# RuyiLian/CheckerPose

Hardware: AMD Instinct MI355X
Metric: crops/sec forward (256x256, npt=512) (higher is better)
Workload: dtype bf16; 1 GPU; LMO 'ape' hr18GNN2_res6_gnn3Skip_mlpQuery npt=512, PoseNet_GNNskip forward, deterministic random-init weights; global_batch=256, parallelism=dp1 (no forward collective), launch=hipGraph replay of 104 kernel launches

## Files before the change

checkerpose_amd/_abi.py:

```python
import ctypes as C
import os

_HERE = os.path.dirname(os.path.abspath(__file__))
LIB_PATH = os.environ.get("CHECKERPOSE_AMD_LIB") or os.path.join(_HERE, "libcheckerpose_hip.so")

CP_F32, CP_BF16, CP_F16 = 0, 1, 2
ACT_NONE, ACT_RELU, ACT_LEAKY = 0, 1, 2
LOSS_BCE, LOSS_L1 = 0, 1
POSE_ERR_ADD, POSE_ERR_ADI = 1, 2


class CpConvDesc(C.Structure):
    _fields_ = [("dtype", C.c_int32), ("out_f32", C.c_int32), ("B", C.c_int32), ("H", C.c_int32), ("W", C.c_int32),
                ("Cin", C.c_int32), ("in_cstride", C.c_int32), ("in_coff", C.c_int32),
                ("R", C.c_int32), ("S", C.c_int32), ("stride", C.c_int32), ("pad", C.c_int32),
                ("Ho", C.c_int32), ("Wo", C.c_int32), ("Cout", C.c_int32), ("act", C.c_int32), ("slope", C.c_float), ("ksplit", C.c_int32),
                ("o_base", C.c_int64), ("o_sb", C.c_int64), ("o_sy", C.c_int64), ("o_sx", C.c_int64),
                ("o_sc", C.c_int64)]


_P, _I, _F, _L = C.c_void_p, C.c_int, C.c_float, C.c_longlong


class CpChainTail(C.Structure):
    _fields_ = [("packed_w", C.c_void_p), ("shift", C.c_void_p), ("out", C.c_void_p * 3), ("nconv", C.c_int32),
                ("Cout", C.c_int32 * 3), ("out_cphys", C.c_int32 * 3), ("relu", C.c_int32 * 3)]


class CpChainTailConv(C.Structure):
    _fields_ = [("packed_w", C.c_void_p), ("shift", C.c_void_p), ("out", C.c_void_p),
                ("kind", C.c_int32), ("Cout", C.c_int32), ("out_cphys", C.c_int32), ("relu", C.c_int32)]


class CpI2fGather(C.Structure):
    _fields_ = [("patches", C.c_void_p), ("x_id", C.c_void_p), ("y_id", C.c_void_p), ("mask", C.c_void_p), ("zeros", C.c_void_p),
                ("p_cstride", C.c_int32), ("p_coff", C.c_int32), ("Hp", C.c_int32), ("Wp", C.c_int32), ("k", C.c_int32)]


class CpFuseConv(C.Structure):
    _fields_ = [("packed_w", C.c_void_p), ("affine", C.c_void_p), ("out", C.c_void_p),
                ("kind", C.c_int32), ("Cout", C.c_int32), ("out_cphys", C.c_int32), ("relu", C.c_int32)]


class CpPackItem(C.Structure):
    _fields_ = [("kind", C.c_int32), ("a", C.c_int32 * 9), ("src", C.c_void_p), ("dst", C.c_void_p), ("row_map", C.c_void_p),
                ("total", C.c_uint64)]


class CpWgradReduceItem(C.Structure):
    _fields_ = [("ws", C.c_void_p), ("dw", C.c_void_p), ("S", C.c_int32), ("GY", C.c_int32), ("co_blocks", C.c_int32),
                ("ci_blocks", C.c_int32), ("R", C.c_int32), ("Ssz", C.c_int32), ("Cout", C.c_int32), ("Cin", C.c_int32),
                ("taps_in_block", C.c_int32), ("dw_base", C.c_int64), ("dw_sco", C.c_int64), ("dw_sci", C.c_int64),
                ("dw_sr", C.c_int64), ("dw_ss", C.c_int64)]


CP_BN_ITEM_STATS, CP_BN_ITEM_APPLY, CP_BN_ITEM_BWD_SUMS, CP_BN_ITEM_BWD_APPLY = 0, 1, 2, 3
BN_GROUP_MAX = 16


class CpBnItem(C.Structure):
    _fields_ = [("kind", C.c_int32), ("dtype", C.c_int32), ("blocks", C.c_uint32), ("lds_bytes", C.c_uint32),
                ("params", C.c_uint64 * 24)]


CP_WGRAD_ITEM_3X3, CP_WGRAD_ITEM_3X3_SMALL, CP_WGRAD_ITEM_GENERIC_BF16, CP_WGRAD_ITEM_GENERIC_F32 = 0, 1, 2, 3
CP_WGRAD_ITEM_3X3_S2_SMALL = 4


class CpWgradItem(C.Structure):
    _fields_ = [("kind", C.c_int32), ("blocks", C.c_uint32), ("gx", C.c_uint32), ("gy", C.c_uint32), ("params", C.c_uint64 * 20)]


class CpOptItem(C.Structure):
    _fields_ = [("p", C.c_void_p), ("g", C.c_void_p), ("m", C.c_void_p), ("v", C.c_void_p), ("n", C.c_uint64), ("step0", C.c_uint32),
                ("pad", C.c_uint32)]


class CpFuseBwdItem(C.Structure):
    _fields_ = [("dout", C.c_void_p), ("out", C.c_void_p), ("dsrc", C.c_void_p), ("Hs", C.c_int32), ("Ws", C.c_int32), ("CG", C.c_int32),
                ("shift", C.c_int32), ("relu", C.c_int32), ("accumulate", C.c_int32), ("total", C.c_uint64)]


class CpWgradDesc(C.Structure):
    _fields_ = [("dtype", C.c_int32), ("B", C.c_int32), ("H", C.c_int32), ("W", C.c_int32), ("Ho", C.c_int32),
                ("Wo", C.c_int32), ("Cout", C.c_int32), ("dy_cstride", C.c_int32), ("dy_coff", C.c_int32),
                ("Cin", C.c_int32), ("x_cstride", C.c_int32), ("x_coff", C.c_int32),
                ("R", C.c_int32), ("S", C.c_int32), ("stride", C.c_int32), ("pad", C.c_int32),
                ("dw_base", C.c_int64), ("dw_sco", C.c_int64), ("dw_sci", C.c_int64), ("dw_sr", C.c_int64),
                ("dw_ss", C.c_int64)]


SIGNATURES = {
    "cp_version": (_I, []),
    "cp_device_status": (_I, [_P, _I]),
    "cp_set_deterministic": (None, [_I]),
    "cp_get_deterministic": (_I, []),
    "cp_strerror": (C.c_char_p, [_I]),
    "cp_last_kernel": (C.c_char_p, []),
    "cp_kernel_log_begin": (None, []),
    "cp_kernel_log": (C.c_char_p, []),
    "cp_chan_align": (_I, [_I]),
    "cp_packed_weight_bytes": (C.c_size_t, [_I, _I, _I, _I, _I]),
    "cp_pack_conv_weight": (_I, [_P, _I, _P, _I, _I, _I, _I, _I, _I, _I, _P, _I, _P]),
    "cp_conv2d_igemm": (_I, [_P, C.POINTER(CpConvDesc), _P, _P, _P, _P, _P, _P]),
    "cp_conv2d_igemm_splitk": (_I, [_I, C.c_longlong, _I, _I]),
    "cp_packed_halo_weight_bytes": (C.c_size_t, [_I, _I, _I]),
    "cp_pack_conv3x3_halo_weight": (_I, [_P, _I, _P, _I, _I, _I, _P]),
    "cp_conv3x3_halo": (_I, [_P, C.POINTER(CpConvDesc), _P, _P, _P, _P, _P, _P]),
    "cp_conv2x2_halo_supported": (_I, [_I, _I, _I, _I]),
    "cp_packed_conv2x2_halo_weight_bytes": (C.c_size_t, [_I, _I, _I]),
    "cp_pack_conv2x2_halo_weight": (_I, [_P, _I, _P, _I, _I, _I, _P]),
    "cp_conv2x2_halo": (_I, [_P, C.POINTER(CpConvDesc), _P, _P, _P, _P, _P, _P]),
    "cp_conv3x3_s2_small_supported": (_I, [_I, _I, _I, _I]),
    "cp_conv3x3_s2_small_weight_bytes": (C.c_size_t, [_I, _I]),
    "cp_pack_conv3x3_s2_small_weight": (_I, [_P, _P, _I, _I, _I, _I, _P]),
    "cp_conv3x3_s2_small": (_I, [_P, C.POINTER(CpConvDesc), _P, _P, _P, _P, _P]),
    "cp_conv3x3_halo_up2x_supported": (_I, [_I, _I]),
    "cp_conv3x3_halo_up2x": (_I, [_P, C.POINTER(CpConvDesc), _P, _P, _P, _P, _P]),
    "cp_conv3x3_halo_seg_supported": (_I, [_I, _I, _I]),
    "cp_conv3x3_halo_seg": (_I, [_P, C.POINTER(CpConvDesc), _P, _P, _P, _P, _P, _P, _P, _I, _P]),
    "cp_pack_conv3x3_rows_weight": (_I, [_P, _I, _P, _I, _I, _I, _P]),
    "cp_basicblock_fused": (_I, [_P, C.POINTER(CpConvDesc), _P, _P, _P, _P, _P, _P, _P, _P]),
    "cp_bottleneck_fused": (_I, [_P, C.POINTER(CpConvDesc)] + [_P] * 14),
    "cp_packed_gemm_weight_bytes": (C.c_size_t, [_I, _I, _I]),
    "cp_pack_gemm_weight": (_I, [_P, _I, _P, _I, _I, _I, _P]),
    "cp_gemm_rows": (_I, [_P, C.POINTER(CpConvDesc), _P, _P, _P, _P, _P, _P]),
    "cp_mlp_query_fused_supported": (_I, [_I, _I, _I, _I]),
    "cp_mlp_query_fused": (_I, [_P, _P, _I, _I, _I, _I, _P, _P, _P, _F, _P, _P, _P, _F, _P, _P, _P, _L, _L, _L, _L]),
    "cp_mlp_query_fused_t": (_I, [_P, _I, _P, _I, _I, _I, _I, _P, _P, _P, _F, _P, _P, _P, _F, _P, _P, _P, _L, _L, _L, _L]),
    "cp_mlp_query_fused_n": (_I, [_P, _I, _P, _I, _I, _I, _I, _P, _P, _P, _F, _P, _P, _P, _F, _P, _P, _I, _P, _L, _L, _L, _L,
                                  _P, _P, _P, _P]),
    "cp_mlp_pair_fused_supported": (_I, [_I, _I, _I]),
    "cp_mlp_pair_fused": (_I, [_P, _P, _I, _I, _I, _I, _I, _P, _P, _F, _P, _P, _F, _P, _I, _I]),
    "cp_mlp_pair_fused_t": (_I, [_P, _I, _P, _I, _I, _I, _I, _I, _P, _P, _F, _P, _P, _F, _P, _I, _I]),
    "cp_mlp_pair_fused_gather_supported": (_I, [_I, _I, _I]),
    "cp_mlp_pair_fused_gather": (_I, [_P, C.POINTER(CpI2fGather), _P, _I, _I, _I, _I, _I, _P, _P, _F, _P, _P, _F, _P, _I, _I]),
    "cp_mlp_pair_fused_gather_t": (_I, [_P, _I, C.POINTER(CpI2fGather), _P, _I, _I, _I, _I, _I, _P, _P, _F, _P, _P, _F, _P, _I, _I]),
    "cp_hr_stem_weight_bytes": (C.c_size_t, [_I]),
    "cp_pack_hr_stem_weights": (_I, [_P, _P, _P, _P, _P]),
    "cp_hr_stem": (_I, [_P, _P, _I, _I, _I, _P, _P, _P, _P, _P, _P, _P]),
    "cp_hr_chain_supported": (_I, [_I, _I, _I]),
    "cp_hr_chain_weight_bytes": (C.c_size_t, [_I, _I, _I]),
    "cp_hr_chain_affine_floats": (_I, [_I, _I, _I]),
    "cp_pack_hr_chain_weight": (_I, [_P, _P, _P, _I, _I, _I, _I, _P]),
    "cp_hr_branch_chain": (_I, [_P, _I, _I, _I, _I, _I, C.POINTER(_P), C.POINTER(C.c_int32), _I, _P, _P, _P]),
    "cp_hr_chain_tail_supported": (_I, [_I, _I, _I]),
    "cp_hr_chain_tail_weight_bytes": (C.c_size_t, []),
    "cp_hr_chain_tail_channels": (_I, []),
    "cp_pack_hr_chain_tail_weight": (_I, [_P, _P, _P, _I, _I, _I, _P]),
    "cp_hr_branch_chain_tail": (_I, [_P, _I, _I, _I, _I, _I, C.POINTER(_P), C.POINTER(C.c_int32), _I, _P, _P, _P, C.POINTER(CpChainTail)]),
    "cp_hr_chain_tailconv_supported": (_I, [_I, _I, _I, _I, _I]),
    "cp_hr_chain_tailconv_weight_bytes": (C.c_size_t, [_I, _I, _I, _I, _I]),
    "cp_pack_hr_chain_tailconv_weight": (_I, [_P, _P, _P, _I, _I, _I, _I, _I, _P]),
    "cp_hr_branch_chain_tails": (_I, [_P, _I, _I, _I, _I, _I, C.POINTER(_P), C.POINTER(C.c_int32), _I, _P, _P, _P, _I, C.POINTER(CpChainTailConv)]),
    "cp_upsample2x_bilinear_ac": (_I, [_P, _I, _P, _P, _I, _I, _I, _I, _I, _I, _I, _I]),
    "cp_fuse_sum_act": (_I, [_P, _I, _I, C.POINTER(_P), C.POINTER(C.c_int32), _P, _I, _I, _I, _I, _I, _I, _I]),
    "cp_maxpool3x3s2": (_I, [_P, _I, _P, _P, _I, _I, _I, _I]),
    "cp_edgeconv_gather_max": (_I, [_P, _I, _P, _P, _P, _P, _I, _I, _I, _I, _I, _I, _I, _F]),
    "cp_hr_fuse_out_supported": (_I, [_I, _I, _I]),
    "cp_hr_fuse_out_weight_bytes": (C.c_size_t, [_I, _I, _I]),
    "cp_hr_fuse_out_affine_floats": (_I, [_I]),
    "cp_pack_hr_fuse_out_weight": (_I, [_P, _P, _I, _I, _I, _I, _I, _P]),
    "cp_hr_fuse_out": (_I, [_P, _P, _I, _I, _I, _I, _I, C.POINTER(CpFuseConv)]),
    "cp_edgeconv_fused_supported": (_I, [_I, _I, _I, _I]),
    "cp_edgeconv_fused_weight_bytes": (C.c_size_t, [_I, _I]),
    "cp_pack_edgeconv_fused_weight": (_I, [_P, _P, _I, _I, _P]),
    "cp_edgeconv_fused": (_I, [_P, _P, _I, _I, _P, _P, _P, _P, _P, _P, _I, _I, _I, _I, _I, _I, _I, _I, _F]),
    "cp_pack_edgeconv_fused_weight_t": (_I, [_P, _I, _P, _I, _I, _P]),
    "cp_edgeconv_fused_t": (_I, [_P, _I, _P, _I, _I, _P, _P, _P, _P, _P, _P, _I, _I, _I, _I, _I, _I, _I, _I, _F]),
    "cp_edgeconv_tiled_supported": (_I, [_I, _I, _I, _I, _I]),
    "cp_edgeconv_tiled_weight_bytes": (C.c_size_t, [_I, _I]),
    "cp_edgeconv_tiled_table_bytes": (C.c_size_t, [_I, _I, _I]),
    "cp_pack_edgeconv_tiled_weight": (_I, [_P, _P, _I, _I, _P]),
    "cp_edgeconv_tiled": (_I, [_P, _P, _I, _I, _P, _P, _P, _P, _P, _P, _P, _P, _P, _I, _I, _I, _I, _I, _I, _I, _I, _I, _F]),
    "cp_pack_edgeconv_tiled_weight_t": (_I, [_P, _I, _P, _I, _I, _P]),
    "cp_edgeconv_tiled_t": (_I, [_P, _I, _P, _I, _I, _P, _P, _P, _P, _P, _P, _P, _P, _P, _I, _I, _I, _I, _I, _I, _I, _I, _I, _F]),
    "cp_permute_rows": (_I, [_P, _P, _P, _P, _P, _I, _I, _I]),
    "cp_permute_cols": (_I, [_P, _P, _P, _P, _P, _I, _I, _I, _I, _I]),
    "cp_index2feat_conv_supported": (_I, [_I, _I, _I]),
    "cp_index2feat_conv_weight_bytes": (C.c_size_t, []),
    "cp_pack_index2feat_conv_weight": (_I, [_P, _P, _P]),
    "cp_index2feat_conv": (_I, [_P, _P, _I, _I, _P, _P, _P, _P, _P, _P, _I, _I, _I, _I, _I, _I, _I]),
    "cp_index2feat_conv_t": (_I, [_P, _I, _P, _I, _I, _P, _P, _P, _P, _P, _P, _I, _I, _I, _I, _I, _I, _I]),
    "cp_index2feat_gather": (_I, [_P, _I, _P, _P, _P, _P, _P, _I, _I, _I, _I, _I, _I, _I, _I]),
    "cp_bits_decode": (_I, [_P, _P, _I, _P, _P, _P, _P, _P, _I, _I]),
    "cp_code_decode": (_I, [_P, _P, _I, _I, _P, _P, _P, _P, _I, _I]),
    "cp_correspondences": (_I, [_P, _P, _P, _P, _P, _P, _P, _P, _P, _I, _I, _I, _I, _I]),
    "cp_correspondences_bbox": (_I, [_P, _P, _P, _P, _P, _P, _P, _P, _P, _I, _I, _I, _I, _I]),
    "cp_pnp_ransac_scratch_bytes": (C.c_size_t, [_I, _I]),
    "cp_pnp_ransac": (_I, [_P, _P, _L, _P, _P, _I, _P, _L, _I, _I, _F, _I, C.c_uint32, _P, _P, _P, _P]),
    "cp_pose_errors_scratch_bytes": (C.c_size_t, [_I, _I]),
    "cp_pose_errors": (_I, [_P, _P, _P, _P, _P, _I, _P, _I, _I, _I, _P, _P, _P]),
    "cp_encode_targets": (_I, [_P, _P, _L, _P, _I, _P, _L, _P, _P, _P, _P, _P, _I, _I, _I, _P, _P, _P, _P, _P, _P, _P]),
    "cp_code_report": (_I, [_P, _P, _L, _P, _L, _P, _L, _I, _P, _I, _I, _P, _P, _P, _I, _P, _P, _I, _I, _I, _I, _P, _P]),
    "cp_edgeconv_bwd_workspace_bytes": (C.c_size_t, [_I, _I, _I]),
    "cp_edgeconv_gather_max_bwd": (_I, [_P, _I, _P, _P, _P, _P, _P, _P, _P, _P, _I, _I, _I, _I, _I, _I, _I, _F]),
    "cp_index2feat_gather_bwd": (_I, [_P, _P, _P, _P, _P, _P, _I, _I, _I, _I, _I, _I, _I, _I]),
    "cp_loss_workspace_bytes": (C.c_size_t, []),
    "cp_code_loss": (_I, [_P, _I, _P, _L, _P, _L, _P, _I, _I, _I, _P, _P, _L, _P]),
    "cp_mask_loss": (_I, [_P, _P, _L, _P, _I, _I, _I, _I, _I, _P, _P, _L, _P]),
    "cp_masked_ce_loss": (_I, [_P, _P, _L, _P, _P, _I, _I, _I, _P, _P, _L, _P]),
    "cp_conv2d_wgrad": (_I, [_P, C.POINTER(CpWgradDesc), _P, _P, _P]),
    "cp_conv2d_wgrad_ws": (_I, [_P, C.POINTER(CpWgradDesc), _P, _P, _P, _P, C.c_size_t]),
    "cp_conv2d_wgrad_scratch_bytes": (C.c_size_t, [C.POINTER(CpWgradDesc)]),
    "cp_conv2d_wgrad_deferred": (_I, [_P, C.POINTER(CpWgradDesc), _P, _P, _P, _P, C.c_size_t, C.POINTER(CpWgradReduceItem)]),
    "cp_conv2d_wgrad_plan": (_I, [C.POINTER(CpWgradDesc), _P, _P, _P, _P, C.c_size_t, C.POINTER(CpWgradReduceItem)]),
    "cp_conv2d_wgrad_item": (_I, [C.POINTER(CpWgradDesc), _P, _P, _P, _P, C.c_size_t, _I, C.POINTER(CpWgradItem), C.POINTER(CpWgradReduceItem)]),
    "cp_wgrad_group": (_I, [_P, _I, _P, _P, _I, C.c_uint32]),
    "cp_opt_item_blocks": (C.c_uint32, [C.c_uint64]),
    "cp_adam_multi": (_I, [_P, _P, _P, _I, C.c_uint32, _F, _F, _F, _F, _F, _I]),
    "cp_sgd_multi": (_I, [_P, _P, _P, _I, C.c_uint32, _F, _F, _F, _I]),
    "cp_wgrad_reduce_item_blocks": (C.c_uint32, [C.POINTER(CpWgradReduceItem)]),
    "cp_wgrad_reduce_batch": (_I, [_P, _P, _P, _I, C.c_uint32]),
    "cp_weight_dgrad": (_I, [_P, _P, _I, _I, _I, _I, _P]),
    "cp_bn_workspace_bytes": (C.c_size_t, [_I]),
    "cp_bn_train_stats": (_I, [_P, _I, _P, _I, _I, _I, _I, _P, _P, _P, _P, _F, _F, _P, _P, _P, _P, _P]),
    "cp_affine_act": (_I, [_P, _I, _P, _I, _I, _P, _P, _P, _I, _I, _P, _I, _I, _I, _I, _I, _F]),
    "cp_bn_bwd_workspace_bytes": (C.c_size_t, [_I]),
    "cp_bn_train_bwd": (_I, [_P, _I, _P, _I, _I, _P, _I, _I, _P, _I, _I, _P, _P, _P, _I, _I, _I, _F, _P, _I, _I, _P, _I, _I,
                             _I, _P, _P, _P]),
    "cp_pack_item_conv": (_I, [_I, _P, _I, _I, _I, _I, _I, _I, _I, _P, _I, _P, C.POINTER(CpPackItem)]),
    "cp_pack_item_halo": (_I, [_I, _P, _I, _I, _I, _P, C.POINTER(CpPackItem)]),
    "cp_pack_item_gemm": (_I, [_I, _P, _I, _I, _I, _P, C.POINTER(CpPackItem)]),
    "cp_pack_item_dgrad_view": (_I, [_P, _I, _I, _I, _I, _P, C.POINTER(CpPackItem)]),
    "cp_pack_item_edge_view": (_I, [_P, _I, _I, _I, _P, C.POINTER(CpPackItem)]),
    "cp_pack_item_copy_f32": (_I, [_P, _P, _I, C.POINTER(CpPackItem)]),
    "cp_pack_batch": (_I, [_P, _I, _P, _P, _I, C.c_uint32]),
    "cp_bn_acc_doubles": (C.c_size_t, [_I]),
    "cp_bn_stats_accumulate": (_I, [_P, _I, _P, _I, _I, _I, _I, _P]),
    "cp_bn_apply": (_I, [_P, _I, _P, _I, _I, _P, _P, _P, _P, _P, _F, _F, _P, _I, _I, _P, _I, _I, _I, _I, _I, _F, _P, _P]),
    "cp_bn_bwd_accumulate": (_I, [_P, _I, _P, _I, _I, _P, _I, _I, _P, _I, _I, _P, _P, _I, _I, _I, _F, _P]),
    "cp_bn_bwd_apply": (_I, [_P, _I, _P, _I, _I, _P, _I, _I, _P, _I, _I, _P, _P, _P, _P, _I, _I, _I, _F, _P, _I, _I, _P, _I, _I,
                             _I, _P, _P]),
    "cp_bn_item_stats": (_I, [_I, _P, _I, _I, _I, _I, _P, C.POINTER(CpBnItem)]),
    "cp_bn_item_apply": (_I, [_I, _P, _I, _I, _P, _P, _P, _P, _P, _F, _F, _P, _I, _I, _P, _I, _I, _I, _I, _I, _F, _P, _P,
                              C.POINTER(CpBnItem)]),
    "cp_bn_item_bwd_sums": (_I, [_I, _P, _I, _I, _P, _I, _I, _P, _I, _I, _P, _P, _I, _I, _I, _F, _P, C.POINTER(CpBnItem)]),
    "cp_bn_item_bwd_apply": (_I, [_I, _P, _I, _I, _P, _I, _I, _P, _I, _I, _P, _P, _P, _P, _I, _I, _I, _F, _P, _I, _I, _P, _I, _I,
                                  _I, _P, _P, C.POINTER(CpBnItem)]),
    "cp_bn_group": (_I, [_P, _I, _I, _P, _P, _I, C.c_uint32, C.c_uint32]),
    "cp_edge_train_workspace_bytes": (C.c_size_t, [_I, _I]),
# ... 78 lines not shown
```

checkerpose_amd/csrc/hr_chain.hip:

```cpp
#include <stdlib.h>

#include "common.h"

size_t cp_chain0_conv_bytes();
int cp_chain0_aff();
int cp_chain0_pack(hipStream_t st, const float* w, const float* scale, int conv_index, void* blob);
int cp_chain0_launch(hipStream_t st, int B, int nsrc, const void* const* srcs, const int32_t* shifts, int relu_in,
                     const void* packed_w, const float* affine, void* out, const CpChainTail* tail);
size_t cp_chain0_tail_bytes();
int cp_chain0_tail_channels();
int cp_chain0_tail_pack(hipStream_t st, const float* w, const float* scale, int Cout, int first_piece, int out_cphys, void* blob);

namespace {

template <int C_, int H_, int W_, int CPW_, int NWC_, int S_, int RL_>
struct ChainCfg {
  static constexpr int C = C_, H = H_, W = W_, CPW = CPW_, NWC = NWC_, S = S_, RL = RL_;
  static constexpr int NW = 8, NTHR = 512;
  static constexpr int CPHYS = (C + 7) / 8 * 8;
  static constexpr int CG = CPHYS / 8;
  static constexpr int NT_ALL = (C + 15) / 16;
  static constexpr int KC = (9 * CG + 3) / 4;
  static constexpr int KCP = (KC + S - 1) / S * S;
  static constexpr int NS = KCP / S;
  static constexpr int HP = H + 2, WP = W + 2;
  static constexpr bool PLANES = W >= 16;
  static constexpr int PLANE = (HP * WP + 15) / 16 * 16 * 16;
  static constexpr int SLOTS = (CG % 2) ? CG : CG + 1;
  static constexpr int PIX = PLANES ? 16 : SLOTS * 16;
  static constexpr int GRP = PLANES ? PLANE : 16;
  static constexpr int MAP = PLANES ? CG * PLANE : HP * WP * SLOTS * 16;
  static constexpr int FPC = H * W / 16;
  static constexpr int NFRAG = CPW * FPC;
  static constexpr int NWP = NW / NWC;
  static constexpr int MT = NFRAG / NWP;
  static constexpr int PM = MT < 4 ? MT : 4;
  static constexpr int NST = MT / PM;
  static constexpr int NTW = (NT_ALL + NWC - 1) / NWC;
  static constexpr int SLAB = S * NT_ALL * 1024;
  static constexpr int WITER = (SLAB / 16 + NTHR - 1) / NTHR;
  static constexpr int AFF = NT_ALL * 16;
  static constexpr int AFF_BYTES = 2 * 2 * AFF * 4;
  static constexpr int RES_LDS = NW * RL * NTW * 64 * 8;
  static constexpr int LDS = CPW * MAP + 2 * SLAB + AFF_BYTES + RES_LDS;
  static constexpr size_t CONV_W = (size_t)KCP * NT_ALL * 1024;
  static_assert(NFRAG % NWP == 0 && MT % PM == 0 && RL <= MT, "fragments must split evenly over the pixel waves");
  static_assert(W >= 16 ? (W % 16 == 0) : (W == 8), "fragment = 16 pixels of a row, or two 8-pixel rows");
  static_assert((SLAB / 16) % 64 == 0, "slab pieces are copied by whole waves");
  static_assert(LDS <= 160 * 1024, "LDS budget");
};

using CfgB1 = ChainCfg<36, 32, 32, 1, 1, 3, 4>;
using CfgB2 = ChainCfg<72, 16, 16, 2, 1, 3, 0>;
using CfgB3 = ChainCfg<144, 8, 8, 4, 2, 2, 0>;
using CfgB2m = ChainCfg<72, 16, 16, 1, 1, 3, 0>;
using CfgB3h = ChainCfg<144, 8, 8, 2, 2, 2, 0>;
using CfgB3m = ChainCfg<144, 8, 8, 1, 2, 2, 0>;

struct ChainTailConv {
  const void* w;
  const float* shift;
  void* out;
  int kind, nt, out_cp, relu;
};
struct ChainParams {
  const void* src[4];
  int shift[4];
  int nsrc, relu_in;
  const void* w;
  const float* aff;
  void* out;
  int B;
  int dbg;
  int ntail;
  ChainTailConv tc[3];
};

#ifdef CP_DEBUG_KNOBS
#define CHAIN_DBG(bit) (p.dbg & (bit))
#else
#define CHAIN_DBG(bit) 0
#endif

__device__ __forceinline__ void mma16(const u32x4& w, const u32x4& a, f32x4& acc) {
  acc = __builtin_amdgcn_mfma_f32_16x16x32_bf16(__builtin_bit_cast(bf16x8, w), __builtin_bit_cast(bf16x8, a), acc, 0, 0, 0);
}

template <typename Cfg, int NSRC>
__device__ __forceinline__ void stage_sources(const ChainParams& p, unsigned char* sMap, int tid, int crop0) {
  constexpr int CG = Cfg::CG, H = Cfg::H, W = Cfg::W, U = 4;
  constexpr int TOTAL = Cfg::CPW * H * W * CG;
  for (int i0 = tid; i0 < TOTAL; i0 += U * Cfg::NTHR) {
    u32x4 v[U][NSRC];
    uint32_t dst[U];
    bool ok[U];
#pragma unroll
    for (int u = 0; u < U; ++u) {
      const int i = i0 + u * Cfg::NTHR;
      const int g = i % CG;
      int t = i / CG;
      const int c = t / (H * W);
      t -= c * (H * W);
      const int y = t / W, xx = t - y * W;
      const int b = crop0 + c;
      ok[u] = i < TOTAL;
      dst[u] = (uint32_t)(c * Cfg::MAP + ((y + 1) * Cfg::WP + xx + 1) * Cfg::PIX + g * Cfg::GRP);
      const bool ld = ok[u] && b < p.B && !(CHAIN_DBG(1));
#pragma unroll
      for (int k = 0; k < NSRC; ++k) {
        const int sh = p.shift[k];
        const size_t o = (((size_t)b * (H >> sh) + (y >> sh)) * (W >> sh) + (xx >> sh)) * CG + g;
        v[u][k] = ld ? ((const u32x4*)p.src[k])[o] : u32x4{0u, 0u, 0u, 0u};
      }
    }
#pragma unroll
    for (int u = 0; u < U; ++u) {
      float acc[8], f[8];
#pragma unroll
      for (int k = 0; k < NSRC; ++k) {
        Vec16<BF16Tag>::unpack(v[u][k], f);
#pragma unroll
        for (int j = 0; j < 8; ++j) acc[j] = (k == 0) ? f[j] : acc[j] + f[j];
      }
      if (p.relu_in) {
#pragma unroll
        for (int j = 0; j < 8; ++j) acc[j] = fmaxf(acc[j], 0.f);
      }
      if (ok[u]) *(u32x4*)(sMap + dst[u]) = Vec16<BF16Tag>::pack(acc);
    }
  }
}

template <typename Cfg, int KIND, int NT, int TG>
__device__ __forceinline__ void chain_tail_conv(const ChainTailConv& t, const unsigned char* sMap, int lane, int wave, int crop0, int B) {
  constexpr int CG = Cfg::CG, H = Cfg::H, W = Cfg::W, WP = Cfg::WP, PIX = Cfg::PIX, GRP = Cfg::GRP, MAP = Cfg::MAP, CPW = Cfg::CPW;
  constexpr int HT = KIND ? H / 2 : H, WT = KIND ? W / 2 : W;
  static_assert(WT >= 16 ? WT % 16 == 0 : WT == 8, "a tail fragment is 16 pixels of an output row, or two 8-pixel rows");
  constexpr int FG = 8 / TG, NTW = (NT + TG - 1) / TG;
  constexpr int FPC = HT * WT / 16, NF = CPW * FPC, FW = (NF + FG - 1) / FG;
  constexpr int KC = KIND ? (9 * CG + 3) / 4 : (CG + 3) / 4;
  constexpr uint32_t CENTER = (uint32_t)((WP + 1) * PIX);
  const int x = lane & 15, q = lane >> 4;
  const int tg = wave % TG, fg = wave / TG;
  const int nt0 = tg * NTW;
  if (nt0 >= NT) return;
  const int ntn = nt0 + NTW <= NT ? NTW : NT - nt0;
  uint32_t base[FW];
  int opix[FW];
  int crop[FW];
#pragma unroll
  for (int f = 0; f < FW; ++f) {
    const int F = fg + FG * f;
    const int c = F / FPC, Fc = F - c * FPC;
    int orow, ocol;
    if (WT >= 16) { orow = Fc / (WT / 16); ocol = (Fc - orow * (WT / 16)) * 16 + x; }
    else { orow = Fc * 2 + (x >> 3); ocol = x & 7; }
    const bool live = F < NF;
    crop[f] = c;
// ... 202 lines not shown
    }

#pragma unroll 1
    for (int s = 0; s < NS; ++s, ++gs) {
      if (gs + 1 < TOTAL_SLABS && !CHAIN_DBG(8)) slab_issue(gs + 1, (gs + 1) & 1);
      if (active) {
        const unsigned char* const sWb = sW + (gs & 1) * SLAB + nt0 * 1024 + lane * 16;
        const int kc0 = s * S;
        u32x4 af[2][PM], wf[2][NTW];
        {
          const uint32_t o = a_off(kc0);
#pragma unroll
          for (int i = 0; i < PM; ++i) af[0][i] = *(const u32x4*)(sMap + base[i] + o);
#pragma unroll
          for (int nt = 0; nt < NTW; ++nt)
            if (has(nt)) wf[0][nt] = *(const u32x4*)(sWb + nt * 1024);
        }
#pragma unroll
        for (int cc = 0; cc < S; ++cc) {
#pragma unroll
          for (int st = 0; st < NST; ++st) {
            const int cur = (cc * NST + st) & 1;
            const bool last = (cc == S - 1) && (st == NST - 1);
            if (!last) {
              const int ncc = (st == NST - 1) ? cc + 1 : cc, nst = (st == NST - 1) ? 0 : st + 1;
              const uint32_t o = a_off(kc0 + ncc);
#pragma unroll
              for (int i = 0; i < PM; ++i) af[cur ^ 1][i] = *(const u32x4*)(sMap + base[nst * PM + i] + o);
            }
            if (st == 0 && cc + 1 < S) {
#pragma unroll
              for (int nt = 0; nt < NTW; ++nt)
                if (has(nt)) wf[(cc + 1) & 1][nt] = *(const u32x4*)(sWb + ((cc + 1) * NT_ALL + nt) * 1024);
            }
            __builtin_amdgcn_sched_barrier(0);
#pragma unroll
            for (int i = 0; i < PM; ++i)
#pragma unroll
              for (int nt = 0; nt < NTW; ++nt)
                if (has(nt)) mma16(wf[cc & 1][nt], af[cur][i], acc[st * PM + i][nt]);
            __builtin_amdgcn_sched_barrier(0);
          }
        }
      }
      __syncthreads();
    }

    if (tid < 2 * AFF) sAff[((cv + 1) & 1) * 2 * AFF + tid] = affv;
    {
#pragma unroll
      for (int nt = 0; nt < NTW; ++nt) {
        const int c0 = q * 4 * NT_ALL + (nt0 + nt) * 4;
        if (has(nt) && c0 < CPHYS) {
          uint32_t co = c_off(c0);
          asm volatile("" : "+v"(co));
#pragma unroll
          for (int f = 0; f < MT; ++f) {
            u32x2 pk;
            pk.x = relu_bf16x2(pack_bf16x2(acc[f][nt][0], acc[f][nt][1]));
            pk.y = relu_bf16x2(pack_bf16x2(acc[f][nt][2], acc[f][nt][3]));
            *(u32x2*)(sMap + base[f] + co) = pk;
          }
        }
      }
    }
    __syncthreads();
  }

  if (!CHAIN_DBG(4)) {
    constexpr int TOTAL = CPW * H * W * CG;
#pragma unroll 4
    for (int i = tid; i < TOTAL; i += NTHR) {
      const int g = i % CG;
      int t = i / CG;
      const int c = t / (H * W);
      t -= c * (H * W);
      const int y = t / W, xx = t - y * W;
      const int b = crop0 + c;
      if (b < p.B)
        ((u32x4*)p.out)[(((size_t)b * H + y) * W + xx) * CG + g] = *(const u32x4*)(sMap + c * MAP + ((y + 1) * WP + xx + 1) * PIX + g * GRP);
    }
  }
  if constexpr (TAIL) chain_tails<Cfg>(p, sMap, lane, wave, crop0);
}

__global__ void pack_chain_tail_kernel(const float* __restrict__ w, const float* __restrict__ scale, uint16_t* __restrict__ out, int Cin,
                                       int CG, int Cout, int NT, int kind, size_t total) {
  const size_t i = (size_t)blockIdx.x * blockDim.x + threadIdx.x;
  if (i >= total) return;
  const int e = (int)(i % 8);
  const int lane = (int)((i / 8) % 64);
  size_t blk = i / 512;
  const int nt = (int)(blk % NT);
  const int kc = (int)(blk / NT);
  const int row = lane & 15, q = lane >> 4;
  const int G = kc * 4 + q;
  int tap = -1, cin = 0;
  if (kind) { tap = G / CG; cin = (G % CG) * 8 + e; if (tap >= 9) tap = -1; }
  else if (G < CG) { tap = 0; cin = G * 8 + e; }
  const int n = (row >> 2) * 4 * NT + nt * 4 + (row & 3);
  const int KK = kind ? 9 : 1;
  float v = 0.f;
  if (tap >= 0 && cin < Cin && n < Cout) v = w[((size_t)n * Cin + cin) * KK + tap] * (scale ? scale[n] : 1.f);
  out[i] = (uint16_t)f32_to_bf16_bits(v);
}

__global__ void pack_chain_weight_kernel(const float* __restrict__ w, const float* __restrict__ scale, uint16_t* __restrict__ out, int C,
                                         int CG, int NT_ALL, size_t total) {
  const size_t i = (size_t)blockIdx.x * blockDim.x + threadIdx.x;
  if (i >= total) return;
  const int e = (int)(i % 8);
  const int lane = (int)((i / 8) % 64);
  size_t blk = i / 512;
  const int nt = (int)(blk % NT_ALL);
  const int kc = (int)(blk / NT_ALL);
  const int row = lane & 15, q = lane >> 4;
  const int G = kc * 4 + q;
  const int tap = G / CG, cin = (G % CG) * 8 + e;
  const int n = (row >> 2) * 4 * NT_ALL + nt * 4 + (row & 3);
  float v = 0.f;
  if (tap < 9 && cin < C && n < C) v = w[((size_t)n * C + cin) * 9 + tap] * (scale ? scale[n] : 1.f);
  out[i] = (uint16_t)f32_to_bf16_bits(v);
}

constexpr int CHAIN_CPW_FULL_B = 192;

template <typename Cfg>
int launch_chain(hipStream_t st, const ChainParams& p) {
  static CpDeviceOnce once;
  const int dev = cp_current_device();
  CP_LDS_ATTR_ONCE(once, dev, cp_set_max_lds((const void*)hr_chain_kernel<Cfg, false>, Cfg::LDS) &&
                                  cp_set_max_lds((const void*)hr_chain_kernel<Cfg, true>, Cfg::LDS));
  const unsigned grid = (unsigned)((p.B + Cfg::CPW - 1) / Cfg::CPW);
  if (p.ntail > 0) CP_LAUNCH((hr_chain_kernel<Cfg, true>), dim3(grid), dim3(Cfg::NTHR), Cfg::LDS, st, p);
  else CP_LAUNCH((hr_chain_kernel<Cfg, false>), dim3(grid), dim3(Cfg::NTHR), Cfg::LDS, st, p);
  return cp_check_launch();
}

int tail_conv_chunks(int C, int kind, int nt) {
  const int CG = (C + 7) / 8;
  bool ok = false;
  if (C == 36) ok = (kind == 0 && nt == 2) || (kind == 1 && (nt == 5 || nt == 3));
  else if (C == 72) ok = (kind == 0 && (nt == 2 || nt == 3)) || (kind == 1 && nt == 9);
  else if (C == 144) ok = kind == 0 && (nt == 2 || nt == 3 || nt == 5);
  if (!ok) return 0;
  return kind ? (9 * CG + 3) / 4 : (CG + 3) / 4;
}

struct ChainInfo { int C, H, W, KCP, NT_ALL, CG, AFF; size_t conv_w; };
bool chain_info(int C, int H, int W, ChainInfo* o) {
#define CP_CI(CFG) if (C == CFG::C && H == CFG::H && W == CFG::W) { *o = ChainInfo{C, H, W, CFG::KCP, CFG::NT_ALL, CFG::CG, CFG::AFF, CFG::CONV_W}; return true; }
  CP_CI(CfgB1) CP_CI(CfgB2) CP_CI(CfgB3)
#undef CP_CI
  if (C == 18 && H == 64 && W == 64) { *o = ChainInfo{C, H, W, 7, 2, 3, cp_chain0_aff(), cp_chain0_conv_bytes()}; return true; }
  return false;
}

}

extern "C" int cp_hr_chain_supported(int C, int H, int W) {
  ChainInfo ci;
  return chain_info(C, H, W, &ci) ? 1 : 0;
}

extern "C" size_t cp_hr_chain_weight_bytes(int C, int H, int W) {
  ChainInfo ci;
  return chain_info(C, H, W, &ci) ? 8 * ci.conv_w : 0;
}

extern "C" int cp_hr_chain_affine_floats(int C, int H, int W) {
  ChainInfo ci;
  return chain_info(C, H, W, &ci) ? ci.AFF : 0;
}

extern "C" int cp_pack_hr_chain_weight(cp_stream_t stream, const float* w, const float* scale, int C, int H, int W, int conv_index,
                                       void* blob) {
  ChainInfo ci;
  if (!w || !blob || conv_index < 0 || conv_index > 7 || !chain_info(C, H, W, &ci)) return CP_ERR_INVALID;
  if (!cp_aligned16(blob)) return CP_ERR_ALIGN;
  if (C == 18) return cp_chain0_pack((hipStream_t)stream, w, scale, conv_index, blob);
  const size_t total = ci.conv_w / 2;
  uint16_t* dst = (uint16_t*)((unsigned char*)blob + (size_t)conv_index * ci.conv_w);
  CP_LAUNCH(pack_chain_weight_kernel, dim3((unsigned)((total + 255) / 256)), dim3(256), 0, (hipStream_t)stream, w, scale, dst, C, ci.CG, ci.NT_ALL, total);
  return cp_check_launch();
}

extern "C" int cp_hr_chain_tail_supported(int C, int H, int W) { return (C == 18 && H == 64 && W == 64) ? 1 : 0; }
extern "C" size_t cp_hr_chain_tail_weight_bytes(void) { return cp_chain0_tail_bytes(); }
extern "C" int cp_hr_chain_tail_channels(void) { return cp_chain0_tail_channels(); }
extern "C" int cp_pack_hr_chain_tail_weight(cp_stream_t stream, const float* w, const float* scale, int Cout, int first_piece, int out_cphys,
                                            void* blob) {
  return cp_chain0_tail_pack((hipStream_t)stream, w, scale, Cout, first_piece, out_cphys, blob);
}

static int branch_chain(cp_stream_t stream, int B, int C, int H, int W, int nsrc, const void* const* srcs, const int32_t* shifts, int relu_in,
                        const void* packed_w, const float* affine, void* out, const CpChainTail* tail, int ntail = 0,
                        const CpChainTailConv* tconvs = nullptr);

extern "C" int cp_hr_chain_tailconv_supported(int C, int H, int W, int kind, int Cout) {
  ChainInfo ci;
  if (C == 18 || !chain_info(C, H, W, &ci) || Cout <= 0 || (kind != 0 && kind != 1)) return 0;
  return tail_conv_chunks(C, kind, (Cout + 15) / 16) > 0 ? 1 : 0;
}
extern "C" size_t cp_hr_chain_tailconv_weight_bytes(int C, int H, int W, int kind, int Cout) {
  if (!cp_hr_chain_tailconv_supported(C, H, W, kind, Cout)) return 0;
  const int nt = (Cout + 15) / 16;
  return (size_t)tail_conv_chunks(C, kind, nt) * nt * 1024;
}
extern "C" int cp_pack_hr_chain_tailconv_weight(cp_stream_t stream, const float* w, const float* scale, int C, int H, int W, int kind, int Cout,
                                                void* packed) {
  if (!w || !packed || !cp_hr_chain_tailconv_supported(C, H, W, kind, Cout)) return CP_ERR_INVALID;
  if (!cp_aligned16(packed)) return CP_ERR_ALIGN;
  const int nt = (Cout + 15) / 16;
  const size_t total = cp_hr_chain_tailconv_weight_bytes(C, H, W, kind, Cout) / 2;
  CP_LAUNCH(pack_chain_tail_kernel, dim3((unsigned)((total + 255) / 256)), dim3(256), 0, (hipStream_t)stream, w, scale, (uint16_t*)packed, C,
            (C + 7) / 8, Cout, nt, kind, total);
  return cp_check_launch();
}
extern "C" int cp_hr_branch_chain_tails(cp_stream_t stream, int B, int C, int H, int W, int nsrc, const void* const* srcs, const int32_t* shifts,
                                        int relu_in, const void* packed_w, const float* affine, void* out, int ntail, const CpChainTailConv* convs) {
  if (ntail < 1 || ntail > 3 || !convs || C == 18) return CP_ERR_INVALID;
  return branch_chain(stream, B, C, H, W, nsrc, srcs, shifts, relu_in, packed_w, affine, out, nullptr, ntail, convs);
}

extern "C" int cp_hr_branch_chain(cp_stream_t stream, int B, int C, int H, int W, int nsrc, const void* const* srcs,
                                  const int32_t* shifts, int relu_in, const void* packed_w, const float* affine, void* out) {
  return branch_chain(stream, B, C, H, W, nsrc, srcs, shifts, relu_in, packed_w, affine, out, nullptr);
}

extern "C" int cp_hr_branch_chain_tail(cp_stream_t stream, int B, int C, int H, int W, int nsrc, const void* const* srcs,
                                       const int32_t* shifts, int relu_in, const void* packed_w, const float* affine, void* out,
                                       const CpChainTail* tail) {
  if (!tail || !cp_hr_chain_tail_supported(C, H, W)) return CP_ERR_INVALID;
  return branch_chain(stream, B, C, H, W, nsrc, srcs, shifts, relu_in, packed_w, affine, out, tail);
}

static int branch_chain(cp_stream_t stream, int B, int C, int H, int W, int nsrc, const void* const* srcs, const int32_t* shifts, int relu_in,
                        const void* packed_w, const float* affine, void* out, const CpChainTail* tail, int ntail, const CpChainTailConv* tconvs) {
  ChainInfo ci;
  if (B <= 0 || !srcs || !shifts || nsrc < 1 || nsrc > 4 || !packed_w || !affine || !out) return CP_ERR_INVALID;
  if (!chain_info(C, H, W, &ci)) return CP_ERR_INVALID;
  if (!cp_aligned16(packed_w) || !cp_aligned16(affine) || !cp_aligned16(out)) return CP_ERR_ALIGN;
  ChainParams p;
  for (int k = 0; k < 4; ++k) { p.src[k] = nullptr; p.shift[k] = 0; }
  for (int k = 0; k < nsrc; ++k) {
    if (!srcs[k] || !cp_aligned16(srcs[k]) || shifts[k] < 0 || shifts[k] > 3) return CP_ERR_INVALID;
    if (((H >> shifts[k]) << shifts[k]) != H || ((W >> shifts[k]) << shifts[k]) != W) return CP_ERR_INVALID;
    if (srcs[k] == out) return CP_ERR_INVALID;
    p.src[k] = srcs[k]; p.shift[k] = shifts[k];
  }
  if (C == 18) return cp_chain0_launch((hipStream_t)stream, B, nsrc, srcs, shifts, relu_in, packed_w, affine, out, tail);
  p.nsrc = nsrc; p.relu_in = relu_in ? 1 : 0;
  p.w = packed_w; p.aff = affine; p.out = out; p.B = B;
  p.dbg = cp_knob("CP_CHAIN_DBG") ? atoi(cp_knob("CP_CHAIN_DBG")) : 0;
  p.ntail = 0;
  for (int i = 0; i < ntail; ++i) {
    const CpChainTailConv& c = tconvs[i];
    const int nt = (c.Cout + 15) / 16;
    if (!c.packed_w || !c.shift || !c.out || c.out == out || !cp_hr_chain_tailconv_supported(C, H, W, c.kind, c.Cout)) return CP_ERR_INVALID;
    if (c.out_cphys % 8 || c.Cout > c.out_cphys || c.out_cphys > nt * 16) return CP_ERR_INVALID;
    if (!cp_aligned16(c.packed_w) || !cp_aligned16(c.shift) || !cp_aligned16(c.out)) return CP_ERR_ALIGN;
    p.tc[i].w = c.packed_w; p.tc[i].shift = c.shift; p.tc[i].out = c.out;
    p.tc[i].kind = c.kind; p.tc[i].nt = nt; p.tc[i].out_cp = c.out_cphys; p.tc[i].relu = c.relu ? 1 : 0;
  }
  p.ntail = ntail;
  hipStream_t st = (hipStream_t)stream;
  if (C == CfgB1::C) return launch_chain<CfgB1>(st, p);
  if (C == CfgB2::C) return B >= CHAIN_CPW_FULL_B ? launch_chain<CfgB2>(st, p) : launch_chain<CfgB2m>(st, p);
  if (B >= CHAIN_CPW_FULL_B) return launch_chain<CfgB3>(st, p);
  return B >= CHAIN_CPW_FULL_B / 2 ? launch_chain<CfgB3h>(st, p) : launch_chain<CfgB3m>(st, p);
}
```

checkerpose_amd/csrc/hr_chain0.hip:

```cpp
#include "common.h"

namespace {

constexpr int ZH = 64, ZW = 64, ZC = 18, ZWP = 66, ZHP = 66;
constexpr int ZPLPX = (ZHP * ZWP + 15) / 16 * 16;
constexpr int ZPL16 = ZPLPX * 16, ZPL4 = ZPLPX * 4;
constexpr int ZAFF = 32;
constexpr int ZLDS = 2 * ZPL16 + ZPL4 + 2 * 2 * ZAFF * 4;
constexpr int ZKC = 6;
constexpr size_t ZCONV_W = (size_t)ZKC * 2 * 1024;
static_assert(ZLDS <= 160 * 1024, "LDS budget");

struct Chain0Params {
  const void* src[4];
  int shift[4];
  int nsrc, relu_in;
  const void* w;
  const float* aff;
  void* out;
  int B;
  int tnp;
  int tps[3], tcph[3], trelu[3];
  const void* tw;
  const float* tshift;
  void* tout[3];
  uint32_t* status;
  int dbg_spin_limit;
};
constexpr int ZTAIL_CH = 96;

__device__ __forceinline__ void mma16z(const u32x4& w, const u32x4& a, f32x4& acc) {
  acc = __builtin_amdgcn_mfma_f32_16x16x32_bf16(__builtin_bit_cast(bf16x8, w), __builtin_bit_cast(bf16x8, a), acc, 0, 0, 0);
}

template <int NSRC>
__device__ __forceinline__ void stage0(const Chain0Params& p, unsigned char* smem, int tid, int b) {
  constexpr int U = 4, TOTAL = ZH * ZW * 3;
  for (int i0 = tid; i0 < TOTAL; i0 += U * 512) {
    u32x4 v[U][NSRC];
#pragma unroll
    for (int u = 0; u < U; ++u) {
      const int i = i0 + u * 512;
      const int g = i % 3, px = i / 3;
      const int y = px >> 6, xx = px & 63;
#pragma unroll
      for (int k = 0; k < NSRC; ++k) {
        const int sh = p.shift[k];
        const size_t o = (((size_t)b * (ZH >> sh) + (y >> sh)) * (ZW >> sh) + (xx >> sh)) * 3 + g;
        v[u][k] = ((const u32x4*)p.src[k])[o];
      }
    }
#pragma unroll
    for (int u = 0; u < U; ++u) {
      const int i = i0 + u * 512;
      const int g = i % 3, px = i / 3;
      const int y = px >> 6, xx = px & 63;
      float acc[8], f[8];
#pragma unroll
      for (int k = 0; k < NSRC; ++k) {
        Vec16<BF16Tag>::unpack(v[u][k], f);
#pragma unroll
        for (int j = 0; j < 8; ++j) acc[j] = (k == 0) ? f[j] : acc[j] + f[j];
      }
      if (p.relu_in) {
#pragma unroll
        for (int j = 0; j < 8; ++j) acc[j] = fmaxf(acc[j], 0.f);
      }
      const u32x4 pk = Vec16<BF16Tag>::pack(acc);
      const int pc = (y + 1) * ZWP + xx + 1;
      if (g < 2) *(u32x4*)(smem + g * ZPL16 + pc * 16) = pk;
      else *(uint32_t*)(smem + 2 * ZPL16 + pc * 4) = pk.x;
      ((u32x4*)p.out)[((size_t)b * ZH * ZW + px) * 3 + g] = pk;
    }
  }
}

#ifdef CP_DEBUG_KNOBS
__device__ unsigned long long z_stamps[8][8];
#define Z_T0() unsigned long long z_t = __builtin_amdgcn_s_memtime(), z_acc[8] = {0, 0, 0, 0, 0, 0, 0, 0}
#define Z_MARK(k) do { const unsigned long long n_ = __builtin_amdgcn_s_memtime(); z_acc[k] += n_ - z_t; z_t = n_; } while (0)
#define Z_DUMP() do { if (blockIdx.x == 0 && lane == 0) for (int k_ = 0; k_ < 8; ++k_) z_stamps[wave][k_] = z_acc[k_]; } while (0)
#else
#define Z_T0() do {} while (0)
#define Z_MARK(k) do {} while (0)
#define Z_DUMP() do {} while (0)
#endif

__global__ __launch_bounds__(512) void hr_chain0_kernel(const Chain0Params p) {
  extern __shared__ __attribute__((aligned(16))) unsigned char smem[];
  float* const sAff = (float*)(smem + 2 * ZPL16 + ZPL4);
  const int tid = threadIdx.x;
  const int lane = tid & 63;
  const int wave = __builtin_amdgcn_readfirstlane(tid >> 6);
  const int x = lane & 15, q = lane >> 4;
  const int b = blockIdx.x;

  const u32x4* const wg = (const u32x4*)p.w;
  u32x4 Wf[ZKC][2];
#pragma unroll
  for (int kc = 0; kc < ZKC; ++kc)
#pragma unroll
    for (int nt = 0; nt < 2; ++nt) Wf[kc][nt] = wg[(kc * 2 + nt) * 64 + lane];

  for (int i = tid; i < ZPLPX; i += 512) {
    const int ry = i / ZWP, rx = i - ry * ZWP;
    if (ry == 0 || ry >= ZH + 1 || rx == 0 || rx == ZW + 1) {
      *(u32x4*)(smem + i * 16) = u32x4{0u, 0u, 0u, 0u};
      *(u32x4*)(smem + ZPL16 + i * 16) = u32x4{0u, 0u, 0u, 0u};
      *(uint32_t*)(smem + 2 * ZPL16 + i * 4) = 0u;
    }
// ... 353 lines not shown
      const uint32_t a16 = live && g < 2 ? ro + (uint32_t)(g * PP1 + (px + 1) * 16) : POOR;
      const uint32_t a4 = live && g == 2 ? ro + (uint32_t)(PP2 + (px + 1) * 4) : POOR;
      *(u32x4*)(smem + a16) = pk;
      *(uint32_t*)(smem + a4) = pk.x;
      p_post(cnt + PC_PART + part, (p_cnt_t*)nullptr, (uint32_t)(ys + 1), lane);
      ++ys;
      did = true;
    }
    if (oy < ZH / 2 && p_peek(cnt + 8) >= (2 * oy + 2 < ZH ? 2 * oy + 2 : ZH)) {
      asm volatile("" ::: "memory");
      uint32_t rb[3];
#pragma unroll
      for (int r = 0; r < 3; ++r) {
        const int yy = 2 * oy - 1 + r;
        rb[r] = yy < 0 ? (uint32_t)PZERO : p_ring(8) + p_slot(8, yy);
      }
      f32x4 acc[2][2];
      u32x4 af[2][2];
      p_load<2>(af[0], 0, smem, tg, rb, qlo, q3);
#pragma unroll
      for (int kc = 0; kc < ZKC; ++kc) {
        if (kc + 1 < ZKC) p_load<2>(af[(kc + 1) & 1], kc + 1, smem, tg, rb, qlo, q3);
        __builtin_amdgcn_sched_barrier(0);
#pragma unroll
        for (int f = 0; f < 2; ++f) {
          if (kc == 0) {
            acc[f][0] = __builtin_amdgcn_mfma_f32_16x16x32_bf16(__builtin_bit_cast(bf16x8, Wt[0][0]), __builtin_bit_cast(bf16x8, af[0][f]), tt0, 0, 0, 0);
            acc[f][1] = __builtin_amdgcn_mfma_f32_16x16x32_bf16(__builtin_bit_cast(bf16x8, Wt[0][1]), __builtin_bit_cast(bf16x8, af[0][f]), tt1, 0, 0, 0);
          } else {
            mma16z(Wt[kc][0], af[kc & 1][f], acc[f][0]);
            mma16z(Wt[kc][1], af[kc & 1][f], acc[f][1]);
          }
        }
        __builtin_amdgcn_sched_barrier(0);
      }
      if (tlive) {
#pragma unroll
        for (int f = 0; f < 2; ++f) {
          float e[8];
#pragma unroll
          for (int j = 0; j < 4; ++j) { e[j] = acc[f][0][j]; e[4 + j] = acc[f][1][j]; }
          u32x4 pk = Vec16<BF16Tag>::pack(e);
          if (trelu) { pk.x = relu_bf16x2(pk.x); pk.y = relu_bf16x2(pk.y); pk.z = relu_bf16x2(pk.z); pk.w = relu_bf16x2(pk.w); }
          *(u32x4*)(ob + (size_t)(oy * 32 + 16 * f + x) * cph * 2) = pk;
        }
      }
      p_post(cnt + PC_TAIL + part, (p_cnt_t*)nullptr, (uint32_t)(oy + 1), lane);
      ++oy;
      did = true;
    }
    if (!did) __builtin_amdgcn_s_sleep(1);
  }
  if ((ys < ZH || oy < ZH / 2) && p.status && lane == 0) atomicOr(p.status, (uint32_t)CP_STATUS_CHAIN0_STAGING);
}

__global__ __launch_bounds__(PNT) void hr_chain0p_kernel(const Chain0Params p) {
  extern __shared__ __attribute__((aligned(16))) unsigned char smem[];
  const int tid = threadIdx.x;
  const int lane = tid & 63;
  const int wave = __builtin_amdgcn_readfirstlane(tid >> 6);
  const int x = lane & 15, q = lane >> 4;
  const int b = blockIdx.x;
  p_cnt_t* const cnt = (p_cnt_t*)(smem + PCNT);

  for (int i = tid; i < PROWS * 2; i += PNT) {
    const int rr = i >> 1, px = (i & 1) ? ZWP - 1 : 0;
    unsigned char* const row = smem + rr * PROW;
    *(u32x4*)(row + px * 16) = u32x4{0u, 0u, 0u, 0u};
    *(u32x4*)(row + PP1 + px * 16) = u32x4{0u, 0u, 0u, 0u};
    *(uint32_t*)(row + PP2 + px * 4) = 0u;
  }
  for (int i = tid; i < PROW / 16; i += PNT) *(u32x4*)(smem + PZERO + i * 16) = u32x4{0u, 0u, 0u, 0u};
  if (tid < 32) cnt[tid] = 0u;
  if (tid < 8 * ZAFF) ((float*)(smem + PSHF))[tid] = p.aff[(tid / ZAFF) * 2 * ZAFF + ZAFF + (tid % ZAFF)];
  __syncthreads();

  if (wave >= 8) {
    switch (p.nsrc) {
      case 1: p_stage_and_tail<1>(p, smem, lane, b, wave - 8); break;
      case 2: p_stage_and_tail<2>(p, smem, lane, b, wave - 8); break;
      case 3: p_stage_and_tail<3>(p, smem, lane, b, wave - 8); break;
      default: p_stage_and_tail<4>(p, smem, lane, b, wave - 8); break;
    }
    return;
  }

#ifdef CP_C0_PLAIN_MAP
  const int s = wave;
#else
  const int s = 2 * (wave & 3) + (wave >> 2);
#endif
  const bool second = s & 1;
  const int nslab = (p.tnp + 3) >> 2;
  const u32x4* const wg = (const u32x4*)p.w + (size_t)s * ZKC * 2 * 64;
  u32x4 Wf[ZKC][2];
#pragma unroll
  for (int kc = 0; kc < ZKC; ++kc)
#pragma unroll
    for (int nt = 0; nt < 2; ++nt) Wf[kc][nt] = wg[(kc * 2 + nt) * 64 + lane];
  const float* const sh = (const float*)(smem + PSHF) + s * ZAFF + q * 8;
#ifndef CP_C0_PRIO_ODD
#define CP_C0_PRIO_ODD 2
#endif
#ifndef CP_C0_PRIO_EVEN
#define CP_C0_PRIO_EVEN 1
#endif
  if (second) __builtin_amdgcn_s_setprio(CP_C0_PRIO_ODD);
  else if (CP_C0_PRIO_EVEN) __builtin_amdgcn_s_setprio(CP_C0_PRIO_EVEN);
  const PGeo cg = p_geo(x, q, 1);
  const bool q3 = q == 3, qlo = q < 2;
  uint32_t wb16 = q < 2 ? (uint32_t)(q * PP1 + (1 + x) * 16) : POOR, wb4 = q == 2 ? (uint32_t)(PP2 + (1 + x) * 4) : POOR;
  asm volatile("" : "+v"(wb16), "+v"(wb4));
  const uint32_t rin = p_ring(s), rout = p_ring(s + 1), rrs = p_ring(second ? s - 1 : 0);
  const int dout = p_depth(s + 1);
  const size_t gpix0 = (size_t)b * ZH * ZW;

  Z_T0();
#pragma unroll 1
  for (int y = 0; y < ZH; ++y) {
    const int need = y + 2 < ZH ? y + 2 : ZH;
    Z_MARK(0);
    if (s == 0) {
#pragma unroll
      for (int k = 0; k < PSW; ++k) p_wait(cnt + PC_PART + k, need, p);
    } else p_wait(cnt + s, need, p);
    Z_MARK(1);
    uint32_t rb[3];
#pragma unroll
    for (int r = 0; r < 3; ++r) {
      const int yy = y - 1 + r;
      rb[r] = (yy < 0 || yy >= ZH) ? (uint32_t)PZERO : rin + p_slot(s, yy);
    }
    u32x4 rbig[4];
    uint32_t rsm[4];
    if (second) {
      const uint32_t rr = rrs + p_slot(s - 1, y);
      const uint32_t rbg = (qlo ? rr : (uint32_t)PZERO) + (uint32_t)((q & 1) * PP1 + (1 + x) * 16);
#pragma unroll
      for (int f = 0; f < 4; ++f) {
        rbig[f] = *(const u32x4*)(smem + rbg + f * 256);
        rsm[f] = *(const uint32_t*)(smem + rr + PP2 + (1 + x) * 4 + f * 64);
      }
    }
    f32x4 acc[4][2];
    u32x4 af[PFD + 1][4];
    const f32x4 t0 = *(const f32x4*)(sh), t1 = *(const f32x4*)(sh + 4);
#pragma unroll
    for (int k = 0; k < PFD; ++k) p_load<4>(af[k], k, smem, cg, rb, qlo, q3);
#pragma unroll
    for (int kc = 0; kc < ZKC; ++kc) {
      if (kc + PFD < ZKC) p_load<4>(af[(kc + PFD) % (PFD + 1)], kc + PFD, smem, cg, rb, qlo, q3);
      __builtin_amdgcn_sched_barrier(0);
#pragma unroll
      for (int f = 0; f < 4; ++f) {
        if (kc == 0) {
          acc[f][0] = __builtin_amdgcn_mfma_f32_16x16x32_bf16(__builtin_bit_cast(bf16x8, Wf[0][0]), __builtin_bit_cast(bf16x8, af[0][f]), t0, 0, 0, 0);
          acc[f][1] = __builtin_amdgcn_mfma_f32_16x16x32_bf16(__builtin_bit_cast(bf16x8, Wf[0][1]), __builtin_bit_cast(bf16x8, af[0][f]), t1, 0, 0, 0);
        } else {
          mma16z(Wf[kc][0], af[kc % (PFD + 1)][f], acc[f][0]);
          mma16z(Wf[kc][1], af[kc % (PFD + 1)][f], acc[f][1]);
        }
      }
      __builtin_amdgcn_sched_barrier(0);
    }
    Z_MARK(2);
#ifndef CP_C0_LATE_CONS
    p_post(cnt + PC_CONS + s, (p_cnt_t*)nullptr, (uint32_t)(y + 1), lane);
#endif
    u32x4 v[4];
#pragma unroll
    for (int f = 0; f < 4; ++f) {
      float e[8];
#pragma unroll
      for (int j = 0; j < 4; ++j) { e[j] = acc[f][0][j]; e[4 + j] = acc[f][1][j]; }
      if (second) {
        const u32x4 raw = u32x4{qlo ? rbig[f].x : rsm[f], rbig[f].y, rbig[f].z, rbig[f].w};
        float r8[8];
        Vec16<BF16Tag>::unpack(raw, r8);
#pragma unroll
        for (int j = 0; j < 8; ++j) e[j] += r8[j];
      }
      u32x4 pk = Vec16<BF16Tag>::pack(e);
      pk.x = relu_bf16x2(pk.x); pk.y = relu_bf16x2(pk.y); pk.z = relu_bf16x2(pk.z); pk.w = relu_bf16x2(pk.w);
      v[f] = pk;
    }
    Z_MARK(3);
    if (s == 7 && q < 3) {
#pragma unroll
      for (int f = 0; f < 4; ++f) ((u32x4*)p.out)[(gpix0 + y * ZW + f * 16 + x) * 3 + q] = v[f];
    }
    if (s < 7 || nslab > 0) {
      if (y >= dout) {
        if (s == 7) {
          for (int k = 0; k < nslab; ++k) p_wait(cnt + PC_TAIL + k, (y - dout + 1) / 2 + 1, p);
        } else if (second) p_wait(cnt + PC_CONS + s + 2, y - (dout - 1), p);
        else p_wait(cnt + PC_CONS + s + 1, y - (dout - 2), p);
      }
      Z_MARK(4);
      const uint32_t ro = rout + p_slot(s + 1, y);
#pragma unroll
      for (int f = 0; f < 4; ++f) {
        *(u32x4*)(smem + ro + wb16 + f * 256) = v[f];
        *(uint32_t*)(smem + ro + wb4 + f * 64) = v[f].x;
      }
#ifdef CP_C0_LATE_CONS
      p_post(cnt + s + 1, cnt + PC_CONS + s, (uint32_t)(y + 1), lane);
    } else p_post(cnt + PC_CONS + s, (p_cnt_t*)nullptr, (uint32_t)(y + 1), lane);
#else
      p_post(cnt + s + 1, (p_cnt_t*)nullptr, (uint32_t)(y + 1), lane);
    }
#endif
    Z_MARK(5);
  }
  Z_DUMP();
}
__global__ void pack_chain0_weight_kernel(const float* __restrict__ w, const float* __restrict__ scale, uint16_t* __restrict__ out, size_t total) {
  const size_t i = (size_t)blockIdx.x * blockDim.x + threadIdx.x;
  if (i >= total) return;
  const int e = (int)(i % 8);
  const int lane = (int)((i / 8) % 64);
  const int nt = (int)((i / 512) % 2);
  const int kc = (int)(i / 1024);
  const int row = lane & 15, q = lane >> 4;
  const int G = kc * 4 + q;
  int tap = -1, cin = 0;
  if (G < 18) { tap = G >> 1; cin = (G & 1) * 8 + e; }
  else if (G < 21 && (G - 18) * 4 + (e >> 1) < 9) { tap = (G - 18) * 4 + (e >> 1); cin = 16 + (e & 1); }
  const int n = (row >> 2) * 8 + nt * 4 + (row & 3);
  float v = 0.f;
  if (tap >= 0 && n < ZC && cin < ZC) v = w[((size_t)n * ZC + cin) * 9 + tap] * (scale ? scale[n] : 1.f);
  out[i] = (uint16_t)f32_to_bf16_bits(v);
}

__global__ void pack_chain0_tail_kernel(const float* __restrict__ w, const float* __restrict__ scale, uint16_t* __restrict__ out, int Cout,
                                        int ps, int cphys, size_t total) {
  const size_t i = (size_t)blockIdx.x * blockDim.x + threadIdx.x;
  if (i >= total) return;
  const int e = (int)(i % 8);
  const int lane = (int)((i / 8) % 64);
  const int nt = (int)((i / 512) % 2);
  const int kc = (int)((i / 1024) % ZKC);
  const int slab = (int)(i / (1024 * ZKC));
  const int row = lane & 15, q = lane >> 4;
  const int G = kc * 4 + q;
  int tap = -1, cin = 0;
  if (G < 18) { tap = G >> 1; cin = (G & 1) * 8 + e; }
  else if (G < 21 && (G - 18) * 4 + (e >> 1) < 9) { tap = (G - 18) * 4 + (e >> 1); cin = 16 + (e & 1); }
  const int c = slab * 32 + (row >> 2) * 8 + nt * 4 + (row & 3) - ps * 8;
  if (c < 0 || c >= cphys) return;
  float v = 0.f;
  if (tap >= 0 && c < Cout && cin < ZC) v = w[((size_t)c * ZC + cin) * 9 + tap] * (scale ? scale[c] : 1.f);
  out[i] = (uint16_t)f32_to_bf16_bits(v);
}

}

#ifdef CP_DEBUG_KNOBS
extern "C" int cp_debug_chain0_stamps(unsigned long long* out64) {
  return hipMemcpyFromSymbol(out64, HIP_SYMBOL(z_stamps), sizeof(unsigned long long) * 64) == hipSuccess ? CP_OK : CP_ERR_HIP;
}
#endif


size_t cp_chain0_conv_bytes() { return ZCONV_W; }
int cp_chain0_aff() { return ZAFF; }

int cp_chain0_pack(hipStream_t st, const float* w, const float* scale, int conv_index, void* blob) {
  const size_t total = ZCONV_W / 2;
  uint16_t* dst = (uint16_t*)((unsigned char*)blob + (size_t)conv_index * ZCONV_W);
  CP_LAUNCH(pack_chain0_weight_kernel, dim3((unsigned)((total + 255) / 256)), dim3(256), 0, st, w, scale, dst, total);
  return cp_check_launch();
}

int cp_chain0_launch(hipStream_t st, int B, int nsrc, const void* const* srcs, const int32_t* shifts, int relu_in,
                     const void* packed_w, const float* affine, void* out, const CpChainTail* tail) {
  static CpDeviceOnce once;
  const int dev = cp_current_device();
  CP_LDS_ATTR_ONCE(once, dev, cp_set_max_lds((const void*)hr_chain0_kernel, ZLDS));
  Chain0Params p = {};
  for (int k = 0; k < 4; ++k) { p.src[k] = k < nsrc ? srcs[k] : nullptr; p.shift[k] = k < nsrc ? shifts[k] : 0; }
  p.nsrc = nsrc; p.relu_in = relu_in ? 1 : 0; p.w = packed_w; p.aff = affine; p.out = out; p.B = B;
  p.status = cp_status_word(true);
  p.dbg_spin_limit = cp_knob("CP_C0_FORCE_TIMEOUT") ? atoi(cp_knob("CP_C0_FORCE_TIMEOUT")) : 0;
  if (tail) {
    if (tail->nconv < 1 || tail->nconv > 3 || !tail->packed_w || !tail->shift) return CP_ERR_INVALID;
    if (!cp_aligned16(tail->packed_w) || !cp_aligned16(tail->shift)) return CP_ERR_ALIGN;
    int ps = 0;
    for (int i = 0; i < 3; ++i) { p.tps[i] = 1 << 20; p.tcph[i] = 8; p.trelu[i] = 0; p.tout[i] = nullptr; }
    for (int i = 0; i < tail->nconv; ++i) {
      const int cph = tail->out_cphys[i];
      if (cph <= 0 || cph % 8 || tail->Cout[i] <= 0 || tail->Cout[i] > cph || !tail->out[i] || tail->out[i] == out) return CP_ERR_INVALID;
      if (!cp_aligned16(tail->out[i])) return CP_ERR_ALIGN;
      p.tps[i] = ps; p.tcph[i] = cph; p.trelu[i] = tail->relu[i] ? 1 : 0; p.tout[i] = tail->out[i];
      ps += cph / 8;
    }
    if (ps * 8 > ZTAIL_CH) return CP_ERR_INVALID;
    p.tnp = ps; p.tw = tail->packed_w; p.tshift = tail->shift;
  }
#ifndef CP_C0_BAND
  {
    static CpDeviceOnce once_p;
    CP_LDS_ATTR_ONCE(once_p, dev, cp_set_max_lds((const void*)hr_chain0p_kernel, PLDS));
    CP_LAUNCH(hr_chain0p_kernel, dim3((unsigned)B), dim3(PNT), PLDS, st, p);
    return cp_check_launch();
  }
#endif
  CP_LAUNCH(hr_chain0_kernel, dim3((unsigned)B), dim3(512), ZLDS, st, p);
  return cp_check_launch();
}

size_t cp_chain0_tail_bytes() { return (size_t)(ZTAIL_CH / 32) * ZCONV_W; }
int cp_chain0_tail_channels() { return ZTAIL_CH; }

int cp_chain0_tail_pack(hipStream_t st, const float* w, const float* scale, int Cout, int first_piece, int out_cphys, void* blob) {
  if (!w || !blob || Cout <= 0 || out_cphys % 8 || Cout > out_cphys || first_piece < 0 || first_piece * 8 + out_cphys > ZTAIL_CH) return CP_ERR_INVALID;
  if (!cp_aligned16(blob)) return CP_ERR_ALIGN;
  const size_t total = cp_chain0_tail_bytes() / 2;
  CP_LAUNCH(pack_chain0_tail_kernel, dim3((unsigned)((total + 255) / 256)), dim3(256), 0, st, w, scale, (uint16_t*)blob, Cout, first_piece, out_cphys, total);
  return cp_check_launch();
}
```

checkerpose_amd/csrc/hr_fuse_out.hip:

```cpp
#include "common.h"

namespace {

constexpr int FO_MAXCONV = 4, FO_NTB = 8, FO_MTB = 3, FO_THREADS = 256, FO_SLOTS = 192, FO_WB = 8, FO_SU = 17, FO_AFF = 160;

struct FuseConvDev {
  const void* w; const float* aff; void* out;
  int kind, relu, mt, nchunk, out_cp, aff_n;
};
struct FuseOutParams {
  const void* src;
  int B, H, W, Cg, band, nconv, plane_bytes;
  FuseConvDev c[FO_MAXCONV];
};

__device__ __forceinline__ void mma16f(const u32x4& w, const u32x4& a, f32x4& acc) {
  acc = __builtin_amdgcn_mfma_f32_16x16x32_bf16(__builtin_bit_cast(bf16x8, w), __builtin_bit_cast(bf16x8, a), acc, 0, 0, 0);
}

__global__ __launch_bounds__(FO_THREADS) void hr_fuse_out_kernel(const FuseOutParams p) {
  extern __shared__ __attribute__((aligned(16))) unsigned char smem[];
  const int tid = threadIdx.x;
  const int lane = tid & 63;
  const int wave = __builtin_amdgcn_readfirstlane(tid >> 6);
  const int x = lane & 15, q = lane >> 4;
  const int nband = p.H / p.band;
  const int b = blockIdx.x / nband, r0 = (blockIdx.x - b * nband) * p.band;
  const int RW = p.W + 1, RH = p.band + 1, Cg = p.Cg;
  const int HE = (p.W >> 1) + 1;
  auto colslot = [&](int rc) { return (rc & 1) ? HE + (rc >> 1) : (rc >> 1); };
  const int planes_end = Cg * p.plane_bytes;
  uint32_t* const tab = (uint32_t*)(smem + planes_end);

  float* const saff = (float*)(tab + 2 * FO_SLOTS);
  uint32_t* const sdesc = (uint32_t*)(saff + FO_MAXCONV * 2 * FO_AFF);
  if (wave == FO_THREADS / 64 - 1) {
    for (int s = lane; s < 2 * FO_SLOTS; s += 64) {
      const int kind = s >= FO_SLOTS, sl = s - kind * FO_SLOTS;
      uint32_t off = 0u;
      if (kind == 0) { if (sl < Cg) off = (uint32_t)(sl * p.plane_bytes); }
      else if (sl < 9 * Cg) {
        const int tap = sl / Cg, cg = sl - tap * Cg;
        const int ts = tap % 3;
        off = (uint32_t)(cg * p.plane_bytes + ((tap / 3) * RW + (ts == 1 ? HE : ts >> 1)) * 16);
      }
      tab[s] = off;
    }
#pragma unroll
    for (int ci = 0; ci < FO_MAXCONV; ++ci) {
      if (ci < p.nconv) {
        const float* const ga = p.c[ci].aff;
        const int an = p.c[ci].aff_n;
        for (int r = lane; r < 2 * FO_AFF; r += 64) {
          const int h = r >= FO_AFF, c = r - h * FO_AFF;
          saff[ci * 2 * FO_AFF + r] = c < an ? ga[h * an + c] : 0.f;
        }
        if (lane == 0) {
          const uint64_t wq = (uint64_t)p.c[ci].w, oq = (uint64_t)p.c[ci].out;
          uint32_t* d = sdesc + ci * 8;
          d[0] = (uint32_t)wq; d[1] = (uint32_t)(wq >> 32); d[2] = (uint32_t)oq; d[3] = (uint32_t)(oq >> 32);
          d[4] = (uint32_t)(p.c[ci].kind | (p.c[ci].relu << 1)); d[5] = (uint32_t)p.c[ci].mt; d[6] = (uint32_t)p.c[ci].nchunk;
          d[7] = (uint32_t)p.c[ci].out_cp;
        }
      }
    }
  }
  const int nconv = p.nconv;
  auto D = [&](int ci, int k) -> int { return __builtin_amdgcn_readfirstlane((int)sdesc[ci * 8 + k]); };
  {
    const int per_row = p.W * Cg;
    const u32x4* src = (const u32x4*)p.src + ((size_t)b * p.H * p.W) * Cg;
    for (int pc = tid; pc < per_row; pc += FO_THREADS) {
      const int c = pc / Cg, cg = pc - c * Cg;
      unsigned char* dst = smem + cg * p.plane_bytes + colslot(c + 1) * 16;
#pragma unroll 1
      for (int ry0 = 0; ry0 < RH; ry0 += FO_SU) {
        u32x4 v[FO_SU];
#pragma unroll
        for (int u = 0; u < FO_SU; ++u) {
          const int gy = r0 - 1 + ry0 + u;
          v[u] = u32x4{0u, 0u, 0u, 0u};
          if (ry0 + u < RH && gy >= 0) v[u] = src[(size_t)gy * per_row + pc];
        }
#pragma unroll
        for (int u = 0; u < FO_SU; ++u)
          if (ry0 + u < RH) *(u32x4*)(dst + (ry0 + u) * RW * 16) = v[u];
      }
    }
    for (int i = tid; i < RH * Cg; i += FO_THREADS) {
      const int ry = i / Cg, cg = i - ry * Cg;
      *(u32x4*)(smem + cg * p.plane_bytes + (ry * RW) * 16) = u32x4{0u, 0u, 0u, 0u};
    }
  }
  __syncthreads();

  auto split = [&](int n, int Wo, int& oy, int& ox) {
    if ((Wo & (Wo - 1)) == 0) { const int lw = 31 - __builtin_clz((unsigned)Wo); oy = n >> lw; ox = n & (Wo - 1); }
    else { oy = n / Wo; ox = n - oy * Wo; }
  };
  auto geom = [&](int ci, int& Wo, int& npx, int& ntile, int& npg, int& nrg) {
    const int kind = D(ci, 4) & 1;
    Wo = kind ? p.W >> 1 : p.W;
    npx = Wo * (kind ? p.band >> 1 : p.band);
    ntile = (npx + 15) >> 4;
    npg = (ntile + FO_NTB - 1) / FO_NTB;
    nrg = (D(ci, 5) + FO_MTB - 1) / FO_MTB;
  };
#pragma unroll 1
  for (int t0 = wave, ci = 0, tbase = 0; ci < nconv; ++ci) {
    int Wo, npx, ntile, npg, nrg;
    geom(ci, Wo, npx, ntile, npg, nrg);
    const int kind = D(ci, 4) & 1, relu = D(ci, 4) >> 1, mtc = D(ci, 5), nch = D(ci, 6), out_cp = D(ci, 7);
    const u32x4* const wbase = (const u32x4*)(((uint64_t)(uint32_t)D(ci, 1) << 32) | (uint32_t)D(ci, 0)) + lane;
    uint16_t* const outp = (uint16_t*)(((uint64_t)(uint32_t)D(ci, 3) << 32) | (uint32_t)D(ci, 2));
    const uint32_t* const tb = tab + (kind ? FO_SLOTS : 0);
    const int Ho = kind ? p.H >> 1 : p.H, oy0 = kind ? r0 >> 1 : r0;
    const int nitem = nrg * npg;
#pragma unroll 1
    for (; t0 < tbase + nitem; t0 += 4) {
      const int it = t0 - tbase;
      const int rg = it / npg, pg = it - rg * npg;
      const int mt0 = rg * FO_MTB, nm = mtc - mt0 < FO_MTB ? mtc - mt0 : FO_MTB;
      const int tlim = ntile - pg * FO_NTB;
      uint32_t base[FO_NTB];
      f32x4 acc[FO_MTB][FO_NTB];
#pragma unroll
      for (int i = 0; i < FO_NTB; ++i) {
        int n = (pg * FO_NTB + i) * 16 + x;
        if (n >= npx) n = 0;
        int oy, ox;
        split(n, Wo, oy, ox);
        base[i] = kind ? (uint32_t)(((2 * oy) * RW + ox) * 16) : (uint32_t)(((oy + 1) * RW + colslot(ox + 1)) * 16);
#pragma unroll
        for (int m = 0; m < FO_MTB; ++m) acc[m][i] = f32x4{0.f, 0.f, 0.f, 0.f};
      }
#pragma unroll 1
      for (int kb = 0; kb < nch; kb += FO_WB) {
        u32x4 wf[FO_MTB][FO_WB];
#pragma unroll
        for (int m = 0; m < FO_MTB; ++m)
#pragma unroll
          for (int k = 0; k < FO_WB; ++k) {
            wf[m][k] = u32x4{0u, 0u, 0u, 0u};
            if (m < nm && kb + k < nch) wf[m][k] = wbase[(size_t)((mt0 + m) * nch + kb + k) * 64];
          }
#pragma unroll
        for (int k = 0; k < FO_WB; ++k) {
          if (kb + k < nch) {
            const uint32_t so = tb[(kb + k) * 4 + q];
#pragma unroll
            for (int i4 = 0; i4 < FO_NTB; i4 += 4) {
              if (i4 < tlim) {
                u32x4 a[4];
#pragma unroll
                for (int i = 0; i < 4; ++i) a[i] = *(const u32x4*)(smem + base[i4 + i] + so);
#pragma unroll
                for (int m = 0; m < FO_MTB; ++m)
                  if (m < nm) {
#pragma unroll
                    for (int i = 0; i < 4; ++i) mma16f(wf[m][k], a[i], acc[m][i4 + i]);
                  }
              }
            }
          }
        }
      }
#pragma unroll
      for (int m = 0; m < FO_MTB; ++m) {
        const int co = (mt0 + m) * 16 + 4 * q;
        if (m < nm && co < out_cp) {
          const f32x4 sc = *(const f32x4*)(saff + ci * 2 * FO_AFF + co), sh = *(const f32x4*)(saff + ci * 2 * FO_AFF + FO_AFF + co);
#pragma unroll
          for (int i = 0; i < FO_NTB; ++i) {
            const int n = (pg * FO_NTB + i) * 16 + x;
            if (i < tlim && n < npx) {
              int oy, ox;
              split(n, Wo, oy, ox);
              float v[4];
#pragma unroll
              for (int j = 0; j < 4; ++j) {
                v[j] = acc[m][i][j] * sc[j] + sh[j];
                if (relu) v[j] = fmaxf(v[j], 0.f);
              }
              u32x2 pk; pk.x = pack_bf16x2(v[0], v[1]); pk.y = pack_bf16x2(v[2], v[3]);
              *(u32x2*)(outp + ((size_t)(b * Ho + oy0 + oy) * Wo + ox) * out_cp + co) = pk;
            }
          }
        }
      }
    }
    tbase += nitem;
  }
}

__global__ void pack_fuse_out_weight_kernel(const float* __restrict__ w, uint16_t* __restrict__ out, int Cout, int Cin, int kind,
                                            int Cg, int nchunk, size_t total) {
  const size_t i = (size_t)blockIdx.x * blockDim.x + threadIdx.x;
  if (i >= total) return;
  const int e = (int)(i & 7);
  const int lane = (int)((i >> 3) & 63);
  const size_t f = i >> 9;
  const int kc = (int)(f % nchunk), mt = (int)(f / nchunk);
  const int row = lane & 15, q = lane >> 4;
  const int co = mt * 16 + row, slot = kc * 4 + q;
  const int taps = kind ? 9 : 1;
  float v = 0.f;
  if (slot < taps * Cg) {
    const int tap = slot / Cg, cg = slot - tap * Cg;
    const int ci = cg * 8 + e;
    if (co < Cout && ci < Cin) v = w[((size_t)co * Cin + ci) * taps + tap];
  }
  out[i] = (uint16_t)f32_to_bf16_bits(v);
}

inline int fo_nchunk(int cin_phys, int kind) { return ((kind ? 9 : 1) * (cin_phys / 8) + 3) / 4; }
inline int fo_mt(int out_cphys) { return (out_cphys + 15) / 16; }

}

extern "C" int cp_hr_fuse_out_supported(int H, int W, int cin_phys) {
  if (H < 2 || W < 2 || (H & 1) || (W & 1) || cin_phys <= 0 || cin_phys % 8) return 0;
  const int Cg = cin_phys / 8;
  if (9 * Cg + 3 > FO_SLOTS) return 0;
  return (3 * (W + 1) * Cg * 16 + 16 * Cg <= 60 * 1024) ? 1 : 0;
}

extern "C" size_t cp_hr_fuse_out_weight_bytes(int cin_phys, int out_cphys, int kind) {
  return (size_t)fo_mt(out_cphys) * fo_nchunk(cin_phys, kind) * 1024;
}

extern "C" int cp_hr_fuse_out_affine_floats(int out_cphys) {
  return (out_cphys <= 0 || out_cphys % 8 || out_cphys > FO_AFF) ? 0 : fo_mt(out_cphys) * 16;
}

extern "C" int cp_pack_hr_fuse_out_weight(cp_stream_t stream, const float* w, int Cout, int Cin, int cin_phys, int out_cphys,
                                          int kind, void* packed) {
  if (!w || !packed || Cout <= 0 || Cin <= 0 || cin_phys % 8 || Cin > cin_phys || Cout > out_cphys || (kind != 0 && kind != 1))
    return CP_ERR_INVALID;
  if (!cp_aligned16(packed)) return CP_ERR_ALIGN;
  const int nchunk = fo_nchunk(cin_phys, kind);
  const size_t total = cp_hr_fuse_out_weight_bytes(cin_phys, out_cphys, kind) / 2;
  CP_LAUNCH(pack_fuse_out_weight_kernel, dim3((unsigned)((total + 255) / 256)), dim3(256), 0, (hipStream_t)stream, w,
            (uint16_t*)packed, Cout, Cin, kind, cin_phys / 8, nchunk, total);
  return cp_check_launch();
}

extern "C" int cp_hr_fuse_out(cp_stream_t stream, const void* src, int B, int H, int W, int cin_phys, int nconv,
                              const CpFuseConv* convs) {
  if (!src || !convs || B <= 0 || nconv <= 0 || nconv > FO_MAXCONV) return CP_ERR_INVALID;
  if (!cp_hr_fuse_out_supported(H, W, cin_phys)) return CP_ERR_INVALID;
  if (!cp_aligned16(src)) return CP_ERR_ALIGN;
  FuseOutParams p;
  p.src = src; p.B = B; p.H = H; p.W = W; p.Cg = cin_phys / 8; p.nconv = nconv;
  int band = 2;
  for (int cand = 2; cand <= H; cand += 2)
    if (H % cand == 0 && (size_t)(cand + 1) * (W + 1) * p.Cg * 16 + 16 * p.Cg <= 60 * 1024) band = cand;
  p.band = band;
  p.plane_bytes = (band + 1) * (W + 1) * 16 + 16;
  for (int i = 0; i < nconv; ++i) {
    const CpFuseConv& c = convs[i];
    if (!c.packed_w || !c.affine || !c.out || (c.kind != 0 && c.kind != 1) || c.out_cphys <= 0 || c.out_cphys % 8 || c.out_cphys > FO_AFF) return CP_ERR_INVALID;
    if (!cp_aligned16(c.packed_w) || !cp_aligned16(c.affine) || !cp_aligned16(c.out)) return CP_ERR_ALIGN;
    if (c.out == src) return CP_ERR_INVALID;
    FuseConvDev& d = p.c[i];
    d.w = c.packed_w; d.aff = c.affine; d.out = c.out; d.kind = c.kind; d.relu = c.relu ? 1 : 0;
    d.mt = fo_mt(c.out_cphys); d.nchunk = fo_nchunk(cin_phys, c.kind); d.out_cp = c.out_cphys; d.aff_n = d.mt * 16;
  }
  const size_t lds = (size_t)p.Cg * p.plane_bytes + 2 * FO_SLOTS * 4 + (size_t)FO_MAXCONV * 2 * FO_AFF * 4 + FO_MAXCONV * 8 * 4;
  const long long grid = (long long)B * (H / band);
  if (grid >= (1LL << 31)) return CP_ERR_RANGE;
  CP_LAUNCH(hr_fuse_out_kernel, dim3((unsigned)grid), dim3(FO_THREADS), lds, (hipStream_t)stream, p);
  return cp_check_launch();
}
```

checkerpose_amd/engine.py:

```python
import ctypes as C
import os

import torch

from . import _abi
from ._abi import ACT_LEAKY, ACT_NONE, ACT_RELU, CP_BF16, CP_F16, CP_F32, CpChainTail, CpChainTailConv, CpConvDesc, CpFuseConv

_TORCH_DT = {CP_F32: torch.float32, CP_BF16: torch.bfloat16}
USE_HALO = os.environ.get("CHECKERPOSE_AMD_HALO", "1") != "0"
USE_FUSED_BN = os.environ.get("CHECKERPOSE_AMD_FUSED_BN", "1") != "0"
USE_FUSED_BB = os.environ.get("CHECKERPOSE_AMD_FUSED_BB", "1") != "0"
USE_GEMM = os.environ.get("CHECKERPOSE_AMD_GEMM", "1") != "0"
USE_CHAIN = os.environ.get("CHECKERPOSE_AMD_CHAIN", "1") != "0"
USE_UP_FUSED = os.environ.get("CHECKERPOSE_AMD_UP_FUSED", "1") != "0"
USE_FUSE_OUT = os.environ.get("CHECKERPOSE_AMD_FUSE_OUT", "1") != "0"
USE_S2_SMALL = os.environ.get("CHECKERPOSE_AMD_S2_SMALL", "1") != "0"
USE_SEG_FUSED = os.environ.get("CHECKERPOSE_AMD_SEG_FUSED", "1") != "0"
USE_HALO2 = os.environ.get("CHECKERPOSE_AMD_HALO2", "1") != "0"
USE_CHAIN_TAILS = os.environ.get("CHECKERPOSE_AMD_CHAIN_TAILS", "1") != "0"
USE_CHAIN_TAIL = os.environ.get("CHECKERPOSE_AMD_CHAIN_TAIL", "1") != "0"
FUSE_OUT_MIN_BATCH = int(os.environ.get("CHECKERPOSE_AMD_FUSE_OUT_MIN_BATCH", "1"))
USE_MLP_FUSED = os.environ.get("CHECKERPOSE_AMD_MLP_FUSED", "1") != "0"
MLP_FUSED_MIN_ROWS = int(os.environ.get("CHECKERPOSE_AMD_MLP_FUSED_MIN_ROWS", "1"))
EDGE_SCHED = os.environ.get("CHECKERPOSE_AMD_EDGE_SCHED", "1") != "0"
USE_SPLITK = os.environ.get("CHECKERPOSE_AMD_SPLITK", "1") != "0"
GEMM_WS_SMALL_K = os.environ.get("CHECKERPOSE_AMD_GEMM_WS_SMALL_K", "1") != "0"
USE_MLP_GATHER = os.environ.get("CHECKERPOSE_AMD_MLP_GATHER", "1") != "0"
USE_PATCH_GATHER = os.environ.get("CHECKERPOSE_AMD_PATCH_GATHER", "1") != "0"
USE_STEM = os.environ.get("CHECKERPOSE_AMD_STEM", "1") != "0"
STEM_MIN_BATCH = int(os.environ.get("CHECKERPOSE_AMD_STEM_MIN_BATCH", "96"))
USE_EDGE_FUSED = os.environ.get("CHECKERPOSE_AMD_EDGE_FUSED", "1") != "0"
USE_GNN_F16 = os.environ.get("CHECKERPOSE_AMD_GNN_F16", "1") != "0"
USE_EDGE_TILED = os.environ.get("CHECKERPOSE_AMD_EDGE_TILED", "1") != "0"
EDGE_FUSED_MIN_BATCH = int(os.environ.get("CHECKERPOSE_AMD_EDGE_FUSED_MIN_BATCH", "96"))
CHAIN_MIN_BATCH = int(os.environ.get("CHECKERPOSE_AMD_CHAIN_MIN_BATCH", "40"))
NO_RECYCLE = os.environ.get("CHECKERPOSE_AMD_NO_RECYCLE", "0") == "1"
DTYPES = {"fp32": CP_F32, "f32": CP_F32, "float32": CP_F32, "bf16": CP_BF16, "bfloat16": CP_BF16}


class _ConvLog(list):

    def __init__(self, prog):
        super().__init__()
        self.prog, self.op_index = prog, []

    def append(self, e):
        super().append(e)
        self.op_index.append(len(self.prog.ops) - 1)


def _rup(x, m):
    return (x + m - 1) // m * m


class TBuf:
    __slots__ = ("nbytes", "offset", "first", "last", "fixed")

    def __init__(self, nbytes):
        self.nbytes, self.offset, self.first, self.last, self.fixed = _rup(nbytes, 256), None, None, None, None


class Act:
    __slots__ = ("tbuf", "B", "H", "W", "C", "Cphys", "cstride", "coff")

    def __init__(self, tbuf, B, H, W, C, Cphys, cstride, coff):
        self.tbuf, self.B, self.H, self.W, self.C, self.Cphys, self.cstride, self.coff = tbuf, B, H, W, C, Cphys, cstride, coff

    def slice(self, coff, C, Cphys=None):
        return Act(self.tbuf, self.B, self.H, self.W, C, Cphys if Cphys is not None else C, self.cstride, self.coff + coff)


class WeightStore:

    def __init__(self, lib, sd, dtype, device):
        self.lib, self.sd, self.dtype, self.device = lib, sd, dtype, device
        self.E = lib.cp_chan_align(dtype)
        self.cache = {}
        self.keep = []
        self.repacks_every_step = False

    def _w(self, key):
        t = self.sd[key]
        if t.device != self.device or t.dtype != torch.float32:
            raise RuntimeError("parameter %s must be an fp32 tensor on %s" % (key, self.device))
        return t.detach().contiguous()

    def pack(self, name, w, Cout, Cin, R, S, cin_phys, cout_rows, transposed=0, phase=0, row_map=None, dtype=None):
        dtype = self.dtype if dtype is None else dtype
        ck = (name, cin_phys, cout_rows, transposed, phase) + (() if dtype == self.dtype else (dtype,))
# ... 351 lines not shown
        sw, sb = self.ws.cache[ck]
        out = self.act(x.H, x.W, wCout)
        d = CpConvDesc()
        d.dtype, d.out_f32 = self.dtype, 0
        d.B, d.H, d.W = x.B, x.H, x.W
        d.Cin, d.in_cstride, d.in_coff = x.Cphys, x.cstride, x.coff
        d.R, d.S, d.stride, d.pad, d.Ho, d.Wo = 3, 3, 1, 1, x.H, x.W
        d.act, d.slope, d.Cout = act, slope, out.Cphys
        d.o_base, d.o_sb, d.o_sy, d.o_sx, d.o_sc = out.coff, out.H * out.W * out.cstride, out.W * out.cstride, out.cstride, 1
        self.keep += [d, packed, sc, sh, sw, sb]
        fn = self.lib.cp_conv3x3_halo_seg
        dref = C.byref(d)
        pw, ps, pt, psw, psb = packed.data_ptr(), sc.data_ptr(), sh.data_ptr(), sw.data_ptr(), sb.data_ptr()
        xtb, otb = x.tbuf, out.tbuf
        self._add(fn, lambda P: (dref, P(xtb), pw, ps, pt, P(otb), psw, psb, S, P(seg_tbuf)), "conv3x3_halo4:" + wkey, [xtb], [otb, seg_tbuf])
        fl = 2 * x.B * x.H * x.W * 9 * wCin * wCout
        self.flops += fl
        nbytes = x.B * x.H * x.W * (wCin + wCout) * self.es + 9 * wCin * wCout * self.es
        self.conv_log.append((wkey, x.B * x.H * x.W, wCout, 9 * wCin, fl, "conv3x3_halo4", nbytes))
        return out

    def can_fuse_basicblock(self, x: Act, C_):
        return (USE_FUSED_BB and C_ <= 32 and x.Cphys <= 4 * self.E and x.W >= 16 and x.H >= 8 and x.C == C_)

    def basicblock_fused(self, x: Act, k1, w1, s1, t1, k2, w2, s2, t2):
        C_ = w1.shape[0]
        pw1 = self.ws.pack_rows3x3(k1, w1, C_, C_, x.Cphys)
        pw2 = self.ws.pack_halo(k2, w2, C_, C_, x.Cphys)
        a1 = self.ws.affine(k1 + "#0", s1, t1, C_)
        a2 = self.ws.affine(k2 + "#0", s2, t2, C_)
        out = self.act(x.H, x.W, C_)
        d = CpConvDesc()
        d.dtype, d.out_f32, d.B, d.H, d.W = self.dtype, 0, x.B, x.H, x.W
        d.Cin, d.in_cstride, d.in_coff = x.Cphys, x.cstride, x.coff
        d.R, d.S, d.stride, d.pad, d.Ho, d.Wo = 3, 3, 1, 1, x.H, x.W
        d.Cout, d.act, d.slope = out.Cphys, ACT_RELU, 0.0
        d.o_base, d.o_sb, d.o_sy, d.o_sx, d.o_sc = out.coff, out.H * out.W * out.cstride, out.W * out.cstride, out.cstride, 1
        self.keep += [d, pw1, pw2, a1, a2]
        fn = self.lib.cp_basicblock_fused
        dref = C.byref(d)
        ptrs = (pw1.data_ptr(), a1[0].data_ptr(), a1[1].data_ptr(), pw2.data_ptr(), a2[0].data_ptr(), a2[1].data_ptr())
        xtb, otb = x.tbuf, out.tbuf
        self._add(fn, lambda P: (dref, P(xtb)) + ptrs + (P(otb),), "basicblock_fused:" + k1, [xtb], [otb])
        fl = 2 * x.B * x.H * x.W * 9 * C_ * C_
        nb = x.B * x.H * x.W * C_ * self.es
        self.flops += 2 * fl
        self.conv_log.append((k1, x.B * x.H * x.W, C_, 9 * C_, 2 * fl, "basicblock_fused", 2 * nb + 2 * 9 * C_ * C_ * self.es))
        return out

    def can_fuse_stem(self, size):
        return USE_STEM and self.dtype == CP_BF16 and self.B >= self.stem_min and size % 64 == 0

    def hr_stem(self, img_t, size, k1, w1, s1, t1, k2, w2, s2, t2):
        ck = ("stem", k1)
        if ck not in self.ws.cache:
            p1 = torch.empty(self.lib.cp_hr_stem_weight_bytes(0), dtype=torch.uint8, device=self.device)
            p2 = torch.empty(self.lib.cp_hr_stem_weight_bytes(1), dtype=torch.uint8, device=self.device)
            w1c, w2c = w1.contiguous(), w2.contiguous()
            self.ws.keep += [w1c, w2c]
            st = torch.cuda.current_stream(self.device).cuda_stream
            _abi.check(self.lib.cp_pack_hr_stem_weights(st, w1c.data_ptr(), w2c.data_ptr(), p1.data_ptr(), p2.data_ptr()), "cp_pack_hr_stem_weights")
            self.ws.cache[ck] = (p1, p2)
        p1, p2 = self.ws.cache[ck]
        a1, a2 = self.ws.affine(k1 + "#0", s1, t1, 64), self.ws.affine(k2 + "#0", s2, t2, 64)
        out = self.act(size // 4, size // 4, 64)
        self.keep += [p1, p2, a1, a2]
        fn = self.lib.cp_hr_stem
        ip = img_t.data_ptr()
        ot = out.tbuf
        args = (p1.data_ptr(), a1[0].data_ptr(), a1[1].data_ptr(), p2.data_ptr(), a2[0].data_ptr(), a2[1].data_ptr())
        self._add(fn, lambda P: (ip, self.B, size, size) + args + (P(ot),), "hr_stem:" + k1, [], [ot])
        fl = 2 * self.B * ((size // 2) ** 2 * 64 * 27 + (size // 4) ** 2 * 64 * 576)
        self.flops += fl
        self.conv_log.append((k1, self.B * (size // 4) ** 2, 64, 576, fl, "hr_stem", self.B * (3 * size * size * 4 + (size // 4) ** 2 * 64 * 2)))
        return out

    def can_chain(self, C_, H, W):
        return (USE_CHAIN and self.dtype == CP_BF16 and self.B >= self.chain_min and bool(self.lib.cp_hr_chain_supported(C_, H, W)))

    def can_chain_tail(self, C_, H, W, convs):
        return (USE_CHAIN_TAIL and self.can_chain(C_, H, W) and 1 <= len(convs) <= 3 and bool(self.lib.cp_hr_chain_tail_supported(C_, H, W))
                and sum(_rup(c[1].shape[0], self.E) for c in convs) <= self.lib.cp_hr_chain_tail_channels())

    def hr_chain(self, name, srcs, shifts, relu_in, ws, affs, C_, H, W, tail=None):
        blob, aff = self.ws.pack_chain(name, ws, affs, C_, H, W)
        out = self.act(H, W, C_)
        if tail is not None:
            return self._hr_chain_tail(name, srcs, shifts, relu_in, blob, aff, out, C_, H, W, tail)
        n = len(srcs)
        arr_p = (C.c_void_p * 4)()
        arr_s = (C.c_int32 * 4)(*([int(v) for v in shifts] + [0] * (4 - n)))
        self.keep += [arr_p, arr_s, blob, aff]
        for s_, sh in zip(srcs, shifts):
            assert s_.coff == 0 and s_.cstride == s_.Cphys == out.Cphys and (s_.H << sh, s_.W << sh) == (H, W)
        tbs = [s_.tbuf for s_ in srcs]
        ot = out.tbuf
        fn = self.lib.cp_hr_branch_chain
        bp, ap = blob.data_ptr(), aff.data_ptr()

        def argb(P):
            for i, t in enumerate(tbs):
                arr_p[i] = P(t)
            return (self.B, C_, H, W, n, arr_p, arr_s, 1 if relu_in else 0, bp, ap, P(ot))

        self._add(fn, argb, "hr_chain:" + name, tbs, [ot])
        fl = 8 * 2 * self.B * H * W * 9 * C_ * C_
        self.flops += fl
        nb = self.B * H * W * C_ * self.es
        self.conv_log.append((name, self.B * H * W, C_, 9 * C_, fl, "hr_chain", (n + 1) * nb + 8 * 9 * C_ * C_ * self.es))
        return out

    def can_chain_tails(self, C_, H, W, convs):
        return (USE_CHAIN_TAILS and self.can_chain(C_, H, W) and 1 <= len(convs) <= 3 and
                all(bool(self.lib.cp_hr_chain_tailconv_supported(C_, H, W, 1 if c[4] == 3 else 0, int(c[1].shape[0]))) for c in convs))

    def hr_chain_tails(self, name, srcs, shifts, relu_in, ws, affs, C_, H, W, convs):
        lib = self.lib
        blob, aff = self.ws.pack_chain(name, ws, affs, C_, H, W)
        out = self.act(H, W, C_)
        arr = (CpChainTailConv * len(convs))()
        touts, keep, fl_t, nb_t = [], [], 0, 0
        for i, (wkey, w, scale, shift, k, relu) in enumerate(convs):
            kind = 1 if k == 3 else 0
            Cout = int(w.shape[0])
            ck = ("chain_tailconv", wkey)
            if ck not in self.ws.cache:
                buf = torch.empty(lib.cp_hr_chain_tailconv_weight_bytes(C_, H, W, kind, Cout), dtype=torch.uint8, device=self.device)
                wc = w.contiguous()
                sc = scale.to(device=self.device, dtype=torch.float32).contiguous()
                self.ws.keep += [wc, sc]
                st = torch.cuda.current_stream(self.device).cuda_stream
                _abi.check(lib.cp_pack_hr_chain_tailconv_weight(st, wc.data_ptr(), sc.data_ptr(), C_, H, W, kind, Cout, buf.data_ptr()),
                           "cp_pack_hr_chain_tailconv_weight(%s)" % wkey)
                sh = torch.zeros(_rup(Cout, 16), dtype=torch.float32, device=self.device)
                sh[:Cout] = shift
                self.ws.cache[ck] = (buf, sh)
            buf, sh = self.ws.cache[ck]
            o = self.act(H >> kind, W >> kind, Cout)
            assert o.coff == 0 and o.cstride == o.Cphys
            arr[i].packed_w, arr[i].shift = buf.data_ptr(), sh.data_ptr()
            arr[i].kind, arr[i].Cout, arr[i].out_cphys, arr[i].relu = kind, Cout, o.Cphys, 1 if relu else 0
            touts.append(o)
            keep += [buf, sh]
            fl_t += 2 * self.B * o.H * o.W * k * k * C_ * Cout
            nb_t += self.B * o.H * o.W * Cout * self.es + k * k * C_ * Cout * self.es
        n = len(srcs)
        arr_p = (C.c_void_p * 4)()
        arr_s = (C.c_int32 * 4)(*([int(v) for v in shifts] + [0] * (4 - n)))
        self.keep += [arr_p, arr_s, blob, aff, arr] + keep
        for s_, sh_ in zip(srcs, shifts):
            assert s_.coff == 0 and s_.cstride == s_.Cphys == out.Cphys and (s_.H << sh_, s_.W << sh_) == (H, W)
        tbs, ot, tts = [s_.tbuf for s_ in srcs], out.tbuf, [o.tbuf for o in touts]
        bp, ap = blob.data_ptr(), aff.data_ptr()

        def argb(P):
            for i, t in enumerate(tbs):
                arr_p[i] = P(t)
            for i, t in enumerate(tts):
                arr[i].out = P(t)
            return (self.B, C_, H, W, n, arr_p, arr_s, 1 if relu_in else 0, bp, ap, P(ot), len(convs), arr)

        self._add(lib.cp_hr_branch_chain_tails, argb, "hr_chain:" + name, tbs, [ot] + tts)
        fl = 8 * 2 * self.B * H * W * 9 * C_ * C_ + fl_t
        self.flops += fl
        nb = self.B * H * W * C_ * self.es
        self.conv_log.append((name, self.B * H * W, C_, 9 * C_, fl, "hr_chain", (n + 1) * nb + 8 * 9 * C_ * C_ * self.es + nb_t))
        return out, touts

    def _hr_chain_tail(self, name, srcs, shifts, relu_in, blob, aff, out, C_, H, W, tail):
        lib = self.lib
        ck = ("chain_tail", name)
        if ck not in self.ws.cache:
            tb = torch.zeros(lib.cp_hr_chain_tail_weight_bytes(), dtype=torch.uint8, device=self.device)
            tsh = torch.zeros(lib.cp_hr_chain_tail_channels(), dtype=torch.float32, device=self.device)
            st = torch.cuda.current_stream(self.device).cuda_stream
            piece = 0
            for wkey, w, scale, shift, relu in tail:
                Cout = w.shape[0]
                cph = _rup(Cout, self.E)
                wc = w.contiguous()
                sc = scale.to(device=self.device, dtype=torch.float32).contiguous()
                self.ws.keep += [wc, sc]
                _abi.check(lib.cp_pack_hr_chain_tail_weight(st, wc.data_ptr(), sc.data_ptr(), Cout, piece, cph, tb.data_ptr()),
                           "cp_pack_hr_chain_tail_weight(%s)" % wkey)
                tsh[piece * 8: piece * 8 + Cout] = shift
                piece += cph // 8
            self.ws.cache[ck] = (tb, tsh)
        tb, tsh = self.ws.cache[ck]
        touts = [self.act(H >> 1, W >> 1, w.shape[0]) for _, w, *_ in tail]
        tl = CpChainTail()
        tl.packed_w, tl.shift, tl.nconv = tb.data_ptr(), tsh.data_ptr(), len(tail)
        for i, ((wkey, w, scale, shift, relu), o) in enumerate(zip(tail, touts)):
            assert o.coff == 0 and o.cstride == o.Cphys
            tl.Cout[i], tl.out_cphys[i], tl.relu[i] = w.shape[0], o.Cphys, 1 if relu else 0
        n = len(srcs)
        arr_p = (C.c_void_p * 4)()
        arr_s = (C.c_int32 * 4)(*([int(v) for v in shifts] + [0] * (4 - n)))
        self.keep += [arr_p, arr_s, blob, aff, tb, tsh, tl]
        for s_, sh in zip(srcs, shifts):
            assert s_.coff == 0 and s_.cstride == s_.Cphys == out.Cphys and (s_.H << sh, s_.W << sh) == (H, W)
        tbs, ot, tts = [s_.tbuf for s_ in srcs], out.tbuf, [o.tbuf for o in touts]
        bp, ap = blob.data_ptr(), aff.data_ptr()

        def argb(P):
            for i, t in enumerate(tbs):
                arr_p[i] = P(t)
            for i, t in enumerate(tts):
                tl.out[i] = P(t)
            return (self.B, C_, H, W, n, arr_p, arr_s, 1 if relu_in else 0, bp, ap, P(ot), C.byref(tl))

        self._add(lib.cp_hr_branch_chain_tail, argb, "hr_chain:" + name, tbs, [ot] + tts)
        fl = 8 * 2 * self.B * H * W * 9 * C_ * C_ + sum(2 * self.B * (H >> 1) * (W >> 1) * 9 * C_ * w.shape[0] for _, w, *_ in tail)
        self.flops += fl
        nb = self.B * H * W * C_ * self.es
        nbt = sum(self.B * (H >> 1) * (W >> 1) * w.shape[0] * self.es + 9 * C_ * w.shape[0] * self.es for _, w, *_ in tail)
        self.conv_log.append((name, self.B * H * W, C_, 9 * C_, fl, "hr_chain", (n + 1) * nb + 8 * 9 * C_ * C_ * self.es + nbt))
        return out, touts

    def can_fuse_out(self, x: Act, couts=()):
        return (USE_FUSE_OUT and self.dtype == CP_BF16 and self.B >= self.fuse_out_min and x.coff == 0 and x.cstride == x.Cphys
                and bool(self.lib.cp_hr_fuse_out_supported(x.H, x.W, x.Cphys))
                and all(self.lib.cp_hr_fuse_out_affine_floats(_rup(int(c), self.E)) > 0 for c in couts))

    def hr_fuse_out(self, x: Act, convs):
        assert 1 <= len(convs) <= 4
        arr = (CpFuseConv * len(convs))()
        outs, keep, fl, nbytes = [], [], 0, x.B * x.H * x.W * x.C * self.es
        for i, (wkey, w, scale, shift, k, relu) in enumerate(convs):
            kind = 1 if k == 3 else 0
            Cout, Cin = w.shape[0], w.shape[1]
            assert Cin == x.C and w.shape[2] == k
            out = self.act(x.H >> kind, x.W >> kind, Cout)
            ck = ("fuse_out", wkey)
            if ck not in self.ws.cache:
                buf = torch.empty(self.lib.cp_hr_fuse_out_weight_bytes(x.Cphys, out.Cphys, kind), dtype=torch.uint8, device=self.device)
                wc = w.contiguous()
                self.ws.keep.append(wc)
                st = torch.cuda.current_stream(self.device).cuda_stream
                _abi.check(self.lib.cp_pack_hr_fuse_out_weight(st, wc.data_ptr(), Cout, Cin, x.Cphys, out.Cphys, kind, buf.data_ptr()),
                           "cp_pack_hr_fuse_out_weight")
                n = self.lib.cp_hr_fuse_out_affine_floats(out.Cphys)
                aff = torch.zeros(2, n, dtype=torch.float32, device=self.device)
                aff[0, :Cout] = scale
                aff[1, :Cout] = shift
                self.ws.cache[ck] = (buf, aff)
            buf, aff = self.ws.cache[ck]
            keep += [buf, aff]
            arr[i].packed_w, arr[i].affine = buf.data_ptr(), aff.data_ptr()
            arr[i].kind, arr[i].Cout, arr[i].out_cphys, arr[i].relu = kind, Cout, out.Cphys, 1 if relu else 0
            outs.append(out)
            fl += 2 * x.B * out.H * out.W * k * k * Cin * Cout
            nbytes += x.B * out.H * out.W * Cout * self.es + k * k * Cin * Cout * self.es
        self.keep += keep + [arr]
        fn = self.lib.cp_hr_fuse_out
        xt, ots = x.tbuf, [o.tbuf for o in outs]

        def argb(P):
            for i, t in enumerate(ots):
                arr[i].out = P(t)
            return (P(xt), x.B, x.H, x.W, x.Cphys, len(convs), arr)

        name = convs[0][0]
        self._add(fn, argb, "hr_fuse_out:" + name, [xt], ots)
        self.flops += fl
        self.conv_log.append((name, x.B * x.H * x.W, sum(c[1].shape[0] for c in convs), x.C, fl, "hr_fuse_out", nbytes))
        return outs

    def can_fuse_bottleneck(self, x: Act, planes, cout, has_ds):
        cin = 64 if has_ds else 256
        return (USE_FUSED_BN and self.dtype == CP_BF16 and x.C == cin and x.Cphys == cin and planes == 64 and cout == 256
                and x.B * x.H * x.W * x.cstride * 2 < (1 << 31))

    def bottleneck_fused(self, x: Act, keys, ws, affs, out: Act = None):
        has_ds = len(keys) == 4
        cin = x.C
        pw = [self.ws.pack(keys[0], ws[0], 64, cin, 1, 1, cin, 64), self.ws.pack(keys[1], ws[1], 64, 64, 3, 3, 64, 64),
              self.ws.pack(keys[2], ws[2], 256, 64, 1, 1, 64, 256)]
        if has_ds:
            pw.append(self.ws.pack(keys[3], ws[3], 256, 64, 1, 1, 64, 256))
        af = [self.ws.affine(keys[i] + "#0", affs[i][0], affs[i][1], (64, 64, 256, 256)[i]) for i in range(len(keys))]
        if out is None:
            out = self.act(x.H, x.W, 256)
        d = CpConvDesc()
        d.dtype, d.out_f32, d.B, d.H, d.W = self.dtype, 0, x.B, x.H, x.W
        d.Cin, d.in_cstride, d.in_coff = cin, x.cstride, x.coff
        d.R, d.S, d.stride, d.pad, d.Ho, d.Wo = 3, 3, 1, 1, x.H, x.W
        d.Cout, d.act, d.slope = 256, ACT_RELU, 0.0
        d.o_base, d.o_sb, d.o_sy, d.o_sx, d.o_sc = out.coff, out.H * out.W * out.cstride, out.W * out.cstride, out.cstride, 1
        self.keep += [d] + pw + af
        fn = self.lib.cp_bottleneck_fused
        dref = C.byref(d)
        ptrs = ()
        for i in range(len(keys)):
            ptrs += (pw[i].data_ptr(), af[i][0].data_ptr(), af[i][1].data_ptr())
        if not has_ds:
            ptrs += (None, None, None)
        xtb, otb = x.tbuf, out.tbuf
        self._add(fn, lambda P: (dref, P(xtb)) + ptrs + (P(otb),), "bottleneck_fused:" + keys[0], [xtb], [otb])
        npx = x.B * x.H * x.W
# ... 510 lines not shown
```

checkerpose_amd/netbuilder.py:

```python
import os

import torch

from ._abi import ACT_LEAKY, ACT_NONE, ACT_RELU
from .engine import Act, Program, _rup

from .model.backbone import HRNET_CFGS
IMG_FEATS_DIMS = {"resnet34": [64, 128, 256, 512], "hrnet_w18": [128, 256, 512, 1024], "hrnet_w18_small": [128, 256, 512, 1024],
                  "hrnet_w30": [128, 256, 512, 1024]}


FUSE_OUT_DEEP = os.environ.get("CHECKERPOSE_AMD_FUSE_OUT_DEEP", "1") != "0"


DECODER_SPLITK = os.environ.get("CHECKERPOSE_AMD_DECODER_SPLITK", "1") != "0"
HEAD_ON_REFINE_LANE = os.environ.get("CHECKERPOSE_AMD_HEAD_LANE", "1") != "0"
FUSE_SAME_LANE = os.environ.get("CHECKERPOSE_AMD_FUSE_SAME_LANE", "1") != "0"


class NetEmitter:
    def __init__(self, prog: Program, sd):
        self.p, self.ws, self.sd = prog, prog.ws, sd
        self.ones = {}
        self.tp = prog if getattr(prog, "training", False) else None
# ... 159 lines not shown
        if self.tp is not None and not kw:
            return self._linear_train(x, key, act, slope, out)
        w = self.W(key + ".weight")
        w4 = w.reshape(w.shape[0], w.shape[1], 1, 1)
        b = self.W(key + ".bias")
        return self.p.conv(x, key, w4, self._unit(w.shape[0]), b, 1, 1, 1, 0, w.shape[0], act, slope, out=out, **kw)

    def basic_block(self, pfx, x, stride=1):
        w1 = self.W(pfx + ".conv1.weight")
        if (self.tp is None and stride == 1 and (pfx + ".downsample.0.weight") not in self.sd and w1.shape[0] == w1.shape[1]
                and self.p.can_fuse_basicblock(x, w1.shape[0])):
            s1, t1 = self.ws.bn_fold(pfx + ".bn1")
            s2, t2 = self.ws.bn_fold(pfx + ".bn2")
            return self.p.basicblock_fused(x, pfx + ".conv1", w1, s1, t1, pfx + ".conv2", self.W(pfx + ".conv2.weight"), s2, t2)
        y = self.conv_bn(x, pfx + ".conv1", pfx + ".bn1", 3, stride, 1)
        sc = x
        if (pfx + ".downsample.0.weight") in self.sd:
            sc = self.conv_bn(x, pfx + ".downsample.0", pfx + ".downsample.1", 1, stride, 0, relu=False)
        return self.conv_bn(y, pfx + ".conv2", pfx + ".bn2", 3, 1, 1, relu=True, residual=sc)

    def bottleneck(self, pfx, x, out=None):
        w1, w3 = self.W(pfx + ".conv1.weight"), self.W(pfx + ".conv3.weight")
        has_ds = (pfx + ".downsample.0.weight") in self.sd
        if (self.tp is None and self.p.can_fuse_bottleneck(x, w1.shape[0], w3.shape[0], has_ds) and w1.shape[1] == x.C
                and (has_ds or w1.shape[1] == w3.shape[0])):
            keys = [pfx + ".conv%d" % i for i in (1, 2, 3)]
            affs = [self.ws.bn_fold(pfx + ".bn%d" % i) for i in (1, 2, 3)]
            ws = [w1, self.W(pfx + ".conv2.weight"), w3]
            if has_ds:
                wd = self.W(pfx + ".downsample.0.weight")
                if tuple(wd.shape[2:]) != (1, 1) or wd.shape[0] != 256:
                    has_ds = None
                else:
                    keys.append(pfx + ".downsample.0")
                    affs.append(self.ws.bn_fold(pfx + ".downsample.1"))
                    ws.append(wd)
            if has_ds is not None:
                return self.p.bottleneck_fused(x, keys, ws, affs, out=out)
        y = self.conv_bn(x, pfx + ".conv1", pfx + ".bn1", 1, 1, 0)
        y = self.conv_bn(y, pfx + ".conv2", pfx + ".bn2", 3, 1, 1)
        sc = x
        if (pfx + ".downsample.0.weight") in self.sd:
            sc = self.conv_bn(x, pfx + ".downsample.0", pfx + ".downsample.1", 1, 1, 0, relu=False, out=None)
        return self.conv_bn(y, pfx + ".conv3", pfx + ".bn3", 1, 1, 0, relu=True, residual=sc, out=out)

    def _fuse_chain_rest(self, a, convs):
        for ck, bk, relu in convs:
            if FUSE_OUT_DEEP and self.p.can_fuse_out(a, [self.W(ck + ".weight").shape[0]]):
                a = self.p.hr_fuse_out(a, [(ck, self.W(ck + ".weight")) + tuple(self.ws.bn_fold(bk)) + (3, relu)])[0]
            else:
                a = self.conv_bn(a, ck, bk, 3, 2, 1, relu=relu)
        return a

    def _materialize(self, x, out=None):
        if isinstance(x, Act):
            assert out is None
            return x
        terms, shifts = x
        if out is None:
            out = self.p.act(terms[0].H << shifts[0], terms[0].W << shifts[0], terms[0].C)
        return self.p.fuse_sum(terms, shifts, out, relu=True)

    def bottleneck_incre(self, pfx, cat: Act, planes, out=None):
        x = cat.slice(planes, cat.C - planes, _rup(cat.C - planes, self.p.E))
        y = self.conv_bn(x, pfx + ".conv1", pfx + ".bn1", 1, 1, 0)
        self.conv_bn(y, pfx + ".conv2", pfx + ".bn2", 3, 1, 1, out=cat.slice(0, planes))
        ck = pfx + ".conv3#merged"
        if ck not in self.ws.cache:
            s3, t3 = self.ws.bn_fold(pfx + ".bn3")
            sd, td = self.ws.bn_fold(pfx + ".downsample.1")
            w3, wd = self.W(pfx + ".conv3.weight"), self.W(pfx + ".downsample.0.weight")
            self.ws.cache[ck] = (torch.cat([w3 * s3.view(-1, 1, 1, 1), wd * sd.view(-1, 1, 1, 1)], dim=1).contiguous(), t3 + td)
        wm, shift = self.ws.cache[ck]
        return self.p.conv(cat, ck, wm, self._unit(wm.shape[0]), shift, 1, 1, 1, 0, wm.shape[0], ACT_RELU, out=out)

    def hr_module(self, pfx, xs, lazy=False, nblocks=4):
        if self.tp is not None:
            return self._hr_module_train(pfx, xs, nblocks)
        nb = len(xs)
        xs = list(xs)
        p = self.p
        terms = [[None] * nb for _ in range(nb)]
        first = {}
        p.par_begin(nb)
        for j in range(nb):
            p.set_lane(j)
            if isinstance(xs[j], Act):
                C_, H, W = xs[j].C, xs[j].H, xs[j].W
            else:
                t0, sh0 = xs[j][0][0], xs[j][1][0]
                C_, H, W = t0.C, t0.H << sh0, t0.W << sh0
            if nblocks == 4 and p.can_chain(C_, H, W):
                srcs, shifts = ([xs[j]], [0]) if isinstance(xs[j], Act) else xs[j]
                bp = "%s.branches.%d" % (pfx, j)
                ws = [self.W("%s.%d.conv%d.weight" % (bp, k, c)) for k in range(4) for c in (1, 2)]
                affs = [self.ws.bn_fold("%s.%d.bn%d" % (bp, k, c)) for k in range(4) for c in (1, 2)]
                tl = [("%s.fuse_layers.%d.%d.0.0" % (pfx, i, j), "%s.fuse_layers.%d.%d.0.1" % (pfx, i, j), i - j > 1) for i in range(j + 1, nb)]
                tconvs = [(ck, self.W(ck + ".weight")) + tuple(self.ws.bn_fold(bk)) + (relu,) for ck, bk, relu in tl]
                if tl and all(i > j for i in range(nb) if i != j) and p.can_chain_tail(C_, H, W, tconvs):
                    xs[j], touts = p.hr_chain(bp, srcs, shifts, not isinstance(xs[j], Act), ws, affs, C_, H, W, tail=tconvs)
                    for i, o in zip(range(j + 1, nb), touts):
                        first[(i, j)] = o
                    continue
                lst_t = []
                for i in range(nb):
                    q = "%s.fuse_layers.%d.%d" % (pfx, i, j)
                    if j > i:
                        lst_t.append((i, q + ".0", q + ".1", 1, False))
                    elif j < i:
                        lst_t.append((i, q + ".0.0", q + ".0.1", 3, i - j > 1))
                tcv = [(ck, self.W(ck + ".weight")) + tuple(self.ws.bn_fold(bk)) + (k, relu) for (_, ck, bk, k, relu) in lst_t]
                if nb > 1 and p.can_chain_tails(C_, H, W, tcv):
                    xs[j], touts = p.hr_chain_tails(bp, srcs, shifts, not isinstance(xs[j], Act), ws, affs, C_, H, W, tcv)
                    for (i, _, _, _, _), o in zip(lst_t, touts):
                        first[(i, j)] = o
                    continue
                xs[j] = p.hr_chain(bp, srcs, shifts, not isinstance(xs[j], Act), ws, affs, C_, H, W)
            else:
                xs[j] = self._materialize(xs[j])
                for k in range(nblocks):
                    xs[j] = self.basic_block("%s.branches.%d.%d" % (pfx, j, k), xs[j])
            lst = []
            for i in range(nb):
                q = "%s.fuse_layers.%d.%d" % (pfx, i, j)
                if j > i:
                    lst.append((i, q + ".0", q + ".1", 1, False))
                elif j < i:
                    lst.append((i, q + ".0.0", q + ".0.1", 3, i - j > 1))
            if nb > 1 and p.can_fuse_out(xs[j], [self.W(ck + ".weight").shape[0] for (_, ck, _, _, _) in lst]):
                outs = p.hr_fuse_out(xs[j], [(ck, self.W(ck + ".weight")) + tuple(self.ws.bn_fold(bk)) + (k, relu)
                                             for (_, ck, bk, k, relu) in lst])
                for (i, _, _, _, _), o in zip(lst, outs):
                    first[(i, j)] = o
        def cost_of(i, j):
            if (i, j) in first:
                return max(i - j - 1, 0)
            return (i - j) if j < i else 0.3
        load = [0.0] * nb
        sched = []
        same_lane = FUSE_SAME_LANE and len(first) == nb * (nb - 1)
        for cost, i, j in sorted([(cost_of(i, j), i, j) for i in range(nb) for j in range(nb) if i != j], reverse=True):
            if same_lane:
                ln = j
            else:
                ln = min(range(nb), key=lambda k: load[k]) if cost > 0 else 0
            load[ln] += cost
            sched.append((ln, i, j))
        second = any(c > 0 for c in load) and not same_lane
        if second:
            p.par_end()
            p.par_begin(nb)
        for i in range(nb):
            terms[i][i] = xs[i]
        for ln, i, j in sched:
            p.set_lane(ln)
            q = "%s.fuse_layers.%d.%d" % (pfx, i, j)
            if (i, j) in first:
                t = self._fuse_chain_rest(first[(i, j)], [("%s.%d.0" % (q, k), "%s.%d.1" % (q, k), k != i - j - 1) for k in range(1, i - j)])
            elif j > i:
                t = self.conv_bn(xs[j], q + ".0", q + ".1", 1, 1, 0, relu=False)
            else:
                t = xs[j]
                for k in range(i - j):
                    t = self.conv_bn(t, "%s.%d.0" % (q, k), "%s.%d.1" % (q, k), 3, 2, 1, relu=(k != i - j - 1))
            terms[i][j] = t
        p.par_end()
        if lazy:
            return [(terms[i], [max(j - i, 0) for j in range(nb)]) for i in range(nb)]
        outs = []
        p.par_begin(nb)
        for i in range(nb):
            p.set_lane(i)
            out = p.act(xs[i].H, xs[i].W, xs[i].C)
            shifts = [max(j - i, 0) for j in range(nb)]
            outs.append(p.fuse_sum(terms[i], shifts, out, relu=True))
        p.par_end()
        return outs

    def hrnet(self, pfx, x, feat_outs=None, stem_done=False, name="hrnet_w18"):
        hcfg = HRNET_CFGS[name]
        stages = [("stage%d" % (si + 2),) + tuple(st) for si, st in enumerate(hcfg["stages"])]
        if not stem_done:
            x = self.conv_bn(x, pfx + "conv1", pfx + "bn1", 3, 2, 1)
            x = self.conv_bn(x, pfx + "conv2", pfx + "bn2", 3, 2, 1)
        for k in range(hcfg["layer1"][0]):
            x = self.bottleneck("%slayer1.%d" % (pfx, k), x)
        if self.tp is None:
            self.p.par_begin(2)
            xs = [self.conv_bn(x, pfx + "transition1.0.0", pfx + "transition1.0.1", 3, 1, 1)]
            self.p.set_lane(1)
            xs.append(self.conv_bn(x, pfx + "transition1.1.0.0", pfx + "transition1.1.0.1", 3, 2, 1))
            self.p.par_end()
        else:
            xs = [self.conv_bn(x, pfx + "transition1.0.0", pfx + "transition1.0.1", 3, 1, 1),
                  self.conv_bn(x, pfx + "transition1.1.0.0", pfx + "transition1.1.0.1", 3, 2, 1)]
        for si, (stage, nmod, nblk, chans) in enumerate(stages):
            if si > 0:
                t = "%stransition%d.%d.0" % (pfx, si + 1, len(chans) - 1)
                xs = xs + [self.conv_bn(xs[-1], t + ".0", t + ".1", 3, 2, 1)]
            last_stage = si == len(stages) - 1
            for m in range(nmod):
                xs = self.hr_module("%s%s.%d" % (pfx, stage, m), xs, lazy=(m + 1 < nmod) or (last_stage and self.tp is None), nblocks=nblk)
        feats = []
        self.p.par_begin(len(xs))
        for i, f in enumerate(xs):
            self.p.set_lane(i)
            q = "%sincre_modules.%d.0" % (pfx, i)
            if isinstance(f, Act):
                feats.append(self.bottleneck(q, f, out=(feat_outs[i] if feat_outs else None)))
            else:
                terms, shifts = f
                planes = self.W(q + ".conv1.weight").shape[0]
                cat = self.p.act(terms[0].H << shifts[0], terms[0].W << shifts[0], planes + terms[0].C)
                self._materialize(f, out=cat.slice(planes, terms[0].C, _rup(terms[0].C, self.p.E)))
                feats.append(self.bottleneck_incre(q, cat, planes, out=(feat_outs[i] if feat_outs else None)))
        self.p.par_end()
        return feats

    def resnet34(self, pfx, x, feat_outs=None):
        x = self.conv_bn(x, pfx + "conv1", pfx + "bn1", 7, 2, 3)
        x0 = x
        x = self.p.maxpool(x0)
        if self.tp is not None:
            tp, xo = self.tp, x

            def bwd_pool():
                if xo.tbuf in tp.grads:
                    tp.maxpool_bwd(x0, tp.grad_of(xo), tp.grad_of(x0))
            tp.tape.append(bwd_pool)
        feats = []
        for li, nblk in enumerate((3, 4, 6, 3)):
            for k in range(nblk):
                x = self.basic_block("%slayer%d.%d" % (pfx, li + 1, k), x, stride=2 if (k == 0 and li > 0) else 1)
            feats.append(x)
        return feats

    def _edgeconv_train(self, pfx, x, graph, slope, out):
        tp = self.tp
        w = self.W(pfx + ".conv.0.weight")
        Co, Cc = w.shape[0], w.shape[1] // 2
# ... 521 lines not shown
```

include/checkerpose_hip.h:

```cpp
#ifndef CHECKERPOSE_HIP_H
#define CHECKERPOSE_HIP_H

#include <stddef.h>
#include <stdint.h>

#ifdef __cplusplus
extern "C" {
#endif

typedef void* cp_stream_t;

enum { CP_F32 = 0, CP_BF16 = 1, CP_F16 = 2 };
enum { CP_ACT_NONE = 0, CP_ACT_RELU = 1, CP_ACT_LEAKY = 2 };
enum { CP_LOSS_BCE = 0, CP_LOSS_L1 = 1 };
enum {
  CP_OK = 0,
  CP_ERR_INVALID = -1,
  CP_ERR_HIP = -2,
  CP_ERR_ALIGN = -3,
  CP_ERR_RANGE = -4
};

int cp_version(void);
const char* cp_strerror(int code);
// ... 102 lines not shown
  const void* patches;
  const int32_t* x_id;
  const int32_t* y_id;
  const float* mask;
  const void* zeros;
  int32_t p_cstride, p_coff, Hp, Wp, k;
} CpI2fGather;
int cp_mlp_pair_fused_gather_supported(int Cg, int E_ch, int k);
int cp_mlp_pair_fused_gather(cp_stream_t stream, const CpI2fGather* g, const void* gin, int gin_cstride, int gin_coff, int Cg, int B, int N,
                             const void* packed_w1, const float* bias1, float slope1, const void* packed_w2, const float* bias2,
                             float slope2, void* out, int out_cstride, int out_coff);
int cp_mlp_pair_fused_gather_t(cp_stream_t stream, int dtype, const CpI2fGather* g, const void* gin, int gin_cstride, int gin_coff, int Cg,
                               int B, int N, const void* packed_w1, const float* bias1, float slope1, const void* packed_w2,
                               const float* bias2, float slope2, void* out, int out_cstride, int out_coff);

int cp_upsample2x_bilinear_ac(cp_stream_t stream, int dtype, const void* in, void* out, int B, int H, int W,
                              int C, int in_cstride, int in_coff, int out_cstride, int out_coff);

int cp_fuse_sum_act(cp_stream_t stream, int dtype, int nsrc, const void* const* srcs, const int32_t* shifts,
                    void* out, int B, int H, int W, int C, int relu, int out_cstride, int out_coff);

int cp_maxpool3x3s2(cp_stream_t stream, int dtype, const void* in, void* out, int B, int H, int W, int C);

int cp_edgeconv_gather_max(cp_stream_t stream, int dtype, const void* pq, const int32_t* idx,
                           const int32_t* graph_ids, void* out, int B, int N, int K, int C, int G,
                           int out_cstride, int out_coff, float slope);

int cp_index2feat_gather(cp_stream_t stream, int dtype, const void* patches, const int32_t* x_id,
                         const int32_t* y_id, const float* mask, void* out, int B, int N, int Hp, int Wp,
                         int E, int k, int out_cstride, int out_coff);

size_t cp_hr_stem_weight_bytes(int which);
int cp_pack_hr_stem_weights(cp_stream_t stream, const float* w1, const float* w2, void* packed1, void* packed2);
int cp_hr_stem(cp_stream_t stream, const float* img_nchw, int B, int Hin, int Win, const void* packed1, const float* scale1,
               const float* shift1, const void* packed2, const float* scale2, const float* shift2, void* out);

int cp_hr_chain_supported(int C, int H, int W);
size_t cp_hr_chain_weight_bytes(int C, int H, int W);
int cp_hr_chain_affine_floats(int C, int H, int W);
int cp_pack_hr_chain_weight(cp_stream_t stream, const float* w, const float* scale, int C, int H, int W, int conv_index, void* blob);
int cp_hr_branch_chain(cp_stream_t stream, int B, int C, int H, int W, int nsrc, const void* const* srcs,
                       const int32_t* shifts, int relu_in, const void* packed_w, const float* affine, void* out);

typedef struct CpChainTail {
  const void* packed_w;
  const float* shift;
  void* out[3];
  int32_t nconv;
  int32_t Cout[3], out_cphys[3], relu[3];
} CpChainTail;
int cp_hr_chain_tail_supported(int C, int H, int W);
size_t cp_hr_chain_tail_weight_bytes(void);
int cp_hr_chain_tail_channels(void);
int cp_pack_hr_chain_tail_weight(cp_stream_t stream, const float* w, const float* scale, int Cout, int first_piece, int out_cphys, void* blob);
int cp_hr_branch_chain_tail(cp_stream_t stream, int B, int C, int H, int W, int nsrc, const void* const* srcs,
                            const int32_t* shifts, int relu_in, const void* packed_w, const float* affine, void* out,
                            const CpChainTail* tail);

typedef struct {
  const void* packed_w;
  const float* shift;
  void* out;
  int32_t kind, Cout, out_cphys, relu;
} CpChainTailConv;
int cp_hr_chain_tailconv_supported(int C, int H, int W, int kind, int Cout);
size_t cp_hr_chain_tailconv_weight_bytes(int C, int H, int W, int kind, int Cout);
int cp_pack_hr_chain_tailconv_weight(cp_stream_t stream, const float* w, const float* scale, int C, int H, int W, int kind, int Cout,
                                     void* packed);
int cp_hr_branch_chain_tails(cp_stream_t stream, int B, int C, int H, int W, int nsrc, const void* const* srcs, const int32_t* shifts,
                             int relu_in, const void* packed_w, const float* affine, void* out, int ntail, const CpChainTailConv* convs);

typedef struct CpFuseConv {
  const void* packed_w;
  const float* affine;
  void* out;
  int32_t kind, Cout, out_cphys, relu;
} CpFuseConv;
int cp_hr_fuse_out_supported(int H, int W, int cin_phys);
size_t cp_hr_fuse_out_weight_bytes(int cin_phys, int out_cphys, int kind);
int cp_hr_fuse_out_affine_floats(int out_cphys);
int cp_pack_hr_fuse_out_weight(cp_stream_t stream, const float* w, int Cout, int Cin, int cin_phys, int out_cphys, int kind,
                               void* packed);
int cp_hr_fuse_out(cp_stream_t stream, const void* src, int B, int H, int W, int cin_phys, int nconv, const CpFuseConv* convs);

int cp_edgeconv_fused_supported(int N, int K, int Cin, int Cout);
size_t cp_edgeconv_fused_weight_bytes(int Cin, int Cout);
int cp_pack_edgeconv_fused_weight(cp_stream_t stream, const float* wpq, int Cin, int Cout, void* packed);
int cp_edgeconv_fused(cp_stream_t stream, const void* x, int in_cstride, int in_coff, const void* packed_w,
                      const float* scale, const float* shift, const int32_t* idx, const int32_t* graph_ids, void* out,
                      int out_cstride, int out_coff, int B, int N, int K, int Cin, int Cout, int G, float slope);
int cp_pack_edgeconv_fused_weight_t(cp_stream_t stream, int dtype, const float* wpq, int Cin, int Cout, void* packed);
int cp_edgeconv_fused_t(cp_stream_t stream, int dtype, const void* x, int in_cstride, int in_coff, const void* packed_w,
                        const float* scale, const float* shift, const int32_t* idx, const int32_t* graph_ids, void* out,
                        int out_cstride, int out_coff, int B, int N, int K, int Cin, int Cout, int G, float slope);

int cp_edgeconv_tiled_supported(int N, int K, int Cin, int Cout, int HPAD);
size_t cp_edgeconv_tiled_weight_bytes(int Cin, int Cout);
size_t cp_edgeconv_tiled_table_bytes(int B, int N, int Cout);
int cp_pack_edgeconv_tiled_weight(cp_stream_t stream, const float* wpq, int Cin, int Cout, void* packed);
int cp_edgeconv_tiled(cp_stream_t stream, const void* x, int in_cstride, int in_coff, const void* packed_w_fused,
                      const void* packed_w_q, const float* scale, const float* shift, const int32_t* halo,
                      const int16_t* nbr, const int32_t* graph_ids, void* key_table, void* out, int out_cstride, int out_coff,
                      int B, int N, int K, int Cin, int Cout, int G, int HPAD, float slope);
int cp_pack_edgeconv_tiled_weight_t(cp_stream_t stream, int dtype, const float* wpq, int Cin, int Cout, void* packed);
int cp_edgeconv_tiled_t(cp_stream_t stream, int dtype, const void* x, int in_cstride, int in_coff, const void* packed_w_fused,
                        const void* packed_w_q, const float* scale, const float* shift, const int32_t* halo, const int16_t* nbr,
                        const int32_t* graph_ids, void* key_table, void* out, int out_cstride, int out_coff, int B, int N, int K,
                        int Cin, int Cout, int G, int HPAD, float slope);
int cp_permute_rows(cp_stream_t stream, const void* in, void* out, const int32_t* perm, const int32_t* graph_ids, int B, int N,
                    int row_bytes);
int cp_permute_cols(cp_stream_t stream, const void* in, void* out, const int32_t* perm, const int32_t* graph_ids, int B, int R,
                    int N, int elem_bytes, int scatter);

int cp_index2feat_conv_supported(int Cin, int E_ch, int k);
size_t cp_index2feat_conv_weight_bytes(void);
int cp_pack_index2feat_conv_weight(cp_stream_t stream, const float* w, void* packed);
int cp_index2feat_conv(cp_stream_t stream, const void* f, int in_cstride, int in_coff, const void* packed_w, const float* bias,
                       const int32_t* x_id, const int32_t* y_id, const float* mask, void* out, int B, int N, int H, int W, int k,
                       int out_cstride, int out_coff);
int cp_index2feat_conv_t(cp_stream_t stream, int out_dtype, const void* f, int in_cstride, int in_coff, const void* packed_w,
                         const float* bias, const int32_t* x_id, const int32_t* y_id, const float* mask, void* out, int B, int N,
                         int H, int W, int k, int out_cstride, int out_coff);

#define CP_SIGMOID_HALF_Z0_BITS 0x33C00000u
int cp_bits_decode(cp_stream_t stream, const float* bits, int stage, float* mask, int32_t* x_id,
                   int32_t* y_id, int64_t* x_id64, int64_t* y_id64, int B, int N);
int cp_code_decode(cp_stream_t stream, const float* bits, int rows, int r, int64_t* x_id64, int64_t* y_id64, int32_t* x_id32,
                   int32_t* y_id32, int B, int N);

int cp_correspondences(cp_stream_t stream, const float* bits, const float* seg, const int64_t* x_id, const int64_t* y_id,
                       const float* roi_xy_ori, float* p2d, uint8_t* valid, int32_t* count, int B, int N, int H, int W,
                       int discard_bd_pixel);
int cp_correspondences_bbox(cp_stream_t stream, const float* bits, const float* seg, const int64_t* x_id, const int64_t* y_id,
                            const int32_t* final_bbox, float* p2d, uint8_t* valid, int32_t* count, int B, int N, int H, int W,
                            int discard_bd_pixel);

size_t cp_pnp_ransac_scratch_bytes(int B, int N);
int cp_pnp_ransac(cp_stream_t stream, const float* p3d, long long p3d_bstride, const float* p2d, const uint8_t* valid,
                  int valid_stride, const float* cam_K, long long K_bstride, int B, int N, float reproj_threshold,
                  int iterations, uint32_t seed, double* pose, uint8_t* inliers, int32_t* status, void* scratch);

enum { CP_POSE_ERR_ADD = 1, CP_POSE_ERR_ADI = 2 };
size_t cp_pose_errors_scratch_bytes(int B, int Vmax);
int cp_pose_errors(cp_stream_t stream, const double* pose_est, const double* pose_gt, const float* verts, const int32_t* offsets,
                   int M, const int32_t* mesh_id, int B, int Vmax, int kinds, double* add, double* adi, void* scratch);

int cp_encode_targets(cp_stream_t stream, const double* p3d, long long p3d_bstride, const int32_t* obj_ids, int n_obj,
                      const double* cam_K, long long K_bstride, const double* R, const double* t, const int32_t* boxes,
                      const int32_t* boxes_host, const uint8_t* no_detection_host, int B, int N, int S, float* roi_mask_bit,
                      float* pixel_x_code, float* pixel_y_code, int32_t* x_id, int32_t* y_id, double* proj_xy, double* depth);

int cp_code_report(cp_stream_t stream, const float* pred_roi, long long roi_bstride, const float* pred_x, long long x_bstride,
                   const float* pred_y, long long y_bstride, int nb, const float* seg, int H, int W, const float* gt_roi,
                   const float* gt_x, const float* gt_y, int bits, const void* mask_visib, const void* mask_full, int mask_f32, int S,
                   int B, int N, int32_t* counts, double* figures);


size_t cp_edgeconv_bwd_workspace_bytes(int B, int N, int C);
int cp_edgeconv_gather_max_bwd(cp_stream_t stream, int dtype, const void* pq, const int32_t* idx,
                               const int32_t* rev_ptr, const int32_t* rev_edge, const int32_t* graph_ids,
                               const float* gout, float* dpq, void* workspace, int B, int N, int K, int C,
                               int G, int gout_cstride, int gout_coff, float slope);

int cp_index2feat_gather_bwd(cp_stream_t stream, const float* gout, const int32_t* x_id, const int32_t* y_id,
                             const float* mask, float* dpatches, int B, int N, int Hp, int Wp, int E, int k,
                             int gout_cstride, int gout_coff);
// ... 194 lines not shown
```

Before: 26490 crops/s.

## Fuse deeper stride-2 fuse-layer convs into HR branch chain kernel tails

Adds a 'deep' stage to the HRNet branch-chain kernels. After the tail convs run, the same kernel runs up to three more stride-2 3x3 downsampling convs from the fuse layers (the multi-hop i-j>1 paths), reusing the block's LDS through a shared fo_run_deep helper. The net builder now marks these paths as fully computed, so the separate fuse-chain-rest launches and the scheduling cost for them go away. This removes kernel launches and intermediate round trips, but serializes the extra convs inside blocks sized for the chain work, which may underuse the GPU on small downsampled maps.

```diff
diff --git a/checkerpose_amd/_abi.py b/checkerpose_amd/_abi.py
--- a/checkerpose_amd/_abi.py
+++ b/checkerpose_amd/_abi.py
@@ -30,6 +30,11 @@
 class CpChainTailConv(C.Structure):
     _fields_ = [("packed_w", C.c_void_p), ("shift", C.c_void_p), ("out", C.c_void_p),
                 ("kind", C.c_int32), ("Cout", C.c_int32), ("out_cphys", C.c_int32), ("relu", C.c_int32)]
+
+
+class CpChainDeep(C.Structure):
+    _fields_ = [("src", C.c_void_p), ("packed_w", C.c_void_p), ("affine", C.c_void_p), ("out", C.c_void_p),
+                ("H", C.c_int32), ("W", C.c_int32), ("cin_phys", C.c_int32), ("Cout", C.c_int32), ("out_cphys", C.c_int32), ("relu", C.c_int32)]
 
 
 class CpI2fGather(C.Structure):
@@ -157,6 +162,11 @@
     "cp_fuse_sum_act": (_I, [_P, _I, _I, C.POINTER(_P), C.POINTER(C.c_int32), _P, _I, _I, _I, _I, _I, _I, _I]),
     "cp_maxpool3x3s2": (_I, [_P, _I, _P, _P, _I, _I, _I, _I]),
     "cp_edgeconv_gather_max": (_I, [_P, _I, _P, _P, _P, _P, _I, _I, _I, _I, _I, _I, _I, _F]),
+    "cp_hr_chain_deep_supported": (_I, [_I, _I, _I, _I, _I, _I, _I]),
+    "cp_hr_branch_chain_tail_deep": (_I, [_P, _I, _I, _I, _I, _I, C.POINTER(_P), C.POINTER(C.c_int32), _I, _P, _P, _P, C.POINTER(CpChainTail),
+                                          _I, C.POINTER(CpChainDeep)]),
+    "cp_hr_branch_chain_tails_deep": (_I, [_P, _I, _I, _I, _I, _I, C.POINTER(_P), C.POINTER(C.c_int32), _I, _P, _P, _P, _I, C.POINTER(CpChainTailConv),
+                                           _I, C.POINTER(CpChainDeep)]),
     "cp_hr_fuse_out_supported": (_I, [_I, _I, _I]),
     "cp_hr_fuse_out_weight_bytes": (C.c_size_t, [_I, _I, _I]),
     "cp_hr_fuse_out_affine_floats": (_I, [_I]),
diff --git a/checkerpose_amd/csrc/hr_chain.hip b/checkerpose_amd/csrc/hr_chain.hip
--- a/checkerpose_amd/csrc/hr_chain.hip
+++ b/checkerpose_amd/csrc/hr_chain.hip
@@ -1,12 +1,13 @@
 #include <stdlib.h>
 
-#include "common.h"
+#include "hr_fuse_dev.h"
 
 size_t cp_chain0_conv_bytes();
 int cp_chain0_aff();
 int cp_chain0_pack(hipStream_t st, const float* w, const float* scale, int conv_index, void* blob);
 int cp_chain0_launch(hipStream_t st, int B, int nsrc, const void* const* srcs, const int32_t* shifts, int relu_in,
-                     const void* packed_w, const float* affine, void* out, const CpChainTail* tail);
+                     const void* packed_w, const float* affine, void* out, const CpChainTail* tail, int ndeep, const CpChainDeep* deep);
+size_t cp_chain0_deep_lds();
 size_t cp_chain0_tail_bytes();
 int cp_chain0_tail_channels();
 int cp_chain0_tail_pack(hipStream_t st, const float* w, const float* scale, int Cout, int first_piece, int out_cphys, void* blob);
@@ -74,6 +75,8 @@
   int dbg;
   int ntail;
   ChainTailConv tc[3];
+  int ndeep;
+  ChainDeepDev deep[CHAIN_MAXDEEP];
 };
 
 #ifdef CP_DEBUG_KNOBS
@@ -442,6 +445,14 @@
     }
   }
   if constexpr (TAIL) chain_tails<Cfg>(p, sMap, lane, wave, crop0);
+  if constexpr (TAIL && CPW == 1 && Cfg::C == 36) {
+#pragma unroll 1
+    for (int i = 0; i < p.ndeep; ++i) {
+      const ChainDeepDev d = p.deep[i];
+      __syncthreads();
+      if (crop0 < p.B) fo_run_deep<NTHR>(d, smem, crop0, p.B);
+    }
+  }
 }
 
 __global__ void pack_chain_tail_kernel(const float* __restrict__ w, const float* __restrict__ scale, uint16_t* __restrict__ out, int Cin,
@@ -555,7 +566,7 @@
 
 static int branch_chain(cp_stream_t stream, int B, int C, int H, int W, int nsrc, const void* const* srcs, const int32_t* shifts, int relu_in,
                         const void* packed_w, const float* affine, void* out, const CpChainTail* tail, int ntail = 0,
-                        const CpChainTailConv* tconvs = nullptr);
+                        const CpChainTailConv* tconvs = nullptr, int ndeep = 0, const CpChainDeep* deep = nullptr);
 
 extern "C" int cp_hr_chain_tailconv_supported(int C, int H, int W, int kind, int Cout) {
   ChainInfo ci;
@@ -583,6 +594,22 @@
   return branch_chain(stream, B, C, H, W, nsrc, srcs, shifts, relu_in, packed_w, affine, out, nullptr, ntail, convs);
 }
 
+extern "C" int cp_hr_branch_chain_tails_deep(cp_stream_t stream, int B, int C, int H, int W, int nsrc, const void* const* srcs,
+                                             const int32_t* shifts, int relu_in, const void* packed_w, const float* affine, void* out, int ntail,
+                                             const CpChainTailConv* convs, int ndeep, const CpChainDeep* deep) {
+  if (ntail < 1 || ntail > 3 || !convs || C != CfgB1::C || ndeep < 1 || ndeep > CHAIN_MAXDEEP || !deep) return CP_ERR_INVALID;
+  return branch_chain(stream, B, C, H, W, nsrc, srcs, shifts, relu_in, packed_w, affine, out, nullptr, ntail, convs, ndeep, deep);
+}
+
+extern "C" int cp_hr_chain_deep_supported(int C, int H, int W, int src_H, int src_W, int cin_phys, int out_cphys) {
+  ChainInfo ci;
+  if (!chain_info(C, H, W, &ci) || (C != 18 && C != CfgB1::C)) return 0;
+  if (src_H < 2 || src_W < 2 || (src_H & 1) || (src_W & 1) || cin_phys <= 0 || cin_phys % 8 || out_cphys <= 0 || out_cphys % 8 || out_cphys > FO_AFF) return 0;
+  if (9 * (cin_phys / 8) + 3 > FO_SLOTS) return 0;
+  const size_t lds = C == 18 ? cp_chain0_deep_lds() : (size_t)CfgB1::LDS;
+  return fo_lds_bytes(cin_phys / 8, fo_plane_bytes(src_H, src_W)) <= lds ? 1 : 0;
+}
+
 extern "C" int cp_hr_branch_chain(cp_stream_t stream, int B, int C, int H, int W, int nsrc, const void* const* srcs,
                                   const int32_t* shifts, int relu_in, const void* packed_w, const float* affine, void* out) {
   return branch_chain(stream, B, C, H, W, nsrc, srcs, shifts, relu_in, packed_w, affine, out, nullptr);
@@ -595,8 +622,16 @@
   return branch_chain(stream, B, C, H, W, nsrc, srcs, shifts, relu_in, packed_w, affine, out, tail);
 }
 
+extern "C" int cp_hr_branch_chain_tail_deep(cp_stream_t stream, int B, int C, int H, int W, int nsrc, const void* const* srcs,
+                                            const int32_t* shifts, int relu_in, const void* packed_w, const float* affine, void* out,
+                                            const CpChainTail* tail, int ndeep, const CpChainDeep* deep) {
+  if (!tail || !cp_hr_chain_tail_supported(C, H, W) || ndeep < 1 || ndeep > CHAIN_MAXDEEP || !deep) return CP_ERR_INVALID;
+  return branch_chain(stream, B, C, H, W, nsrc, srcs, shifts, relu_in, packed_w, affine, out, tail, 0, nullptr, ndeep, deep);
+}
+
 static int branch_chain(cp_stream_t stream, int B, int C, int H, int W, int nsrc, const void* const* srcs, const int32_t* shifts, int relu_in,
-                        const void* packed_w, const float* affine, void* out, const CpChainTail* tail, int ntail, const CpChainTailConv* tconvs) {
+                        const void* packed_w, const float* affine, void* out, const CpChainTail* tail, int ntail, const CpChainTailConv* tconvs,
+                        int ndeep, const CpChainDeep* deep) {
   ChainInfo ci;
   if (B <= 0 || !srcs || !shifts || nsrc < 1 || nsrc > 4 || !packed_w || !affine || !out) return CP_ERR_INVALID;
   if (!chain_info(C, H, W, &ci)) return CP_ERR_INVALID;
@@ -609,7 +644,7 @@
     if (srcs[k] == out) return CP_ERR_INVALID;
     p.src[k] = srcs[k]; p.shift[k] = shifts[k];
   }
-  if (C == 18) return cp_chain0_launch((hipStream_t)stream, B, nsrc, srcs, shifts, relu_in, packed_w, affine, out, tail);
+  if (C == 18) return cp_chain0_launch((hipStream_t)stream, B, nsrc, srcs, shifts, relu_in, packed_w, affine, out, tail, ndeep, deep);
   p.nsrc = nsrc; p.relu_in = relu_in ? 1 : 0;
   p.w = packed_w; p.aff = affine; p.out = out; p.B = B;
   p.dbg = cp_knob("CP_CHAIN_DBG") ? atoi(cp_knob("CP_CHAIN_DBG")) : 0;
@@ -624,6 +659,13 @@
     p.tc[i].kind = c.kind; p.tc[i].nt = nt; p.tc[i].out_cp = c.out_cphys; p.tc[i].relu = c.relu ? 1 : 0;
   }
   p.ntail = ntail;
+  p.ndeep = 0;
+  if (ndeep > 0) {
+    if (C != CfgB1::C || ntail < 1) return CP_ERR_INVALID;
+    const int rc = fo_deep_fill(ndeep, deep, out, (size_t)CfgB1::LDS, p.deep);
+    if (rc != CP_OK) return rc;
+    p.ndeep = ndeep;
+  }
   hipStream_t st = (hipStream_t)stream;
   if (C == CfgB1::C) return launch_chain<CfgB1>(st, p);
   if (C == CfgB2::C) return B >= CHAIN_CPW_FULL_B ? launch_chain<CfgB2>(st, p) : launch_chain<CfgB2m>(st, p);
diff --git a/checkerpose_amd/csrc/hr_chain0.hip b/checkerpose_amd/csrc/hr_chain0.hip
--- a/checkerpose_amd/csrc/hr_chain0.hip
+++ b/checkerpose_amd/csrc/hr_chain0.hip
@@ -1,4 +1,4 @@
-#include "common.h"
+#include "hr_fuse_dev.h"
 
 namespace {
 
@@ -26,6 +26,8 @@
   void* tout[3];
   uint32_t* status;
   int dbg_spin_limit;
+  int ndeep;
+  ChainDeepDev deep[CHAIN_MAXDEEP];
 };
 constexpr int ZTAIL_CH = 96;
 
@@ -545,8 +547,7 @@
       case 3: p_stage_and_tail<3>(p, smem, lane, b, wave - 8); break;
       default: p_stage_and_tail<4>(p, smem, lane, b, wave - 8); break;
     }
-    return;
-  }
+  } else {
 
 #ifdef CP_C0_PLAIN_MAP
   const int s = wave;
@@ -676,6 +677,14 @@
     Z_MARK(5);
   }
   Z_DUMP();
+  __builtin_amdgcn_s_setprio(0);
+  }
+#pragma unroll 1
+  for (int i = 0; i < p.ndeep; ++i) {
+    const ChainDeepDev d = p.deep[i];
+    __syncthreads();
+    fo_run_deep<PNT>(d, smem, b, p.B);
+  }
 }
 __global__ void pack_chain0_weight_kernel(const float* __restrict__ w, const float* __restrict__ scale, uint16_t* __restrict__ out, size_t total) {
   const size_t i = (size_t)blockIdx.x * blockDim.x + threadIdx.x;
@@ -736,7 +745,7 @@
 }
 
 int cp_chain0_launch(hipStream_t st, int B, int nsrc, const void* const* srcs, const int32_t* shifts, int relu_in,
-                     const void* packed_w, const float* affine, void* out, const CpChainTail* tail) {
+                     const void* packed_w, const float* affine, void* out, const CpChainTail* tail, int ndeep, const CpChainDeep* deep) {
   static CpDeviceOnce once;
   const int dev = cp_current_device();
   CP_LDS_ATTR_ONCE(once, dev, cp_set_max_lds((const void*)hr_chain0_kernel, ZLDS));
@@ -760,6 +769,15 @@
     if (ps * 8 > ZTAIL_CH) return CP_ERR_INVALID;
     p.tnp = ps; p.tw = tail->packed_w; p.tshift = tail->shift;
   }
+  if (ndeep > 0) {
+#ifdef CP_C0_BAND
+    return CP_ERR_INVALID;
+#endif
+    if (!tail) return CP_ERR_INVALID;
+    const int rc = fo_deep_fill(ndeep, deep, out, (size_t)PLDS, p.deep);
+    if (rc != CP_OK) return rc;
+    p.ndeep = ndeep;
+  }
 #ifndef CP_C0_BAND
   {
     static CpDeviceOnce once_p;
@@ -772,6 +790,7 @@
   return cp_check_launch();
 }
 
+size_t cp_chain0_deep_lds() { return (size_t)PLDS; }
 size_t cp_chain0_tail_bytes() { return (size_t)(ZTAIL_CH / 32) * ZCONV_W; }
 int cp_chain0_tail_channels() { return ZTAIL_CH; }
 
diff --git a/checkerpose_amd/csrc/hr_fuse_dev.h b/checkerpose_amd/csrc/hr_fuse_dev.h
--- /dev/null
+++ b/checkerpose_amd/csrc/hr_fuse_dev.h
@@ -0,0 +1,255 @@
+#pragma once
+#include "common.h"
+
+namespace {
+
+constexpr int FO_MAXCONV = 4, FO_NTB = 8, FO_MTB = 3, FO_THREADS = 256, FO_SLOTS = 192, FO_WB = 8, FO_SU = 17, FO_AFF = 160;
+
+struct FuseConvDev {
+  const void* w; const float* aff; void* out;
+  int kind, relu, mt, nchunk, out_cp, aff_n;
+};
+struct FuseOutParams {
+  const void* src;
+  int B, H, W, Cg, band, nconv, plane_bytes;
+  FuseConvDev c[FO_MAXCONV];
+};
+
+__device__ __forceinline__ void mma16f(const u32x4& w, const u32x4& a, f32x4& acc) {
+  acc = __builtin_amdgcn_mfma_f32_16x16x32_bf16(__builtin_bit_cast(bf16x8, w), __builtin_bit_cast(bf16x8, a), acc, 0, 0, 0);
+}
+
+template <int NTHR, int MTB, int NTB, int WB, int SU>
+__device__ __forceinline__ void fo_run(const FuseOutParams& p, unsigned char* smem, int b, int r0) {
+  const int tid = threadIdx.x;
+  const int lane = tid & 63;
+  const int wave = __builtin_amdgcn_readfirstlane(tid >> 6);
+  const int x = lane & 15, q = lane >> 4;
+  const int RW = p.W + 1, RH = p.band + 1, Cg = p.Cg;
+  const int HE = (p.W >> 1) + 1;
+  auto colslot = [&](int rc) { return (rc & 1) ? HE + (rc >> 1) : (rc >> 1); };
+  const int planes_end = Cg * p.plane_bytes;
+  uint32_t* const tab = (uint32_t*)(smem + planes_end);
+
+  float* const saff = (float*)(tab + 2 * FO_SLOTS);
+  uint32_t* const sdesc = (uint32_t*)(saff + FO_MAXCONV * 2 * FO_AFF);
+  if (wave == NTHR / 64 - 1) {
+    for (int s = lane; s < 2 * FO_SLOTS; s += 64) {
+      const int kind = s >= FO_SLOTS, sl = s - kind * FO_SLOTS;
+      uint32_t off = 0u;
+      if (kind == 0) { if (sl < Cg) off = (uint32_t)(sl * p.plane_bytes); }
+      else if (sl < 9 * Cg) {
+        const int tap = sl / Cg, cg = sl - tap * Cg;
+        const int ts = tap % 3;
+        off = (uint32_t)(cg * p.plane_bytes + ((tap / 3) * RW + (ts == 1 ? HE : ts >> 1)) * 16);
+      }
+      tab[s] = off;
+    }
+#pragma unroll
+    for (int ci = 0; ci < FO_MAXCONV; ++ci) {
+      if (ci < p.nconv) {
+        const float* const ga = p.c[ci].aff;
+        const int an = p.c[ci].aff_n;
+        for (int r = lane; r < 2 * FO_AFF; r += 64) {
+          const int h = r >= FO_AFF, c = r - h * FO_AFF;
+          saff[ci * 2 * FO_AFF + r] = c < an ? ga[h * an + c] : 0.f;
+        }
+        if (lane == 0) {
+          const uint64_t wq = (uint64_t)p.c[ci].w, oq = (uint64_t)p.c[ci].out;
+          uint32_t* d = sdesc + ci * 8;
+          d[0] = (uint32_t)wq; d[1] = (uint32_t)(wq >> 32); d[2] = (uint32_t)oq; d[3] = (uint32_t)(oq >> 32);
+          d[4] = (uint32_t)(p.c[ci].kind | (p.c[ci].relu << 1)); d[5] = (uint32_t)p.c[ci].mt; d[6] = (uint32_t)p.c[ci].nchunk;
+          d[7] = (uint32_t)p.c[ci].out_cp;
+        }
+      }
+    }
+  }
+  const int nconv = p.nconv;
+  auto D = [&](int ci, int k) -> int { return __builtin_amdgcn_readfirstlane((int)sdesc[ci * 8 + k]); };
+  {
+    const int per_row = p.W * Cg;
+    const u32x4* src = (const u32x4*)p.src + ((size_t)b * p.H * p.W) * Cg;
+    if constexpr (SU == 0) {
+      const int total = RH * per_row;
+      for (int i0 = tid; i0 < total; i0 += 4 * NTHR) {
+        u32x4 v[4];
+#pragma unroll
+        for (int u = 0; u < 4; ++u) {
+          const int i = i0 + u * NTHR;
+          const int ry = i / per_row, pc = i - ry * per_row, gy = r0 - 1 + ry;
+          v[u] = u32x4{0u, 0u, 0u, 0u};
+          if (i < total && gy >= 0) v[u] = src[(size_t)gy * per_row + pc];
+        }
+#pragma unroll
+        for (int u = 0; u < 4; ++u) {
+          const int i = i0 + u * NTHR;
+          const int ry = i / per_row, pc = i - ry * per_row;
+          const int c = pc / Cg, cg = pc - c * Cg;
+          if (i < total) *(u32x4*)(smem + cg * p.plane_bytes + (ry * RW + colslot(c + 1)) * 16) = v[u];
+        }
+      }
+    } else
+    for (int pc = tid; pc < per_row; pc += NTHR) {
+      const int c = pc / Cg, cg = pc - c * Cg;
+      unsigned char* dst = smem + cg * p.plane_bytes + colslot(c + 1) * 16;
+#pragma unroll 1
+      for (int ry0 = 0; ry0 < RH; ry0 += SU) {
+        u32x4 v[SU > 0 ? SU : 1];
+#pragma unroll
+        for (int u = 0; u < SU; ++u) {
+          const int gy = r0 - 1 + ry0 + u;
+          v[u] = u32x4{0u, 0u, 0u, 0u};
+          if (ry0 + u < RH && gy >= 0) v[u] = src[(size_t)gy * per_row + pc];
+        }
+#pragma unroll
+        for (int u = 0; u < SU; ++u)
+          if (ry0 + u < RH) *(u32x4*)(dst + (ry0 + u) * RW * 16) = v[u];
+      }
+    }
+    for (int i = tid; i < RH * Cg; i += NTHR) {
+      const int ry = i / Cg, cg = i - ry * Cg;
+      *(u32x4*)(smem + cg * p.plane_bytes + (ry * RW) * 16) = u32x4{0u, 0u, 0u, 0u};
+    }
+  }
+  __syncthreads();
+
+  auto split = [&](int n, int Wo, int& oy, int& ox) {
+    if ((Wo & (Wo - 1)) == 0) { const int lw = 31 - __builtin_clz((unsigned)Wo); oy = n >> lw; ox = n & (Wo - 1); }
+    else { oy = n / Wo; ox = n - oy * Wo; }
+  };
+  auto geom = [&](int ci, int& Wo, int& npx, int& ntile, int& npg, int& nrg) {
+    const int kind = D(ci, 4) & 1;
+    Wo = kind ? p.W >> 1 : p.W;
+    npx = Wo * (kind ? p.band >> 1 : p.band);
+    ntile = (npx + 15) >> 4;
+    npg = (ntile + NTB - 1) / NTB;
+    nrg = (D(ci, 5) + MTB - 1) / MTB;
+  };
+#pragma unroll 1
+  for (int t0 = wave, ci = 0, tbase = 0; ci < nconv; ++ci) {
+    int Wo, npx, ntile, npg, nrg;
+    geom(ci, Wo, npx, ntile, npg, nrg);
+    const int kind = D(ci, 4) & 1, relu = D(ci, 4) >> 1, mtc = D(ci, 5), nch = D(ci, 6), out_cp = D(ci, 7);
+    const u32x4* const wbase = (const u32x4*)(((uint64_t)(uint32_t)D(ci, 1) << 32) | (uint32_t)D(ci, 0)) + lane;
+    uint16_t* const outp = (uint16_t*)(((uint64_t)(uint32_t)D(ci, 3) << 32) | (uint32_t)D(ci, 2));
+    const uint32_t* const tb = tab + (kind ? FO_SLOTS : 0);
+    const int Ho = kind ? p.H >> 1 : p.H, oy0 = kind ? r0 >> 1 : r0;
+    const int nitem = nrg * npg;
+#pragma unroll 1
+    for (; t0 < tbase + nitem; t0 += NTHR / 64) {
+      const int it = t0 - tbase;
+      const int rg = it / npg, pg = it - rg * npg;
+      const int mt0 = rg * MTB, nm = mtc - mt0 < MTB ? mtc - mt0 : MTB;
+      const int tlim = ntile - pg * NTB;
+      uint32_t base[NTB];
+      f32x4 acc[MTB][NTB];
+#pragma unroll
+      for (int i = 0; i < NTB; ++i) {
+        int n = (pg * NTB + i) * 16 + x;
+        if (n >= npx) n = 0;
+        int oy, ox;
+        split(n, Wo, oy, ox);
+        base[i] = kind ? (uint32_t)(((2 * oy) * RW + ox) * 16) : (uint32_t)(((oy + 1) * RW + colslot(ox + 1)) * 16);
+#pragma unroll
+        for (int m = 0; m < MTB; ++m) acc[m][i] = f32x4{0.f, 0.f, 0.f, 0.f};
+      }
+#pragma unroll 1
+      for (int kb = 0; kb < nch; kb += WB) {
+        u32x4 wf[MTB][WB];
+#pragma unroll
+        for (int m = 0; m < MTB; ++m)
+#pragma unroll
+          for (int k = 0; k < WB; ++k) {
+            wf[m][k] = u32x4{0u, 0u, 0u, 0u};
+            if (m < nm && kb + k < nch) wf[m][k] = wbase[(size_t)((mt0 + m) * nch + kb + k) * 64];
+          }
+#pragma unroll
+        for (int k = 0; k < WB; ++k) {
+          if (kb + k < nch) {
+            const uint32_t so = tb[(kb + k) * 4 + q];
+#pragma unroll
+            for (int i4 = 0; i4 < NTB; i4 += 4) {
+              if (i4 < tlim) {
+                u32x4 a[4];
+#pragma unroll
+                for (int i = 0; i < 4; ++i) a[i] = *(const u32x4*)(smem + base[i4 + i] + so);
+#pragma unroll
+                for (int m = 0; m < MTB; ++m)
+                  if (m < nm) {
+#pragma unroll
+                    for (int i = 0; i < 4; ++i) mma16f(wf[m][k], a[i], acc[m][i4 + i]);
+                  }
+              }
+            }
+          }
+        }
+      }
+#pragma unroll
+      for (int m = 0; m < MTB; ++m) {
+        const int co = (mt0 + m) * 16 + 4 * q;
+        if (m < nm && co < out_cp) {
+          const f32x4 sc = *(const f32x4*)(saff + ci * 2 * FO_AFF + co), sh = *(const f32x4*)(saff + ci * 2 * FO_AFF + FO_AFF + co);
+#pragma unroll
+          for (int i = 0; i < NTB; ++i) {
+            const int n = (pg * NTB + i) * 16 + x;
+            if (i < tlim && n < npx) {
+              int oy, ox;
+              split(n, Wo, oy, ox);
+              float v[4];
+#pragma unroll
+              for (int j = 0; j < 4; ++j) {
+                v[j] = acc[m][i][j] * sc[j] + sh[j];
+                if (relu) v[j] = fmaxf(v[j], 0.f);
+              }
+              u32x2 pk; pk.x = pack_bf16x2(v[0], v[1]); pk.y = pack_bf16x2(v[2], v[3]);
+              *(u32x2*)(outp + ((size_t)(b * Ho + oy0 + oy) * Wo + ox) * out_cp + co) = pk;
+            }
+          }
+        }
+      }
+    }
+    tbase += nitem;
+  }
+}
+
+struct ChainDeepDev {
+  const void* src; const void* w; const float* aff; void* out;
+  int H, W, Cg, relu, mt, nchunk, out_cp;
+};
+constexpr int CHAIN_MAXDEEP = 3;
+
+template <int NTHR>
+__device__ __forceinline__ void fo_run_deep(const ChainDeepDev& d, unsigned char* smem, int b, int B) {
+  FuseOutParams fp = {};
+  fp.src = d.src; fp.B = B; fp.H = d.H; fp.W = d.W; fp.Cg = d.Cg; fp.band = d.H; fp.nconv = 1;
+  fp.plane_bytes = (d.H + 1) * (d.W + 1) * 16 + 16;
+  fp.c[0].w = d.w; fp.c[0].aff = d.aff; fp.c[0].out = d.out; fp.c[0].kind = 1; fp.c[0].relu = d.relu;
+  fp.c[0].mt = d.mt; fp.c[0].nchunk = d.nchunk; fp.c[0].out_cp = d.out_cp; fp.c[0].aff_n = d.mt * 16;
+  fo_run<NTHR, 3, 2, 4, 0>(fp, smem, b, 0);
+}
+
+inline int fo_nchunk(int cin_phys, int kind) { return ((kind ? 9 : 1) * (cin_phys / 8) + 3) / 4; }
+inline int fo_mt(int out_cphys) { return (out_cphys + 15) / 16; }
+inline int fo_plane_bytes(int band, int W) { return (band + 1) * (W + 1) * 16 + 16; }
+inline size_t fo_lds_bytes(int Cg, int plane_bytes) { return (size_t)Cg * plane_bytes + 2 * FO_SLOTS * 4 + (size_t)FO_MAXCONV * 2 * FO_AFF * 4 + FO_MAXCONV * 8 * 4; }
+
+inline int fo_deep_fill(int ndeep, const CpChainDeep* deep, const void* chain_out, size_t lds_avail, ChainDeepDev* dev) {
+  if (ndeep < 0 || ndeep > CHAIN_MAXDEEP || (ndeep > 0 && !deep)) return CP_ERR_INVALID;
+  for (int i = 0; i < ndeep; ++i) {
+    const CpChainDeep& c = deep[i];
+    if (!c.src || !c.packed_w || !c.affine || !c.out || c.out == c.src || c.out == chain_out) return CP_ERR_INVALID;
+    if (c.H < 2 || c.W < 2 || (c.H & 1) || (c.W & 1) || c.cin_phys <= 0 || c.cin_phys % 8) return CP_ERR_INVALID;
+    if (c.out_cphys <= 0 || c.out_cphys % 8 || c.out_cphys > FO_AFF || c.Cout <= 0 || c.Cout > c.out_cphys) return CP_ERR_INVALID;
+    const int Cg = c.cin_phys / 8;
+    if (9 * Cg + 3 > FO_SLOTS || fo_lds_bytes(Cg, fo_plane_bytes(c.H, c.W)) > lds_avail) return CP_ERR_INVALID;
+    if (!cp_aligned16(c.src) || !cp_aligned16(c.packed_w) || !cp_aligned16(c.affine) || !cp_aligned16(c.out)) return CP_ERR_ALIGN;
+    for (int k = 0; k < i; ++k)
+      if (deep[k].out == c.out) return CP_ERR_INVALID;
+    ChainDeepDev& d = dev[i];
+    d.src = c.src; d.w = c.packed_w; d.aff = c.affine; d.out = c.out; d.H = c.H; d.W = c.W; d.Cg = Cg; d.relu = c.relu ? 1 : 0;
+    d.mt = fo_mt(c.out_cphys); d.nchunk = fo_nchunk(c.cin_phys, 1); d.out_cp = c.out_cphys;
+  }
+  return CP_OK;
+}
+
+}
diff --git a/checkerpose_amd/csrc/hr_fuse_out.hip b/checkerpose_amd/csrc/hr_fuse_out.hip
--- a/checkerpose_amd/csrc/hr_fuse_out.hip
+++ b/checkerpose_amd/csrc/hr_fuse_out.hip
@@ -1,196 +1,12 @@
-#include "common.h"
+#include "hr_fuse_dev.h"
 
 namespace {
 
-constexpr int FO_MAXCONV = 4, FO_NTB = 8, FO_MTB = 3, FO_THREADS = 256, FO_SLOTS = 192, FO_WB = 8, FO_SU = 17, FO_AFF = 160;
-
-struct FuseConvDev {
-  const void* w; const float* aff; void* out;
-  int kind, relu, mt, nchunk, out_cp, aff_n;
-};
-struct FuseOutParams {
-  const void* src;
-  int B, H, W, Cg, band, nconv, plane_bytes;
-  FuseConvDev c[FO_MAXCONV];
-};
-
-__device__ __forceinline__ void mma16f(const u32x4& w, const u32x4& a, f32x4& acc) {
-  acc = __builtin_amdgcn_mfma_f32_16x16x32_bf16(__builtin_bit_cast(bf16x8, w), __builtin_bit_cast(bf16x8, a), acc, 0, 0, 0);
-}
-
 __global__ __launch_bounds__(FO_THREADS) void hr_fuse_out_kernel(const FuseOutParams p) {
   extern __shared__ __attribute__((aligned(16))) unsigned char smem[];
-  const int tid = threadIdx.x;
-  const int lane = tid & 63;
-  const int wave = __builtin_amdgcn_readfirstlane(tid >> 6);
-  const int x = lane & 15, q = lane >> 4;
   const int nband = p.H / p.band;
   const int b = blockIdx.x / nband, r0 = (blockIdx.x - b * nband) * p.band;
-  const int RW = p.W + 1, RH = p.band + 1, Cg = p.Cg;
-  const int HE = (p.W >> 1) + 1;
-  auto colslot = [&](int rc) { return (rc & 1) ? HE + (rc >> 1) : (rc >> 1); };
-  const int planes_end = Cg * p.plane_bytes;
-  uint32_t* const tab = (uint32_t*)(smem + planes_end);
-
-  float* const saff = (float*)(tab + 2 * FO_SLOTS);
-  uint32_t* const sdesc = (uint32_t*)(saff + FO_MAXCONV * 2 * FO_AFF);
-  if (wave == FO_THREADS / 64 - 1) {
-    for (int s = lane; s < 2 * FO_SLOTS; s += 64) {
-      const int kind = s >= FO_SLOTS, sl = s - kind * FO_SLOTS;
-      uint32_t off = 0u;
-      if (kind == 0) { if (sl < Cg) off = (uint32_t)(sl * p.plane_bytes); }
-      else if (sl < 9 * Cg) {
-        const int tap = sl / Cg, cg = sl - tap * Cg;
-        const int ts = tap % 3;
-        off = (uint32_t)(cg * p.plane_bytes + ((tap / 3) * RW + (ts == 1 ? HE : ts >> 1)) * 16);
-      }
-      tab[s] = off;
-    }
-#pragma unroll
-    for (int ci = 0; ci < FO_MAXCONV; ++ci) {
-      if (ci < p.nconv) {
-        const float* const ga = p.c[ci].aff;
-        const int an = p.c[ci].aff_n;
-        for (int r = lane; r < 2 * FO_AFF; r += 64) {
-          const int h = r >= FO_AFF, c = r - h * FO_AFF;
-          saff[ci * 2 * FO_AFF + r] = c < an ? ga[h * an + c] : 0.f;
-        }
-        if (lane == 0) {
-          const uint64_t wq = (uint64_t)p.c[ci].w, oq = (uint64_t)p.c[ci].out;
-          uint32_t* d = sdesc + ci * 8;
-          d[0] = (uint32_t)wq; d[1] = (uint32_t)(wq >> 32); d[2] = (uint32_t)oq; d[3] = (uint32_t)(oq >> 32);
-          d[4] = (uint32_t)(p.c[ci].kind | (p.c[ci].relu << 1)); d[5] = (uint32_t)p.c[ci].mt; d[6] = (uint32_t)p.c[ci].nchunk;
-          d[7] = (uint32_t)p.c[ci].out_cp;
-        }
-      }
-    }
-  }
-  const int nconv = p.nconv;
-  auto D = [&](int ci, int k) -> int { return __builtin_amdgcn_readfirstlane((int)sdesc[ci * 8 + k]); };
-  {
-    const int per_row = p.W * Cg;
-    const u32x4* src = (const u32x4*)p.src + ((size_t)b * p.H * p.W) * Cg;
-    for (int pc = tid; pc < per_row; pc += FO_THREADS) {
-      const int c = pc / Cg, cg = pc - c * Cg;
-      unsigned char* dst = smem + cg * p.plane_bytes + colslot(c + 1) * 16;
-#pragma unroll 1
-      for (int ry0 = 0; ry0 < RH; ry0 += FO_SU) {
-        u32x4 v[FO_SU];
-#pragma unroll
-        for (int u = 0; u < FO_SU; ++u) {
-          const int gy = r0 - 1 + ry0 + u;
-          v[u] = u32x4{0u, 0u, 0u, 0u};
-          if (ry0 + u < RH && gy >= 0) v[u] = src[(size_t)gy * per_row + pc];
-        }
-#pragma unroll
-        for (int u = 0; u < FO_SU; ++u)
-          if (ry0 + u < RH) *(u32x4*)(dst + (ry0 + u) * RW * 16) = v[u];
-      }
-    }
-    for (int i = tid; i < RH * Cg; i += FO_THREADS) {
-      const int ry = i / Cg, cg = i - ry * Cg;
-      *(u32x4*)(smem + cg * p.plane_bytes + (ry * RW) * 16) = u32x4{0u, 0u, 0u, 0u};
-    }
-  }
-  __syncthreads();
-
-  auto split = [&](int n, int Wo, int& oy, int& ox) {
-    if ((Wo & (Wo - 1)) == 0) { const int lw = 31 - __builtin_clz((unsigned)Wo); oy = n >> lw; ox = n & (Wo - 1); }
-    else { oy = n / Wo; ox = n - oy * Wo; }
-  };
-  auto geom = [&](int ci, int& Wo, int& npx, int& ntile, int& npg, int& nrg) {
-    const int kind = D(ci, 4) & 1;
-    Wo = kind ? p.W >> 1 : p.W;
-    npx = Wo * (kind ? p.band >> 1 : p.band);
-    ntile = (npx + 15) >> 4;
-    npg = (ntile + FO_NTB - 1) / FO_NTB;
-    nrg = (D(ci, 5) + FO_MTB - 1) / FO_MTB;
-  };
-#pragma unroll 1
-  for (int t0 = wave, ci = 0, tbase = 0; ci < nconv; ++ci) {
-    int Wo, npx, ntile, npg, nrg;
-    geom(ci, Wo, npx, ntile, npg, nrg);
-    const int kind = D(ci, 4) & 1, relu = D(ci, 4) >> 1, mtc = D(ci, 5), nch = D(ci, 6), out_cp = D(ci, 7);
-    const u32x4* const wbase = (const u32x4*)(((uint64_t)(uint32_t)D(ci, 1) << 32) | (uint32_t)D(ci, 0)) + lane;
-    uint16_t* const outp = (uint16_t*)(((uint64_t)(uint32_t)D(ci, 3) << 32) | (uint32_t)D(ci, 2));
-    const uint32_t* const tb = tab + (kind ? FO_SLOTS : 0);
-    const int Ho = kind ? p.H >> 1 : p.H, oy0 = kind ? r0 >> 1 : r0;
-    const int nitem = nrg * npg;
-#pragma unroll 1
-    for (; t0 < tbase + nitem; t0 += 4) {
-      const int it = t0 - tbase;
-      const int rg = it / npg, pg = it - rg * npg;
-      const int mt0 = rg * FO_MTB, nm = mtc - mt0 < FO_MTB ? mtc - mt0 : FO_MTB;
-      const int tlim = ntile - pg * FO_NTB;
-      uint32_t base[FO_NTB];
-      f32x4 acc[FO_MTB][FO_NTB];
-#pragma unroll
-      for (int i = 0; i < FO_NTB; ++i) {
-        int n = (pg * FO_NTB + i) * 16 + x;
-        if (n >= npx) n = 0;
-        int oy, ox;
-        split(n, Wo, oy, ox);
-        base[i] = kind ? (uint32_t)(((2 * oy) * RW + ox) * 16) : (uint32_t)(((oy + 1) * RW + colslot(ox + 1)) * 16);
-#pragma unroll
-        for (int m = 0; m < FO_MTB; ++m) acc[m][i] = f32x4{0.f, 0.f, 0.f, 0.f};
-      }
-#pragma unroll 1
-      for (int kb = 0; kb < nch; kb += FO_WB) {
-        u32x4 wf[FO_MTB][FO_WB];
-#pragma unroll
-        for (int m = 0; m < FO_MTB; ++m)
-#pragma unroll
-          for (int k = 0; k < FO_WB; ++k) {
-            wf[m][k] = u32x4{0u, 0u, 0u, 0u};
-            if (m < nm && kb + k < nch) wf[m][k] = wbase[(size_t)((mt0 + m) * nch + kb + k) * 64];
-          }
-#pragma unroll
-        for (int k = 0; k < FO_WB; ++k) {
-          if (kb + k < nch) {
-            const uint32_t so = tb[(kb + k) * 4 + q];
-#pragma unroll
-            for (int i4 = 0; i4 < FO_NTB; i4 += 4) {
-              if (i4 < tlim) {
-                u32x4 a[4];
-#pragma unroll
-                for (int i = 0; i < 4; ++i) a[i] = *(const u32x4*)(smem + base[i4 + i] + so);
-#pragma unroll
-                for (int m = 0; m < FO_MTB; ++m)
-                  if (m < nm) {
-#pragma unroll
-                    for (int i = 0; i < 4; ++i) mma16f(wf[m][k], a[i], acc[m][i4 + i]);
-                  }
-              }
-            }
-          }
-        }
-      }
-#pragma unroll
-      for (int m = 0; m < FO_MTB; ++m) {
-        const int co = (mt0 + m) * 16 + 4 * q;
-        if (m < nm && co < out_cp) {
-          const f32x4 sc = *(const f32x4*)(saff + ci * 2 * FO_AFF + co), sh = *(const f32x4*)(saff + ci * 2 * FO_AFF + FO_AFF + co);
-#pragma unroll
-          for (int i = 0; i < FO_NTB; ++i) {
-            const int n = (pg * FO_NTB + i) * 16 + x;
-            if (i < tlim && n < npx) {
-              int oy, ox;
-              split(n, Wo, oy, ox);
-              float v[4];
-#pragma unroll
-              for (int j = 0; j < 4; ++j) {
-                v[j] = acc[m][i][j] * sc[j] + sh[j];
-                if (relu) v[j] = fmaxf(v[j], 0.f);
-              }
-              u32x2 pk; pk.x = pack_bf16x2(v[0], v[1]); pk.y = pack_bf16x2(v[2], v[3]);
-              *(u32x2*)(outp + ((size_t)(b * Ho + oy0 + oy) * Wo + ox) * out_cp + co) = pk;
-            }
-          }
-        }
-      }
-    }
-    tbase += nitem;
-  }
+  fo_run<FO_THREADS, FO_MTB, FO_NTB, FO_WB, FO_SU>(p, smem, b, r0);
 }
 
 __global__ void pack_fuse_out_weight_kernel(const float* __restrict__ w, uint16_t* __restrict__ out, int Cout, int Cin, int kind,
@@ -212,9 +28,6 @@
   }
   out[i] = (uint16_t)f32_to_bf16_bits(v);
 }
-
-inline int fo_nchunk(int cin_phys, int kind) { return ((kind ? 9 : 1) * (cin_phys / 8) + 3) / 4; }
-inline int fo_mt(int out_cphys) { return (out_cphys + 15) / 16; }
 
 }
 
@@ -256,7 +69,7 @@
   for (int cand = 2; cand <= H; cand += 2)
     if (H % cand == 0 && (size_t)(cand + 1) * (W + 1) * p.Cg * 16 + 16 * p.Cg <= 60 * 1024) band = cand;
   p.band = band;
-  p.plane_bytes = (band + 1) * (W + 1) * 16 + 16;
+  p.plane_bytes = fo_plane_bytes(band, W);
   for (int i = 0; i < nconv; ++i) {
     const CpFuseConv& c = convs[i];
     if (!c.packed_w || !c.affine || !c.out || (c.kind != 0 && c.kind != 1) || c.out_cphys <= 0 || c.out_cphys % 8 || c.out_cphys > FO_AFF) return CP_ERR_INVALID;
@@ -266,7 +79,7 @@
     d.w = c.packed_w; d.aff = c.affine; d.out = c.out; d.kind = c.kind; d.relu = c.relu ? 1 : 0;
     d.mt = fo_mt(c.out_cphys); d.nchunk = fo_nchunk(cin_phys, c.kind); d.out_cp = c.out_cphys; d.aff_n = d.mt * 16;
   }
-  const size_t lds = (size_t)p.Cg * p.plane_bytes + 2 * FO_SLOTS * 4 + (size_t)FO_MAXCONV * 2 * FO_AFF * 4 + FO_MAXCONV * 8 * 4;
+  const size_t lds = fo_lds_bytes(p.Cg, p.plane_bytes);
   const long long grid = (long long)B * (H / band);
   if (grid >= (1LL << 31)) return CP_ERR_RANGE;
   CP_LAUNCH(hr_fuse_out_kernel, dim3((unsigned)grid), dim3(FO_THREADS), lds, (hipStream_t)stream, p);
diff --git a/checkerpose_amd/engine.py b/checkerpose_amd/engine.py
--- a/checkerpose_amd/engine.py
+++ b/checkerpose_amd/engine.py
@@ -4,7 +4,7 @@
 import torch
 
 from . import _abi
-from ._abi import ACT_LEAKY, ACT_NONE, ACT_RELU, CP_BF16, CP_F16, CP_F32, CpChainTail, CpChainTailConv, CpConvDesc, CpFuseConv
+from ._abi import ACT_LEAKY, ACT_NONE, ACT_RELU, CP_BF16, CP_F16, CP_F32, CpChainDeep, CpChainTail, CpChainTailConv, CpConvDesc, CpFuseConv
 
 _TORCH_DT = {CP_F32: torch.float32, CP_BF16: torch.bfloat16}
 USE_HALO = os.environ.get("CHECKERPOSE_AMD_HALO", "1") != "0"
@@ -522,11 +522,11 @@
         return (USE_CHAIN_TAIL and self.can_chain(C_, H, W) and 1 <= len(convs) <= 3 and bool(self.lib.cp_hr_chain_tail_supported(C_, H, W))
                 and sum(_rup(c[1].shape[0], self.E) for c in convs) <= self.lib.cp_hr_chain_tail_channels())
 
-    def hr_chain(self, name, srcs, shifts, relu_in, ws, affs, C_, H, W, tail=None):
+    def hr_chain(self, name, srcs, shifts, relu_in, ws, affs, C_, H, W, tail=None, deep=None):
         blob, aff = self.ws.pack_chain(name, ws, affs, C_, H, W)
         out = self.act(H, W, C_)
         if tail is not None:
-            return self._hr_chain_tail(name, srcs, shifts, relu_in, blob, aff, out, C_, H, W, tail)
+            return self._hr_chain_tail(name, srcs, shifts, relu_in, blob, aff, out, C_, H, W, tail, deep)
         n = len(srcs)
         arr_p = (C.c_void_p * 4)()
         arr_s = (C.c_int32 * 4)(*([int(v) for v in shifts] + [0] * (4 - n)))
@@ -550,11 +550,52 @@
         self.conv_log.append((name, self.B * H * W, C_, 9 * C_, fl, "hr_chain", (n + 1) * nb + 8 * 9 * C_ * C_ * self.es))
         return out
 
+    def can_chain_deep(self, C_, H, W, c_first, couts):
+        hh, ww, cp = H >> 1, W >> 1, _rup(int(c_first), self.E)
+        for c in couts:
+            ocp = _rup(int(c), self.E)
+            if not self.lib.cp_hr_chain_deep_supported(C_, H, W, hh, ww, cp, ocp):
+                return False
+            hh, ww, cp = hh >> 1, ww >> 1, ocp
+        return True
+
+    def _chain_deep(self, touts, deep):
+        arr = (CpChainDeep * len(deep))()
+        douts, keep, fl, nbytes, srcs = [], [], 0, 0, []
+        for i, ((kind_, idx), wkey, w, scale, shift, relu) in enumerate(deep):
+            x = touts[idx] if kind_ == "t" else douts[idx]
+            assert kind_ == "t" or idx < i
+            Cout, Cin = int(w.shape[0]), int(w.shape[1])
+            assert Cin == x.C and x.coff == 0 and x.cstride == x.Cphys
+            out = self.act(x.H >> 1, x.W >> 1, Cout)
+            ck = ("fuse_out", wkey)
+            if ck not in self.ws.cache:
+                buf = torch.empty(self.lib.cp_hr_fuse_out_weight_bytes(x.Cphys, out.Cphys, 1), dtype=torch.uint8, device=self.device)
+                wc = w.contiguous()
+                self.ws.keep.append(wc)
+                st = torch.cuda.current_stream(self.device).cuda_stream
+                _abi.check(self.lib.cp_pack_hr_fuse_out_weight(st, wc.data_ptr(), Cout, Cin, x.Cphys, out.Cphys, 1, buf.data_ptr()),
+                           "cp_pack_hr_fuse_out_weight")
+                n = self.lib.cp_hr_fuse_out_affine_floats(out.Cphys)
+                aff = torch.zeros(2, n, dtype=torch.float32, device=self.device)
+                aff[0, :Cout] = scale
+                aff[1, :Cout] = shift
+                self.ws.cache[ck] = (buf, aff)
+            buf, aff = self.ws.cache[ck]
+            keep += [buf, aff]
+            arr[i].packed_w, arr[i].affine = buf.data_ptr(), aff.data_ptr()
+            arr[i].H, arr[i].W, arr[i].cin_phys, arr[i].Cout, arr[i].out_cphys, arr[i].relu = x.H, x.W, x.Cphys, Cout, out.Cphys, 1 if relu else 0
+            douts.append(out)
+            srcs.append(x.tbuf)
+            fl += 2 * x.B * out.H * out.W * 9 * Cin * Cout
+            nbytes += x.B * out.H * out.W * Cout * self.es + 9 * Cin * Cout * self.es
+        return arr, douts, keep, fl, nbytes, srcs
+
     def can_chain_tails(self, C_, H, W, convs):
         return (USE_CHAIN_TAILS and self.can_chain(C_, H, W) and 1 <= len(convs) <= 3 and
                 all(bool(self.lib.cp_hr_chain_tailconv_supported(C_, H, W, 1 if c[4] == 3 else 0, int(c[1].shape[0]))) for c in convs))
 
-    def hr_chain_tails(self, name, srcs, shifts, relu_in, ws, affs, C_, H, W, convs):
+    def hr_chain_tails(self, name, srcs, shifts, relu_in, ws, affs, C_, H, W, convs, deep=None):
         lib = self.lib
         blob, aff = self.ws.pack_chain(name, ws, affs, C_, H, W)
         out = self.act(H, W, C_)
@@ -592,22 +633,35 @@
             assert s_.coff == 0 and s_.cstride == s_.Cphys == out.Cphys and (s_.H << sh_, s_.W << sh_) == (H, W)
         tbs, ot, tts = [s_.tbuf for s_ in srcs], out.tbuf, [o.tbuf for o in touts]
         bp, ap = blob.data_ptr(), aff.data_ptr()
+        darr, douts, dsrc, dts = None, [], [], []
+        if deep:
+            darr, douts, dkeep, fl_d, nb_d, dsrc = self._chain_deep(touts, deep)
+            self.keep += dkeep + [darr]
+            dts = [o.tbuf for o in douts]
+            fl_t += fl_d
+            nb_t += nb_d
 
         def argb(P):
             for i, t in enumerate(tbs):
                 arr_p[i] = P(t)
             for i, t in enumerate(tts):
                 arr[i].out = P(t)
+            for i, t in enumerate(dts):
+                darr[i].src, darr[i].out = P(dsrc[i]), P(t)
+            if deep:
+                return (self.B, C_, H, W, n, arr_p, arr_s, 1 if relu_in else 0, bp, ap, P(ot), len(convs), arr, len(deep), darr)
             return (self.B, C_, H, W, n, arr_p, arr_s, 1 if relu_in else 0, bp, ap, P(ot), len(convs), arr)
 
-        self._add(lib.cp_hr_branch_chain_tails, argb, "hr_chain:" + name, tbs, [ot] + tts)
+        self._add(lib.cp_hr_branch_chain_tails_deep if deep else lib.cp_hr_branch_chain_tails, argb, "hr_chain:" + name, tbs, [ot] + tts + dts)
         fl = 8 * 2 * self.B * H * W * 9 * C_ * C_ + fl_t
         self.flops += fl
         nb = self.B * H * W * C_ * self.es
         self.conv_log.append((name, self.B * H * W, C_, 9 * C_, fl, "hr_chain", (n + 1) * nb + 8 * 9 * C_ * C_ * self.es + nb_t))
+        if deep:
+            return out, touts, douts
         return out, touts
 
-    def _hr_chain_tail(self, name, srcs, shifts, relu_in, blob, aff, out, C_, H, W, tail):
+    def _hr_chain_tail(self, name, srcs, shifts, relu_in, blob, aff, out, C_, H, W, tail, deep=None):
         lib = self.lib
         ck = ("chain_tail", name)
         if ck not in self.ws.cache:
@@ -641,20 +695,31 @@
             assert s_.coff == 0 and s_.cstride == s_.Cphys == out.Cphys and (s_.H << sh, s_.W << sh) == (H, W)
         tbs, ot, tts = [s_.tbuf for s_ in srcs], out.tbuf, [o.tbuf for o in touts]
         bp, ap = blob.data_ptr(), aff.data_ptr()
+        darr, douts, dsrc, dts, fl_d, nb_d = None, [], [], [], 0, 0
+        if deep:
+            darr, douts, dkeep, fl_d, nb_d, dsrc = self._chain_deep(touts, deep)
+            self.keep += dkeep + [darr]
+            dts = [o.tbuf for o in douts]
 
         def argb(P):
             for i, t in enumerate(tbs):
                 arr_p[i] = P(t)
             for i, t in enumerate(tts):
                 tl.out[i] = P(t)
+            for i, t in enumerate(dts):
+                darr[i].src, darr[i].out = P(dsrc[i]), P(t)
+            if deep:
+                return (self.B, C_, H, W, n, arr_p, arr_s, 1 if relu_in else 0, bp, ap, P(ot), C.byref(tl), len(deep), darr)
             return (self.B, C_, H, W, n, arr_p, arr_s, 1 if relu_in else 0, bp, ap, P(ot), C.byref(tl))
 
-        self._add(lib.cp_hr_branch_chain_tail, argb, "hr_chain:" + name, tbs, [ot] + tts)
-        fl = 8 * 2 * self.B * H * W * 9 * C_ * C_ + sum(2 * self.B * (H >> 1) * (W >> 1) * 9 * C_ * w.shape[0] for _, w, *_ in tail)
+        self._add(lib.cp_hr_branch_chain_tail_deep if deep else lib.cp_hr_branch_chain_tail, argb, "hr_chain:" + name, tbs, [ot] + tts + dts)
+        fl = 8 * 2 * self.B * H * W * 9 * C_ * C_ + sum(2 * self.B * (H >> 1) * (W >> 1) * 9 * C_ * w.shape[0] for _, w, *_ in tail) + fl_d
         self.flops += fl
         nb = self.B * H * W * C_ * self.es
-        nbt = sum(self.B * (H >> 1) * (W >> 1) * w.shape[0] * self.es + 9 * C_ * w.shape[0] * self.es for _, w, *_ in tail)
+        nbt = sum(self.B * (H >> 1) * (W >> 1) * w.shape[0] * self.es + 9 * C_ * w.shape[0] * self.es for _, w, *_ in tail) + nb_d
         self.conv_log.append((name, self.B * H * W, C_, 9 * C_, fl, "hr_chain", (n + 1) * nb + 8 * 9 * C_ * C_ * self.es + nbt))
+        if deep:
+            return out, touts, douts
         return out, touts
 
     def can_fuse_out(self, x: Act, couts=()):
diff --git a/checkerpose_amd/netbuilder.py b/checkerpose_amd/netbuilder.py
--- a/checkerpose_amd/netbuilder.py
+++ b/checkerpose_amd/netbuilder.py
@@ -265,6 +265,26 @@
         p = self.p
         terms = [[None] * nb for _ in range(nb)]
         first = {}
+        whole = set()
+
+        def deep_of(j, C_, H, W, targets):
+            ent, last = [], []
+            for n_, i in enumerate(targets):
+                if i - j <= 1:
+                    continue
+                q = "%s.fuse_layers.%d.%d" % (pfx, i, j)
+                keys = [("%s.%d.0" % (q, k), "%s.%d.1" % (q, k), k != i - j - 1) for k in range(1, i - j)]
+                if not p.can_chain_deep(C_, H, W, self.W(q + ".0.0.weight").shape[0], [self.W(ck + ".weight").shape[0] for ck, _, _ in keys]):
+                    return None, None
+                ref = ("t", n_)
+                for ck, bk, relu in keys:
+                    ent.append((ref, ck, self.W(ck + ".weight")) + tuple(self.ws.bn_fold(bk)) + (relu,))
+                    ref = ("d", len(ent) - 1)
+                last.append((i, len(ent) - 1))
+            if not ent or len(ent) > 3:
+                return None, None
+            return ent, last
+
         p.par_begin(nb)
         for j in range(nb):
             p.set_lane(j)
@@ -281,9 +301,16 @@
                 tl = [("%s.fuse_layers.%d.%d.0.0" % (pfx, i, j), "%s.fuse_layers.%d.%d.0.1" % (pfx, i, j), i - j > 1) for i in range(j + 1, nb)]
                 tconvs = [(ck, self.W(ck + ".weight")) + tuple(self.ws.bn_fold(bk)) + (relu,) for ck, bk, relu in tl]
                 if tl and all(i > j for i in range(nb) if i != j) and p.can_chain_tail(C_, H, W, tconvs):
-                    xs[j], touts = p.hr_chain(bp, srcs, shifts, not isinstance(xs[j], Act), ws, affs, C_, H, W, tail=tconvs)
+                    dent, dlast = deep_of(j, C_, H, W, list(range(j + 1, nb)))
+                    if dent:
+                        xs[j], touts, douts = p.hr_chain(bp, srcs, shifts, not isinstance(xs[j], Act), ws, affs, C_, H, W, tail=tconvs, deep=dent)
+                    else:
+                        xs[j], touts = p.hr_chain(bp, srcs, shifts, not isinstance(xs[j], Act), ws, affs, C_, H, W, tail=tconvs)
                     for i, o in zip(range(j + 1, nb), touts):
                         first[(i, j)] = o
+                    for i, k in (dlast or []):
+                        first[(i, j)] = douts[k]
+                        whole.add((i, j))
                     continue
                 lst_t = []
                 for i in range(nb):
@@ -294,9 +321,16 @@
                         lst_t.append((i, q + ".0.0", q + ".0.1", 3, i - j > 1))
                 tcv = [(ck, self.W(ck + ".weight")) + tuple(self.ws.bn_fold(bk)) + (k, relu) for (_, ck, bk, k, relu) in lst_t]
                 if nb > 1 and p.can_chain_tails(C_, H, W, tcv):
-                    xs[j], touts = p.hr_chain_tails(bp, srcs, shifts, not isinstance(xs[j], Act), ws, affs, C_, H, W, tcv)
+                    dent, dlast = deep_of(j, C_, H, W, [i for (i, _, _, _, _) in lst_t])
+                    if dent:
+                        xs[j], touts, douts = p.hr_chain_tails(bp, srcs, shifts, not isinstance(xs[j], Act), ws, affs, C_, H, W, tcv, deep=dent)
+                    else:
+                        xs[j], touts = p.hr_chain_tails(bp, srcs, shifts, not isinstance(xs[j], Act), ws, affs, C_, H, W, tcv)
                     for (i, _, _, _, _), o in zip(lst_t, touts):
                         first[(i, j)] = o
+                    for i, k in (dlast or []):
+                        first[(i, j)] = douts[k]
+                        whole.add((i, j))
                     continue
                 xs[j] = p.hr_chain(bp, srcs, shifts, not isinstance(xs[j], Act), ws, affs, C_, H, W)
             else:
@@ -317,7 +351,7 @@
                     first[(i, j)] = o
         def cost_of(i, j):
             if (i, j) in first:
-                return max(i - j - 1, 0)
+                return 0 if (i, j) in whole else max(i - j - 1, 0)
             return (i - j) if j < i else 0.3
         load = [0.0] * nb
         sched = []
@@ -338,7 +372,9 @@
         for ln, i, j in sched:
             p.set_lane(ln)
             q = "%s.fuse_layers.%d.%d" % (pfx, i, j)
-            if (i, j) in first:
+            if (i, j) in whole:
+                t = first[(i, j)]
+            elif (i, j) in first:
                 t = self._fuse_chain_rest(first[(i, j)], [("%s.%d.0" % (q, k), "%s.%d.1" % (q, k), k != i - j - 1) for k in range(1, i - j)])
             elif j > i:
                 t = self.conv_bn(xs[j], q + ".0", q + ".1", 1, 1, 0, relu=False)
diff --git a/include/checkerpose_hip.h b/include/checkerpose_hip.h
--- a/include/checkerpose_hip.h
+++ b/include/checkerpose_hip.h
@@ -208,6 +208,21 @@
 int cp_pack_hr_fuse_out_weight(cp_stream_t stream, const float* w, int Cout, int Cin, int cin_phys, int out_cphys, int kind,
                                void* packed);
 int cp_hr_fuse_out(cp_stream_t stream, const void* src, int B, int H, int W, int cin_phys, int nconv, const CpFuseConv* convs);
+
+typedef struct CpChainDeep {
+  const void* src;
+  const void* packed_w;
+  const float* affine;
+  void* out;
+  int32_t H, W, cin_phys, Cout, out_cphys, relu;
+} CpChainDeep;
+int cp_hr_chain_deep_supported(int C, int H, int W, int src_H, int src_W, int cin_phys, int out_cphys);
+int cp_hr_branch_chain_tail_deep(cp_stream_t stream, int B, int C, int H, int W, int nsrc, const void* const* srcs,
+                                 const int32_t* shifts, int relu_in, const void* packed_w, const float* affine, void* out,
+                                 const CpChainTail* tail, int ndeep, const CpChainDeep* deep);
+int cp_hr_branch_chain_tails_deep(cp_stream_t stream, int B, int C, int H, int W, int nsrc, const void* const* srcs, const int32_t* shifts,
+                                  int relu_in, const void* packed_w, const float* affine, void* out, int ntail, const CpChainTailConv* convs,
+                                  int ndeep, const CpChainDeep* deep);
 
 int cp_edgeconv_fused_supported(int N, int K, int Cin, int Cout);
 size_t cp_edgeconv_fused_weight_bytes(int Cin, int Cout);
```

Result: slower. 25190 crops/s (-4.9%).
